# CodexploreRepo/deepfm

Measured on AMD Instinct MI355X. Metric: train samples/sec DeepFM Criteo-shape bs4096, higher is better.
Workload: dtype f32

## Files before the change

deepfm_amd/_lib.py:

```python

from __future__ import annotations

import ctypes as C
import os
from typing import Optional

_HERE = os.path.dirname(os.path.abspath(__file__))
LIB_PATH = os.environ.get("DFM_LIB_PATH") or os.path.join(_HERE, "lib", "libdeepfm_hip.so")

ABI_VERSION = 9

MAX_FIELDS = 64
MAX_RANKS = 64
ROWPLAN_CHUNK = 4096
RECORD_PARAM_LDS_BYTES = 32768
BWD_RECORD_MAX_ROW_SAMPLES = 1 << 27
BWD_RECORD_LDS_BYTES = 65536
SPARSE, DENSE, SEQUENCE = 0, 1, 2
COMBINER = {"mean": 0, "sum": 1, "max": 2}

c_float_p = C.c_void_p
c_int_p = C.c_void_p


class Field(C.Structure):
    _fields_ = [("kind", C.c_int32), ("dim", C.c_int32), ("vocab", C.c_int32), ("max_len", C.c_int32),
                ("combiner", C.c_int32), ("flat_offset", C.c_int32), ("stride2", C.c_int32),
                ("stride1", C.c_int32),
                ("w2", C.c_void_p), ("b2", C.c_void_p), ("w1", C.c_void_p), ("b1", C.c_void_p),
                ("proj", C.c_void_p)]


class FieldGrad(C.Structure):
    _fields_ = [("w2", C.c_void_p), ("b2", C.c_void_p), ("w1", C.c_void_p), ("b1", C.c_void_p),
                ("proj", C.c_void_p)]


class Table(C.Structure):
    _fields_ = [("w2", C.c_void_p), ("m2", C.c_void_p), ("v2", C.c_void_p),
                ("w1", C.c_void_p), ("m1", C.c_void_p), ("v1", C.c_void_p),
                ("stride2", C.c_int32), ("stride1", C.c_int32)]


class Optim(C.Structure):
    _fields_ = [("kind", C.c_int32), ("beta1", C.c_float), ("beta2", C.c_float), ("eps", C.c_float),
                ("weight_decay", C.c_float), ("momentum", C.c_float), ("d_lr", C.c_void_p)]


OPT_ADAM, OPT_ADAMW, OPT_SGD = 0, 1, 2


class BnBwd(C.Structure):
    _fields_ = [("z", C.c_void_p), ("mean_rstd", C.c_void_p), ("gamma", C.c_void_p), ("beta", C.c_void_p),
                ("dy", C.c_void_p), ("g_gamma", C.c_void_p), ("g_beta", C.c_void_p),
                ("seed", C.c_void_p), ("workspace", C.c_void_p), ("p_drop", C.c_float), ("salt", C.c_int32)]


class FmBwd(C.Structure):
    _fields_ = [("g_fm", C.c_void_p), ("fm_sum", C.c_void_p), ("e", C.c_void_p), ("addend", C.c_void_p),
                ("dim", C.c_int32)]


class SlabRef(C.Structure):
    _fields_ = [("workspace", C.c_void_p), ("g_w", C.c_void_p), ("batch", C.c_int64), ("out_features", C.c_int32),
                ("in_features", C.c_int32), ("splits", C.c_int32), ("reserved", C.c_int32)]


class SplitJob(C.Structure):
    _fields_ = [("src", C.c_void_p), ("rows", C.c_int64), ("cols", C.c_int64), ("planes_f", C.c_void_p),
                ("planes_s", C.c_void_p)]


class PartialJob(C.Structure):
    _fields_ = [("kind", C.c_int32), ("blocks", C.c_int32), ("n1", C.c_int32), ("n2", C.c_int32),
                ("accumulate", C.c_int32), ("reserved", C.c_int32), ("partial", C.c_void_p), ("out_w", C.c_void_p),
                ("out_b", C.c_void_p), ("ldw", C.c_int64)]


class HeadTail(C.Structure):
    _fields_ = [("g_w", C.c_void_p), ("g_b", C.c_void_p), ("loss", C.c_void_p), ("g_b2", C.c_void_p)]


_P, _I, _L, _F, _SZ = C.c_void_p, C.c_int, C.c_int64, C.c_float, C.c_size_t
SIGNATURES = {
    "dfm_abi_version": (_I, []),
    "dfm_last_error": (C.c_char_p, []),
    "dfm_device_info": (_I, [_P, _P, C.c_char_p, _I]),
    "dfm_debug_empty_launch": (_I, [_P]),
    "dfm_embedding_plan_create": (_I, [C.POINTER(Field), _I, _I, C.POINTER(_P)]),
    "dfm_embedding_plan_destroy": (_I, [_P]),
    "dfm_embedding_plan_is_uniform": (_I, [_P]),
    "dfm_embedding_workspace_bytes": (_SZ, [_P, _L]),
    "dfm_embedding_forward": (_I, [_P, C.POINTER(_P), _L, _P, _P, _P, _P, _P, _P, _P, _P]),
    "dfm_embedding_forward_staged": (_I, [_P, C.POINTER(_P), C.POINTER(_P), _P, _P, _L, _P, _P, _P, _P, _P, _P]),
    "dfm_embedding_forward_staged_update": (_I, [_P, _P, _P, C.POINTER(_P), C.POINTER(_P), _P, _P, _L, _P, _P, _P, _P, _P]),
    "dfm_embedding_forward_record": (_I, [_P, _P, _L, _P, _P, _P, _L, _P, _P, _P, _P]),
    "dfm_embedding_forward_record_update": (_I, [_P, _P, _P, _P, _L, _P, _P, _P, _L, _P, _P, _P]),
    "dfm_embedding_backward_record_parts": (_I, [_L]),
    "dfm_embedding_backward_record_workspace_bytes": (_SZ, [_L, _L]),
    "dfm_embedding_backward_record": (_I, [_P, _P, _L, _P, _P, _P, _L, _P, _L, C.POINTER(FieldGrad), _P, _L, _P, _P]),
    "dfm_embedding_backward_record_update": (_I, [_P, _P, _P, _P, _L, _P, _P, _P, _L, _P, _L, C.POINTER(FieldGrad), _P,
                                                  _L, _P]),
    "dfm_embedding_forward_record_sum": (_I, [_P, _P, _L, _P, _P, _P, _L, _P, _P, _P, _P, _P]),
    "dfm_embedding_forward_record_sum_update": (_I, [_P, _P, _P, _P, _L, _P, _P, _P, _L, _P, _P, _P, _P]),
    "dfm_embedding_backward_record_fm": (_I, [_P, _P, _L, _P, _P, _P, _L, _P, _L, _P, _P, _P, C.POINTER(FieldGrad), _P,
                                              _L, _P, _P]),
    "dfm_embedding_backward_record_fm_update": (_I, [_P, _P, _P, _P, _L, _P, _P, _P, _L, _P, _L, _P, _P, _P,
                                                     C.POINTER(FieldGrad), _P, _L, _P]),
    "dfm_graph_last_node": (_I, [_P, C.POINTER(_P)]),
    "dfm_gather_timing_begin": (_I, [_I]),
    "dfm_gather_timing_end": (_I, [C.POINTER(C.c_float), _I, C.POINTER(_I)]),
    "dfm_gather_set_shape": (_I, [_I]),
    "dfm_cin_set_mode": (_I, [_I]),
    "dfm_cin_get_mode": (_I, []),
    "dfm_embedding_backward_dense": (_I, [_P, C.POINTER(_P), _L, _P, _P, _P, C.POINTER(FieldGrad), _P, _P]),
    "dfm_embedding_backward_dense_fields": (_I, [_P, C.POINTER(_P), _L, _P, _P, _P, C.POINTER(FieldGrad), _P]),
    "dfm_rowplan_build": (_I, [C.POINTER(_P), C.POINTER(C.c_int32), _I, _L, _P, _P, _P, _P, _P, _P, _I, _P]),
    "dfm_rowplan_build_update": (_I, [_P, _P, C.POINTER(_P), C.POINTER(C.c_int32), _I, _L, _P, _P, _P, _P, _P, _P, _I]),
    "dfm_rowgrad_build": (_I, [C.POINTER(C.c_int32), _I, _I, _I, _L, _P, _P, _P, _P, _P, _P, _P, _P]),
    "dfm_rowadam_num_partials": (_L, [_I, _I, _I]),
    "dfm_grad_norm_finalize": (_I, [_P, _L, _F, _P, _P, _P, _P, _P]),
    "dfm_cin_output_dim": (_I, [C.POINTER(C.c_int32), _I, _I]),
    "dfm_cin_saved_bytes": (_SZ, [C.POINTER(C.c_int32), _I, _I, _L, _I, _I]),
    "dfm_cin_backward_workspace_bytes": (_SZ, [C.POINTER(C.c_int32), _I, _I, _L, _I, _I]),
    "dfm_cin_forward_workspace_bytes": (_SZ, [C.POINTER(C.c_int32), _I, _I, _I, _I]),
    "dfm_cin_forward": (_I, [_P, _L, _I, _I, C.POINTER(_P), C.POINTER(_P), C.POINTER(C.c_int32), _I, _I, _P, _P, _P, _P]),
    "dfm_cin_backward": (_I, [_P, _L, _I, _I, C.POINTER(_P), C.POINTER(C.c_int32), _I, _I, _P, _P, _P,
                              C.POINTER(_P), C.POINTER(_P), _P, _P]),
    "dfm_attention_forward": (_I, [_P, _L, _I, _I, _I, _I, _I, C.POINTER(_P), _P, _P]),
    "dfm_attention_backward_workspace_bytes": (_SZ, [_L, _I, _I]),
    "dfm_attention_backward": (_I, [_P, _P, _L, _I, _I, _I, _I, _I, C.POINTER(_P), _P, C.POINTER(_P), _P, _P]),
    "dfm_bn_workspace_bytes": (_SZ, [_L, _I]),
    "dfm_bn_relu_dropout_forward": (_I, [_P, _L, _I, _P, _P, _P, _P, _P, _F, _F, _F, _P, _I, _P, _P, _P, _P]),
    "dfm_bn_relu_dropout_backward": (_I, [_P, _P, _P, _P, _P, _L, _I, _F, _P, _I, _P, _P, _P, _P, _P]),
    "dfm_bce_workspace_bytes": (_SZ, [_L]),
    "dfm_bce_with_logits": (_I, [_P, _P, _L, _P, _P, _P, _P]),
    "dfm_gemm_workspace_bytes": (_SZ, [_I, _I, _I]),
    "dfm_gemm_f32": (_I, [_P, _L, _I, _P, _L, _I, _P, _L, _I, _I, _I, _P, _I, _P, _P]),
    "dfm_weight_grad_workspace_bytes": (_SZ, [_L, _I, _I]),
    "dfm_weight_grad_f32": (_I, [_P, _L, _P, _L, _L, _I, _I, _P, _L, _P, _I, _P, _P]),
    "dfm_attention_core_supported": (_I, [_I, _I, _I]),
    "dfm_attention_core_forward": (_I, [_P, _L, _I, _I, _I, _P, _P]),
    "dfm_attention_core_backward": (_I, [_P, _P, _L, _I, _I, _I, _P, _P]),
    "dfm_attention_qkv_core_supported": (_I, [_I, _I, _I, _I]),
    "dfm_attention_qkv_core_forward": (_I, [_P, _P, _P, _L, _I, _I, _I, _I, _P, _P]),
    "dfm_attention_qkv_core_backward": (_I, [_P, _P, _P, _P, _L, _I, _I, _I, _I, _P, _P]),
    "dfm_attention_block_supported": (_I, [_I, _I, _I, _I]),
    "dfm_attention_block_forward": (_I, [_P, _P, _P, _P, _P, _P, _P, _F, _L, _I, _I, _I, _I, _P, _P, _P, _P, _L, _P, _L,
                                         _P]),
    "dfm_attention_block_backward": (_I, [_P, _P, _P, _P, _P, _I, _L, _I, _I, _I, _I, _P, _P, _P, _L, _P, _P, _P]),
    "dfm_layernorm_workspace_bytes": (_SZ, [_L, _I]),
    "dfm_layernorm_forward": (_I, [_P, _P, _L, _I, _P, _P, _F, _P, _P, _L, _L, _P]),
    "dfm_layernorm_backward": (_I, [_P, _P, _P, _P, _L, _I, _P, _P, _P, _P, _P, _L, _L, _P]),
    "dfm_linear_bn_workspace_bytes": (_SZ, [_L, _I]),
    "dfm_linear_bn_forward": (_I, [_P, _L, _P, _P, _L, _I, _I, _P, _P, _P]),
    "dfm_bn_relu_dropout_apply": (_I, [_P, _L, _I, _P, _P, _P, _P, _P, _P, _P, _F, _F, _F, _P, _I, _P, _P]),
    "dfm_bn_bwd_workspace_bytes": (_SZ, [_L, _I]),
    "dfm_bn_backward_apply": (_I, [C.POINTER(BnBwd), _L, _I, C.POINTER(HeadTail), _P, _P]),
    "dfm_linear1_supported": (_I, [_I]),
    "dfm_linear1_forward": (_I, [_P, _L, _I, _P, _P, _P, _P]),
    "dfm_linear1_backward_splits": (_I, [_L]),
    "dfm_linear1_backward": (_I, [_P, _P, _L, _I, _P, _P, _P, _P]),
    "dfm_head_bce": (_I, [_P, _L, _I, _P, _P, _P, _P, _P, _P, _P, C.POINTER(BnBwd), _P]),
    "dfm_head_bn_bce": (_I, [_P, _P, _P, _P, _P, _F, _F, _L, _I, _P, _P, _P, _P, _P, _P, _P, C.POINTER(BnBwd), _P]),
    "dfm_linear_backward_workspace_bytes": (_SZ, [_L, _I, _I]),
    "dfm_linear_backward": (_I, [_P, _L, _I, _P, _I, _P, _P, C.POINTER(BnBwd), C.POINTER(FmBwd), _I, _P, _P]),
    "dfm_linear_backward_finish": (_I, [C.POINTER(SlabRef), _I, _P]),
    "dfm_linear_backward_splits": (_I, [_L, _I, _I]),
    "dfm_step_embedding_backward": (_I, [_P, _I, C.POINTER(_P), C.POINTER(FieldGrad), C.POINTER(C.c_int32), _I, _I, _I,
                                         _L, _P, _P, _P, _P, _P, _P, _P, _P, _I, _P, _L, _P]),
    "dfm_step_prepare_num_partials": (_L, [_I, _I, _I, _L]),
    "dfm_step_match_bytes": (_SZ, [_I, _I]),
    "dfm_step_prepare": (_I, [C.POINTER(Table), _I, _I, _I, _P, _P, _P, _P, _P, _F, _F, _P, _P, _L, _L,
                              C.POINTER(SlabRef), _I, _P, _I, _L, _P, _L, _P, _P]),
    "dfm_step_apply": (_I, [C.POINTER(Table), _I, _I, _I, _P, _P, _P, _P, _P, _P, C.POINTER(Optim), _P, _P, _P, _P,
                            _P, _L, _I, _P]),
    "dfm_step_apply_plan": (_I, [C.POINTER(Table), _I, _I, _I, _P, _P, _P, _P, _P, _P, C.POINTER(Optim), _P, _P, _P,
                                 _P, _P, _L, _I, _P, _L, _P, _I, _L, _P, _P, _P, _P, _P, _P]),
    "dfm_step_apply_plan_update": (_I, [_P, _P, C.POINTER(Table), _I, _I, _I, _P, _P, _P, _P, _P, _P,
                                        C.POINTER(Optim), _P, _P, _P, _P, _P, _L, _I, _P, _L, _P, _I, _L, _P, _P, _P,
                                        _P, _P]),
    "dfm_step_dense_num_partials": (_L, [_L]),
    "dfm_step_dense_prepare": (_I, [_F, _P, _P, _L, _L, C.POINTER(SlabRef), _I, _P, _P]),
    "dfm_step_dense_apply": (_I, [_P, C.POINTER(Optim), _P, _P, _P, _P, _P, _L, _I, _P]),
    "dfm_weight_grad_partial_blocks": (_I, [_L]),
    "dfm_weight_grad_partials_f32": (_I, [_P, _L, _P, _L, _L, _I, _I, _P, _P]),
    "dfm_weight_grad_partials_pair_f32": (_I, [_P, _L, _P, _L, _I, _I, _P, _P, _L, _P, _L, _I, _I, _P, _L, _P]),
    "dfm_layernorm_partial_blocks": (_I, [_L]),
    "dfm_partials_finish": (_I, [C.POINTER(PartialJob), _I, _P]),
    "dfm_tower_set_mode": (_I, [_I]),
    "dfm_tower_get_mode": (_I, []),
    "dfm_planes_bytes": (_SZ, [_L, _L]),
    "dfm_tower_x6_supported": (_I, [_L, _I, _I]),
    "dfm_split_planes": (_I, [C.POINTER(SplitJob), _I, _P]),
    "dfm_linear_bn_forward_x6": (_I, [_P, _L, _P, _P, _P, _L, _I, _I, _P, _P, _P]),
    "dfm_bn_relu_dropout_apply_planes": (_I, [_P, _L, _I, _P, _P, _P, _P, _P, _P, _P, _F, _F, _F, _P, _I, _P, _P, _P,
                                              _P]),
    "dfm_bn_backward_apply_planes": (_I, [C.POINTER(BnBwd), _L, _I, C.POINTER(HeadTail), _P, _P, _P, _P]),
    "dfm_linear_backward_x6_splits": (_I, [_L, _I, _I]),
    "dfm_linear_backward_x6_workspace_bytes": (_SZ, [_L, _I, _I]),
    "dfm_linear_backward_x6": (_I, [_P, _P, _L, _I, _P, _P, _I, _P, _P, C.POINTER(BnBwd), C.POINTER(FmBwd), _P, _P]),
    "dfm_fm_forward": (_I, [_P, _L, _I, _I, _P, _P]),
    "dfm_fm_backward": (_I, [_P, _P, _L, _I, _I, _P, _P]),
    "dfm_copy_2d": (_I, [_P, _L, _P, _L, _L, _I, _P]),
    "dfm_stage_record": (_I, [_P, _P, _L, _P]),
    "dfm_stage_record_update": (_I, [_P, _P, _P, _P, _L]),
    "dfm_shard_gather": (_I, [C.POINTER(Table), C.POINTER(C.c_int32), _I, _I, _I, _L, _P, _P, _P, _P, _P]),
    "dfm_shard_pack_segment": (_L, [_L, _I, _I, _L]),
    "dfm_shard_pack": (_I, [C.POINTER(C.c_int32), C.POINTER(C.c_int32), _I, C.POINTER(C.c_int32), _I, _I, _I, _L,
                            _P, _P, _P, _L, C.POINTER(SlabRef), _I, _P, _P]),
    "dfm_shard_rowgrad": (_I, [_I, _I, _I, _L, _P, _L, _P, _P, _P, _P, _P, _P]),
    "dfm_sum_floats": (_I, [_P, _L, _P, _P]),
    "dfm_embedding_grad_combine": (_I, [_P, _L, _P, _P, _P, _P, _L, _I, _I, _P, _P]),
    "dfm_linear_bn_eval": (_I, [_P, _L, _P, _P, _L, _I, _I, _P, _P, _P, _P, _F, _P, _P]),
    "dfm_predict_head": (_I, [_P, _L, _I, _P, _P, _P, _P, _L, _P, _P, _P]),
    "dfm_predict_head_update": (_I, [_P, _P, _P, _L, _I, _P, _P, _P, _P, _L, _P, _P]),
    "dfm_metrics_workspace_bytes": (_SZ, [_L]),
    "dfm_metrics_prepare": (_I, [_P, _P, _L, _P, _P, _P]),
    "dfm_metrics_finish": (_I, [_P, _P, _L, _P, _P, _P, _P]),
    "dfm_ranking_workspace_bytes": (_SZ, [_L, _L]),
    "dfm_ranking_metrics": (_I, [_P, _P, _P, _L, _L, _P, _I, _I, _P, _P, _P]),
}

_lib: Optional[C.CDLL] = None


class HipLibraryError(RuntimeError):
    pass


def load() -> C.CDLL:
    global _lib
    if _lib is not None:
        return _lib
    if not os.path.exists(LIB_PATH):
        raise HipLibraryError(
            f"{LIB_PATH} not found: build it with `python -c 'import __graft_entry__ as g; g.build()'` "
            "(or `make -C deepfm_amd/csrc`). deepfm_amd has no CPU or eager-PyTorch fallback.")
    lib = C.CDLL(LIB_PATH)
    for name, (restype, argtypes) in SIGNATURES.items():
        fn = getattr(lib, name)
        fn.restype = restype
        fn.argtypes = argtypes
    if lib.dfm_abi_version() != ABI_VERSION:
        raise HipLibraryError(f"ABI version mismatch: library {lib.dfm_abi_version()} != binding {ABI_VERSION} "
                              f"(stale {LIB_PATH}? rebuild with make -C deepfm_amd/csrc)")
    _lib = lib
    return lib


ERR_UNSUPPORTED = 3


def check(rc: int) -> None:
    if rc != 0:
        msg = load().dfm_last_error().decode("utf-8", "replace")
        raise HipLibraryError(f"deepfm_hip error {rc}: {msg}")


def ptr(t) -> int:
    return 0 if t is None else t.data_ptr()


def stream_handle() -> int:
    import torch
    return torch.cuda.current_stream().cuda_stream


def require_device(t, what: str) -> None:
    if not t.is_cuda:
        raise RuntimeError(
            f"{what} is on {t.device}: deepfm_amd runs on an MI355X HIP device only "
            "(there is no CPU fallback; use the reference implementation on CPU).")
```

deepfm_amd/csrc/step_tail.hip:

```cpp
#include "rowplan_body.h"
#include "tail_bodies.h"

using namespace dfm;
using namespace dfm::tail;

namespace {
constexpr int kStepPrepPerThread = 4;
__device__ __forceinline__ void dense_prepare_slabs_body(int blk, float* __restrict__ g, const float* __restrict__ p,
                                                         int64_t n, int64_t n_l2, float l2, const SlabTable& st,
                                                         const float* __restrict__ gathered, int world,
                                                         int64_t gathered_stride, float scale,
                                                         float* __restrict__ partial) {
  const int64_t i = (static_cast<int64_t>(blk) * kTailThreads + threadIdx.x) * kStepPrepPerThread;
  float sq = 0.f;
  const float k = 2.f * l2;
  if (i + 3 < n) {
    float4 gi = ld4(g + i);
    bool dirty = false;
    if (gathered) {
      gi = make_float4(0.f, 0.f, 0.f, 0.f);
      for (int r = 0; r < world; ++r) {
        const float4 t = ld4(gathered + static_cast<int64_t>(r) * gathered_stride + i);
        gi.x += t.x; gi.y += t.y; gi.z += t.z; gi.w += t.w;
      }
      gi.x *= scale; gi.y *= scale; gi.z *= scale; gi.w *= scale;
      dirty = true;
    }
    if (add_slabs(gi, g + i, st)) dirty = true;
    if (i < n_l2) {
      const float4 pi = ld4(p + i);
      gi.x = fmaf(k, pi.x, gi.x); gi.y = fmaf(k, pi.y, gi.y); gi.z = fmaf(k, pi.z, gi.z); gi.w = fmaf(k, pi.w, gi.w);
      dirty = true;
    }
    if (dirty) st4(g + i, gi);
    sq = fmaf(gi.x, gi.x, sq); sq = fmaf(gi.y, gi.y, sq); sq = fmaf(gi.z, gi.z, sq); sq = fmaf(gi.w, gi.w, sq);
  } else {
    for (int64_t e = i; e < n; ++e) {
      float ge = g[e];
      if (gathered) {
        ge = 0.f;
        for (int r = 0; r < world; ++r) ge += gathered[static_cast<int64_t>(r) * gathered_stride + e];
        ge *= scale;
        g[e] = ge;
      }
      if (e < n_l2) { ge = fmaf(k, p[e], ge); g[e] = ge; }
      sq = fmaf(ge, ge, sq);
    }
  }
  block_partial(sq, partial, blk);
}
}

__global__ __launch_bounds__(kTailThreads) void step_embedding_backward_kernel(
    int dense_blocks, const int32_t* __restrict__ dense_list, PtrTable in, GradTable gt, int64_t B, int F, int D,
    const float* __restrict__ g_first, const float* __restrict__ g_field, FieldMap fmap, int S, int lists,
    const int32_t* __restrict__ sorted_pos, int32_t* seg_start,
    const int32_t* __restrict__ num_uniq, float* __restrict__ row_g2, float* __restrict__ row_g1,
    DensePartials dp) {
  const int blk = blockIdx.x;
  if (blk < dense_blocks)
    dense_fields_uniform_body(blk, dense_list, in, gt, B, F, D, g_first, g_field, dp);
  else
    rowgrad_body(blk - dense_blocks, fmap, S, F, D, lists, g_first, g_field, sorted_pos, seg_start, num_uniq, row_g2,
                 row_g1);
}

constexpr int kMatchThreads = 1024;
__global__ __launch_bounds__(kMatchThreads) void step_match_kernel(int S, int L, const int32_t* __restrict__ uniq_rows,
                                                                  const int32_t* __restrict__ num_uniq,
                                                                  uint8_t* __restrict__ match) {
  rowadam_match_body<kMatchThreads>(blockIdx.x, S, L, uniq_rows, num_uniq, match);
}

__global__ __launch_bounds__(kTailThreads) void step_prepare_kernel(
    int merge_blocks, TableArgs tabs, int S, int D, int L, const int32_t* __restrict__ uniq_rows,
    const int32_t* __restrict__ num_uniq, float* __restrict__ row_g2, float* __restrict__ row_g1,
    int32_t* __restrict__ owner_flag, float grad_scale, float l2, float* __restrict__ g, const float* __restrict__ p,
    int64_t n, int64_t n_l2, SlabTable slabs, const float* __restrict__ dense_gathered, int world,
    int64_t gathered_stride, float* __restrict__ partial, int64_t dense_partial_offset,
    const uint8_t* __restrict__ match) {
  const int blk = blockIdx.x;
  if (blk < merge_blocks)
    rowadam_merge_body(blk, tabs, S, D, L, uniq_rows, num_uniq, row_g2, row_g1, owner_flag, grad_scale, l2, partial,
                       match);
  else
    dense_prepare_slabs_body(blk - merge_blocks, g, p, n, n_l2, l2, slabs, dense_gathered, world, gathered_stride,
                             grad_scale, partial + dense_partial_offset);
}

__global__ __launch_bounds__(1024) void norm_finalize_kernel(const float* __restrict__ partial, int n,
                                                             float max_norm, float* __restrict__ sq_out,
                                                             float* __restrict__ clip_out,
                                                             int32_t* __restrict__ step_tick,
                                                             int64_t* __restrict__ seed_tick) {
  __shared__ float wsum[16];
  float acc = 0.f;
  for (int i = threadIdx.x; i < n; i += 1024) acc += partial[i];
#pragma unroll
  for (int m = 32; m >= 1; m >>= 1) acc += __shfl_xor(acc, m, kWave);
  if (lane_id() == 0) wsum[threadIdx.x >> 6] = acc;
  __syncthreads();
  if (threadIdx.x == 0) {
    float tot = 0.f;
    for (int i = 0; i < 16; ++i) tot += wsum[i];
    sq_out[0] = tot;
    if (clip_out) {
      float c = 1.f;
      if (max_norm > 0.f) c = fminf(1.f, max_norm / (sqrtf(tot) + 1e-6f));
      clip_out[0] = c;
    }
    if (step_tick) step_tick[0] += 1;
    if (seed_tick) seed_tick[0] += 1;
  }
}

template <int RULE>
__global__ __launch_bounds__(kTailThreads) void step_apply_kernel(
    int row_blocks, TableArgs tabs, int S, int D, int L, const int32_t* __restrict__ uniq_rows,
    const int32_t* __restrict__ num_uniq, const float* __restrict__ row_g2, const float* __restrict__ row_g1,
    const int32_t* __restrict__ owner_flag, const float* __restrict__ clip_coef, const float* __restrict__ lr_ptr,
    OptHyper h, const int32_t* __restrict__ step_ptr, float* __restrict__ p, float* __restrict__ m,
    float* __restrict__ v, float* __restrict__ g, int64_t n, int zero_grad) {
  const int blk = blockIdx.x;
  const float lr_now = lr_ptr[0];
  if (blk < row_blocks)
    rowadam_apply_body<RULE>(blk, tabs, S, D, L, uniq_rows, num_uniq, row_g2, row_g1, owner_flag, clip_coef, lr_now, h,
                             step_ptr);
  else
    dense_adam_body<RULE>(blk - row_blocks, p, m, v, g, n, clip_coef, lr_now, h, step_ptr, zero_grad ? g : nullptr);
}

template <typename KeyT, int SHIFT, int RULE>
__global__ __launch_bounds__(rowplan::SORT_THREADS) void step_apply_plan_kernel(
    int plan_blocks, const int64_t* __restrict__ ids_base, int64_t ids_stride, const int32_t* __restrict__ vocab,
    int64_t plan_n, int chunks, int32_t* __restrict__ p_sorted_pos, int32_t* __restrict__ p_uniq_rows,
    int32_t* __restrict__ p_seg_start, int32_t* __restrict__ p_num_uniq, int32_t* p_error,
    int row_blocks4, TableArgs tabs, int S, int D, int L, const int32_t* __restrict__ uniq_rows,
    const int32_t* __restrict__ num_uniq, const float* __restrict__ row_g2, const float* __restrict__ row_g1,
    const int32_t* __restrict__ owner_flag, const float* __restrict__ clip_coef, const float* __restrict__ lr_ptr,
    OptHyper h, const int32_t* __restrict__ step_ptr, float* __restrict__ p, float* __restrict__ m,
    float* __restrict__ v, float* __restrict__ g, int64_t n, int zero_grad) {
  if (static_cast<int>(blockIdx.x) < plan_blocks) {
    const int s = blockIdx.x % S, y = blockIdx.x / S;
    const int64_t* src = ids_base + s * ids_stride;
    if (y < chunks) {
      rowplan::rowplan_chunk_body<KeyT, SHIFT>(src, vocab[s], s, y, S, plan_n, p_sorted_pos, p_uniq_rows, p_seg_start,
                                               p_num_uniq, p_error, 0);
    } else {
      const int q = y - chunks;
      const dfm_table tb = tabs.t[s];
      rowplan::rowplan_touch_body(src, vocab[s], tb.w2, tb.stride2, q / rowplan::kTouchParts, q % rowplan::kTouchParts,
                                  plan_n);
    }
    return;
  }
  const int blk = (static_cast<int>(blockIdx.x) - plan_blocks) * (rowplan::SORT_THREADS / kTailThreads);
  const float lr_now = lr_ptr[0];
  if (blk < row_blocks4)
    rowadam_apply_body<RULE>(blk, tabs, S, D, L, uniq_rows, num_uniq, row_g2, row_g1, owner_flag, clip_coef, lr_now, h,
                             step_ptr);
  else
    dense_adam_body<RULE>(blk - row_blocks4, p, m, v, g, n, clip_coef, lr_now, h, step_ptr, zero_grad ? g : nullptr);
}

namespace {
int fill_tables(const dfm_table* tables, int S, int D, TableArgs* out, int need_state) {
  memset(out, 0, sizeof(*out));
  for (int s = 0; s < S; ++s) {
    DFM_REQUIRE(tables[s].w2 && tables[s].w1, "table %d: null weights", s);
    if (need_state >= 1) DFM_REQUIRE(tables[s].m2 && tables[s].m1, "table %d: null optimizer state", s);
    if (need_state >= 2) DFM_REQUIRE(tables[s].v2 && tables[s].v1, "table %d: null Adam state", s);
    out->t[s] = tables[s];
    if (out->t[s].stride2 == 0) out->t[s].stride2 = D;
    if (out->t[s].stride1 == 0) out->t[s].stride1 = 1;
    DFM_REQUIRE(out->t[s].stride2 >= D && out->t[s].stride2 % 4 == 0 && out->t[s].stride1 >= 1,
                "table %d: bad row strides", s);
  }
  return DFM_OK;
}
inline int64_t row_blocks(int S, int D, int L) {
  return (static_cast<int64_t>(L) * S * CH * (D / 4) + kTailThreads - 1) / kTailThreads;
}
inline int64_t prep_blocks(int64_t n) {
  const int64_t per = static_cast<int64_t>(kTailThreads) * kStepPrepPerThread;
  return (n + per - 1) / per;
}
}

extern "C" int dfm_step_embedding_backward(const int32_t* d_dense_list, int num_dense, const void* const* dense_x,
                                           const dfm_field_grad* dense_grads, const int32_t* field_of_sparse,
                                           int num_sparse, int num_fields, int dim, int64_t batch,
                                           const float* d_g_first, const float* d_g_field,
                                           const int32_t* d_sorted_pos, int32_t* d_seg_start,
                                           const int32_t* d_num_uniq, float* d_row_g2, float* d_row_g1,
                                           float* d_dense_partials, int dense_parts, const float* d_dense_grad_base,
                                           int64_t dense_grad_elems, dfm_stream_t stream) {
  DFM_REQUIRE(d_g_first && d_g_field, "null argument");
  DFM_REQUIRE(num_dense >= 0 && num_sparse >= 0 && num_dense + num_sparse > 0 && num_fields <= DFM_MAX_FIELDS &&
                  num_dense + num_sparse <= num_fields, "bad field counts");
  DFM_REQUIRE(dim > 0 && dim % 4 == 0 && batch > 0 && batch < (int64_t(1) << 31), "bad shape");
  DFM_REQUIRE((reinterpret_cast<uintptr_t>(d_g_field) & 15) == 0, "d_g_field must be 16-byte aligned");
  PtrTable in;
  GradTable gt;
  memset(&in, 0, sizeof(in));
  memset(&gt, 0, sizeof(gt));
  if (num_dense > 0) {
    DFM_REQUIRE(d_dense_list && dense_x && dense_grads, "null argument");
    for (int f = 0; f < num_fields; ++f) {
      in.p[f] = dense_x[f];
      gt.g[f] = dense_grads[f];
    }
  }
  FieldMap fm;
  memset(&fm, 0, sizeof(fm));
  int lists = 0;
  int64_t rg_blocks = 0;
  if (num_sparse > 0) {
    DFM_REQUIRE(field_of_sparse && d_sorted_pos && d_seg_start && d_num_uniq && d_row_g2 && d_row_g1, "null argument");
    for (int s = 0; s < num_sparse; ++s) {
      DFM_REQUIRE(field_of_sparse[s] >= 0 && field_of_sparse[s] < num_fields, "field_of_sparse[%d] out of range", s);
      fm.f[s] = field_of_sparse[s];
    }
    lists = static_cast<int>((batch + CH - 1) / CH) * num_sparse;
    rg_blocks = (static_cast<int64_t>(lists) * CH * (dim / 4) + kTailThreads - 1) / kTailThreads;
  }
  int dense_blocks = num_dense * (dim / 4 + 1);
  DensePartials dp = {nullptr, nullptr, 0, 0, 0};
  if (d_dense_partials && num_dense > 0) {
    DFM_REQUIRE(dense_parts >= 1 && dense_parts <= 64 && d_dense_grad_base && dense_grad_elems > 0, "bad dense slices");
    for (int i = 0; i < num_fields; ++i) {
      const dfm_field_grad& g = gt.g[i];
      if (!g.w2) continue;
      DFM_REQUIRE(g.w2 >= d_dense_grad_base && g.w2 + dim <= d_dense_grad_base + dense_grad_elems &&
                      g.b2 >= d_dense_grad_base && g.b2 + dim <= d_dense_grad_base + dense_grad_elems &&
                      g.w1 >= d_dense_grad_base && g.w1 < d_dense_grad_base + dense_grad_elems &&
                      g.b1 >= d_dense_grad_base && g.b1 < d_dense_grad_base + dense_grad_elems,
                  "field %d: a DENSE-field gradient buffer lies outside the sliced range", i);
    }
    dp.out = d_dense_partials; dp.base = d_dense_grad_base; dp.elems = dense_grad_elems;
    dp.rows = (batch + dense_parts - 1) / dense_parts;
    dp.per_slice = dense_blocks;
    dense_blocks *= dense_parts;
  }
  hipLaunchKernelGGL(step_embedding_backward_kernel, dim3(static_cast<unsigned>(dense_blocks + rg_blocks)),
                     dim3(kTailThreads), 0, as_stream(stream), dense_blocks, d_dense_list, in, gt, batch, num_fields, dim,
                     d_g_first, d_g_field, fm, num_sparse, lists, d_sorted_pos, d_seg_start, d_num_uniq, d_row_g2,
                     d_row_g1, dp);
  DFM_LAUNCH_CHECK();
  return DFM_OK;
}

extern "C" size_t dfm_step_match_bytes(int num_sparse, int num_lists) {
  return num_lists > 2 ? static_cast<size_t>(num_lists) * num_sparse * CH * num_lists : 0;
}

extern "C" int64_t dfm_rowadam_num_partials(int num_sparse, int dim, int num_lists) {
  return row_blocks(num_sparse, dim, num_lists);
}

extern "C" int64_t dfm_step_prepare_num_partials(int num_sparse, int dim, int num_lists, int64_t n) {
  return row_blocks(num_sparse, dim, num_lists) + prep_blocks(n);
}

extern "C" int dfm_step_prepare(const dfm_table* tables, int num_sparse, int dim, int num_lists,
                                const int32_t* d_uniq_rows, const int32_t* d_num_uniq, float* d_row_g2,
                                float* d_row_g1, int32_t* d_owner_flag, float grad_scale, float l2, float* d_g,
                                const float* d_p, int64_t n, int64_t n_l2, const dfm_slab_ref* slabs, int num_slabs,
                                const float* d_dense_gathered, int world, int64_t gathered_stride, float* d_partials,
                                int64_t dense_partial_offset, void* d_match, dfm_stream_t stream) {
  DFM_REQUIRE(tables && d_uniq_rows && d_num_uniq && d_row_g2 && d_row_g1 && d_owner_flag && d_partials && d_g && d_p,
              "null argument");
  DFM_REQUIRE(num_sparse > 0 && num_sparse <= DFM_MAX_FIELDS && num_lists > 0, "bad sizes");
  DFM_REQUIRE(dim > 0 && dim % 4 == 0 && dim <= 256, "dim must be a multiple of 4 and <= 256");
  DFM_REQUIRE(n > 0 && n_l2 >= 0 && n_l2 <= n && n_l2 % 16 == 0, "bad dense sizes (n_l2 must be a multiple of 16)");
  DFM_REQUIRE((reinterpret_cast<uintptr_t>(d_g) & 63) == 0 && (reinterpret_cast<uintptr_t>(d_p) & 15) == 0,
              "dense buffers must be 64-byte aligned");
  DFM_REQUIRE(!d_dense_gathered || (world >= 1 && (reinterpret_cast<uintptr_t>(d_dense_gathered) & 15) == 0 && n % 4 == 0),
              "gathered dense gradients: world >= 1, 16-byte aligned, n a multiple of 4");
  if (d_dense_gathered && gathered_stride == 0) gathered_stride = n;
  DFM_REQUIRE(!d_dense_gathered || (gathered_stride >= n && gathered_stride % 4 == 0),
              "gathered dense gradients: the stride between ranks must be >= n and a multiple of 4 floats");
  TableArgs ta;
  if (int rc = fill_tables(tables, num_sparse, dim, &ta, 0)) return rc;
  SlabTable st = {};
  if (int rc = fill_slab_table(slabs, num_slabs, d_g, n, &st)) return rc;
  const int64_t mb = row_blocks(num_sparse, dim, num_lists), pb = prep_blocks(n);
  if (dense_partial_offset == 0) dense_partial_offset = mb;
  DFM_REQUIRE(dense_partial_offset >= mb, "the dense partials must not overlap the %lld row partials", (long long)mb);
  uint8_t* match = (d_match && num_lists > 2) ? static_cast<uint8_t*>(d_match) : nullptr;
  if (match) {
    DFM_REQUIRE(num_lists <= 255, "at most 255 lists");
    hipLaunchKernelGGL(step_match_kernel, dim3(static_cast<unsigned>(num_sparse * num_lists * num_lists)),
                       dim3(kMatchThreads), 0, as_stream(stream), num_sparse, num_lists, d_uniq_rows, d_num_uniq, match);
    DFM_LAUNCH_CHECK();
  }
  hipLaunchKernelGGL(step_prepare_kernel, dim3(static_cast<unsigned>(mb + pb)), dim3(kTailThreads), 0,
                     as_stream(stream), static_cast<int>(mb), ta, num_sparse, dim, num_lists, d_uniq_rows, d_num_uniq,
                     d_row_g2, d_row_g1, d_owner_flag, grad_scale, l2, d_g, d_p, n, n_l2, st, d_dense_gathered, world,
                     gathered_stride, d_partials, dense_partial_offset, match);
  DFM_LAUNCH_CHECK();
  return DFM_OK;
}

extern "C" int dfm_grad_norm_finalize(const float* d_partials, int64_t num_partials, float max_norm,
                                      float* d_sq_norm, float* d_clip_coef, int32_t* d_step_tick,
                                      int64_t* d_seed_tick, dfm_stream_t stream) {
  DFM_REQUIRE(d_partials && d_sq_norm, "null argument");
  DFM_REQUIRE(num_partials >= 0 && num_partials < (int64_t(1) << 31), "bad partial count");
  hipLaunchKernelGGL(norm_finalize_kernel, dim3(1), dim3(1024), 0, as_stream(stream), d_partials,
                     static_cast<int>(num_partials), max_norm, d_sq_norm, d_clip_coef, d_step_tick, d_seed_tick);
  DFM_LAUNCH_CHECK();
  return DFM_OK;
}

namespace {
int check_optim(const dfm_optim* o) {
  DFM_REQUIRE(o, "null dfm_optim");
  DFM_REQUIRE(o->kind == DFM_OPT_ADAM || o->kind == DFM_OPT_ADAMW || o->kind == DFM_OPT_SGD,
              "unknown dfm_optim.kind %d", static_cast<int>(o->kind));
  DFM_REQUIRE(o->d_lr, "dfm_optim.d_lr must point to the learning rate on the device");
  DFM_REQUIRE((reinterpret_cast<uintptr_t>(o->d_lr) & 3) == 0, "dfm_optim.d_lr must be 4-byte aligned");
  return DFM_OK;
}
inline int state_needed(int kind) { return kind == DFM_OPT_SGD ? 1 : 2; }
inline OptHyper hyper_of(const dfm_optim& o) { return OptHyper{o.beta1, o.beta2, o.eps, o.weight_decay, o.momentum}; }
}

extern "C" int dfm_step_apply(const dfm_table* tables, int num_sparse, int dim, int num_lists,
                              const int32_t* d_uniq_rows, const int32_t* d_num_uniq, const float* d_row_g2,
                              const float* d_row_g1, const int32_t* d_owner_flag, const float* d_clip_coef,
                              const dfm_optim* opt, const int32_t* d_step, float* d_p, float* d_m, float* d_v,
                              float* d_g, int64_t n, int zero_grad, dfm_stream_t stream) {
  if (int rc = check_optim(opt)) return rc;
  const dfm_optim& o = *opt;
  DFM_REQUIRE(tables && d_uniq_rows && d_num_uniq && d_row_g2 && d_row_g1 && d_owner_flag && d_step && d_p && d_m &&
                  (d_v || o.kind == DFM_OPT_SGD) && d_g, "null argument");
  DFM_REQUIRE(num_sparse > 0 && num_sparse <= DFM_MAX_FIELDS && num_lists > 0 && n > 0, "bad sizes");
  DFM_REQUIRE(dim > 0 && dim % 4 == 0 && dim <= 256, "dim must be a multiple of 4 and <= 256");
  TableArgs ta;
  if (int rc = fill_tables(tables, num_sparse, dim, &ta, state_needed(o.kind))) return rc;
  const int64_t rb = row_blocks(num_sparse, dim, num_lists), ab = (n + kTailThreads - 1) / kTailThreads;
  const OptHyper h = hyper_of(o);
  const dim3 grid(static_cast<unsigned>(rb + ab));
  switch (o.kind) {
#define DFM_LAUNCH_APPLY(RULE)                                                                                          \
  hipLaunchKernelGGL((step_apply_kernel<RULE>), grid, dim3(kTailThreads), 0, as_stream(stream), static_cast<int>(rb), ta, \
                     num_sparse, dim, num_lists, d_uniq_rows, d_num_uniq, d_row_g2, d_row_g1, d_owner_flag,            \
                     d_clip_coef, o.d_lr, h, d_step, d_p, d_m, d_v, d_g, n, zero_grad)
    case DFM_OPT_ADAM: DFM_LAUNCH_APPLY(kRuleAdam); break;
    case DFM_OPT_ADAMW: DFM_LAUNCH_APPLY(kRuleAdamW); break;
    default: DFM_LAUNCH_APPLY(kRuleSGD); break;
#undef DFM_LAUNCH_APPLY
  }
  DFM_LAUNCH_CHECK();
  return DFM_OK;
}

namespace {
struct ApplyPlanLaunch {
  const void* func = nullptr;
  dim3 grid, block;
  unsigned lds = 0;
  int plan_blocks = 0, chunks = 0, row_blocks4 = 0, S = 0, D = 0, L = 0, zero_grad = 0;
  const int64_t* ids_base = nullptr;
  int64_t ids_stride = 0, plan_n = 0, n = 0;
  const int32_t* vocab = nullptr;
  int32_t *p_sorted_pos = nullptr, *p_uniq_rows = nullptr, *p_seg_start = nullptr, *p_num_uniq = nullptr, *p_error = nullptr;
  TableArgs tabs;
  const int32_t *uniq_rows = nullptr, *num_uniq = nullptr, *owner_flag = nullptr, *step_ptr = nullptr;
  const float *row_g2 = nullptr, *row_g1 = nullptr, *clip_coef = nullptr, *lr_ptr = nullptr;
  OptHyper h = {0, 0, 0, 0, 0};
  float *p = nullptr, *m = nullptr, *v = nullptr, *g = nullptr;
  void* params[36];
  void bind() {
    int k = 0;
    params[k++] = &plan_blocks; params[k++] = &ids_base; params[k++] = &ids_stride; params[k++] = &vocab;
    params[k++] = &plan_n; params[k++] = &chunks; params[k++] = &p_sorted_pos; params[k++] = &p_uniq_rows;
    params[k++] = &p_seg_start; params[k++] = &p_num_uniq; params[k++] = &p_error; params[k++] = &row_blocks4;
    params[k++] = &tabs; params[k++] = &S; params[k++] = &D; params[k++] = &L; params[k++] = &uniq_rows;
    params[k++] = &num_uniq; params[k++] = &row_g2; params[k++] = &row_g1; params[k++] = &owner_flag;
    params[k++] = &clip_coef; params[k++] = &lr_ptr; params[k++] = &h;
    params[k++] = &step_ptr; params[k++] = &p; params[k++] = &m; params[k++] = &v; params[k++] = &g; params[k++] = &n;
    params[k++] = &zero_grad;
  }
};

template <int RULE>
const void* apply_plan_func(bool narrow) {
  return narrow ? reinterpret_cast<const void*>(step_apply_plan_kernel<uint32_t, 12, RULE>)
                : reinterpret_cast<const void*>(step_apply_plan_kernel<unsigned long long, 32, RULE>);
}

int describe_apply_plan(const dfm_table* tables, int num_sparse, int dim, int num_lists, const int32_t* d_uniq_rows,
                        const int32_t* d_num_uniq, const float* d_row_g2, const float* d_row_g1,
                        const int32_t* d_owner_flag, const float* d_clip_coef, const dfm_optim& o,
                        const int32_t* d_step, float* d_p, float* d_m, float* d_v, float* d_g, int64_t n,
                        int zero_grad, const int64_t* d_next_ids, int64_t ids_stride, const int32_t* d_vocab,
                        int max_vocab, int64_t batch, int32_t* d_next_sorted_pos, int32_t* d_next_uniq_rows,
                        int32_t* d_next_seg_start, int32_t* d_next_num_uniq, int32_t* d_error_flag, ApplyPlanLaunch* a) {
  DFM_REQUIRE(tables && d_uniq_rows && d_num_uniq && d_row_g2 && d_row_g1 && d_owner_flag && d_step && d_p && d_m &&
                  (d_v || o.kind == DFM_OPT_SGD) && d_g, "null argument");
  DFM_REQUIRE(d_next_ids && d_vocab && d_next_sorted_pos && d_next_uniq_rows && d_next_seg_start && d_next_num_uniq,
              "null row-plan argument");
  DFM_REQUIRE(num_sparse > 0 && num_sparse <= DFM_MAX_FIELDS && num_lists > 0 && n > 0, "bad sizes");
  DFM_REQUIRE(dim > 0 && dim % 4 == 0 && dim <= 256, "dim must be a multiple of 4 and <= 256");
  DFM_REQUIRE(batch > 0 && batch < (int64_t(1) << 31) && ids_stride >= batch && max_vocab > 0, "bad batch / id stride");
  if (int rc = fill_tables(tables, num_sparse, dim, &a->tabs, state_needed(o.kind))) return rc;
  const bool narrow = max_vocab < (1 << 20) - 1;
  a->func = o.kind == DFM_OPT_ADAM ? apply_plan_func<kRuleAdam>(narrow)
          : o.kind == DFM_OPT_ADAMW ? apply_plan_func<kRuleAdamW>(narrow)
                                    : apply_plan_func<kRuleSGD>(narrow);
  a->lds = rowplan::lds_bytes(narrow);
  static bool allowed[3][2] = {{false, false}, {false, false}, {false, false}};
  if (!allowed[o.kind][narrow ? 0 : 1]) {
    DFM_HIP_TRY(hipFuncSetAttribute(a->func, hipFuncAttributeMaxDynamicSharedMemorySize, static_cast<int>(a->lds)));
    allowed[o.kind][narrow ? 0 : 1] = true;
  }
  constexpr int kPer = rowplan::SORT_THREADS / kTailThreads;
  const int64_t rb = row_blocks(num_sparse, dim, num_lists), ab = (n + kTailThreads - 1) / kTailThreads;
  const int64_t rb4 = (rb + kPer - 1) / kPer * kPer;
  a->chunks = static_cast<int>((batch + CH - 1) / CH);
  a->plan_blocks = num_sparse * a->chunks * (1 + rowplan::kTouchParts);
  a->row_blocks4 = static_cast<int>(rb4);
  a->grid = dim3(static_cast<unsigned>(a->plan_blocks + rb4 / kPer + (ab + kPer - 1) / kPer));
  a->block = dim3(rowplan::SORT_THREADS);
  a->S = num_sparse; a->D = dim; a->L = num_lists; a->zero_grad = zero_grad;
  a->ids_base = d_next_ids; a->ids_stride = ids_stride; a->vocab = d_vocab; a->plan_n = batch; a->n = n;
  a->p_sorted_pos = d_next_sorted_pos; a->p_uniq_rows = d_next_uniq_rows; a->p_seg_start = d_next_seg_start;
  a->p_num_uniq = d_next_num_uniq; a->p_error = d_error_flag;
  a->uniq_rows = d_uniq_rows; a->num_uniq = d_num_uniq; a->row_g2 = d_row_g2; a->row_g1 = d_row_g1;
  a->owner_flag = d_owner_flag; a->clip_coef = d_clip_coef; a->lr_ptr = o.d_lr; a->h = hyper_of(o);
  a->step_ptr = d_step; a->p = d_p; a->m = d_m; a->v = d_v; a->g = d_g;
  a->bind();
  return DFM_OK;
}

int update_apply_plan(void* graph_exec, void* node, const ApplyPlanLaunch& a) {
  return update_kernel_node(graph_exec, node, a.func, a.grid, a.block, a.lds, const_cast<void**>(a.params), true);
}
}

#define DFM_APPLY_PLAN_ARGS                                                                                              \
  tables, num_sparse, dim, num_lists, d_uniq_rows, d_num_uniq, d_row_g2, d_row_g1, d_owner_flag, d_clip_coef, *opt,      \
      d_step, d_p, d_m, d_v, d_g, n, zero_grad, d_next_ids, ids_stride, d_vocab, max_vocab, batch, d_next_sorted_pos,  \
      d_next_uniq_rows, d_next_seg_start, d_next_num_uniq, d_error_flag

extern "C" int dfm_step_apply_plan(const dfm_table* tables, int num_sparse, int dim, int num_lists,
                                   const int32_t* d_uniq_rows, const int32_t* d_num_uniq, const float* d_row_g2,
                                   const float* d_row_g1, const int32_t* d_owner_flag, const float* d_clip_coef,
                                   const dfm_optim* opt, const int32_t* d_step, float* d_p, float* d_m, float* d_v,
                                   float* d_g, int64_t n, int zero_grad, const int64_t* d_next_ids, int64_t ids_stride,
                                   const int32_t* d_vocab, int max_vocab, int64_t batch, int32_t* d_next_sorted_pos,
                                   int32_t* d_next_uniq_rows, int32_t* d_next_seg_start, int32_t* d_next_num_uniq,
                                   int32_t* d_error_flag, dfm_stream_t stream) {
  if (int rc = check_optim(opt)) return rc;
  ApplyPlanLaunch a;
  if (int rc = describe_apply_plan(DFM_APPLY_PLAN_ARGS, &a)) return rc;
  DFM_HIP_TRY(hipLaunchKernel(a.func, a.grid, a.block, a.params, a.lds, as_stream(stream)));
  DFM_LAUNCH_CHECK();
  return DFM_OK;
}

extern "C" int dfm_step_apply_plan_update(void* graph_exec, void* node, const dfm_table* tables, int num_sparse, int dim,
                                          int num_lists, const int32_t* d_uniq_rows, const int32_t* d_num_uniq,
                                          const float* d_row_g2, const float* d_row_g1, const int32_t* d_owner_flag,
                                          const float* d_clip_coef, const dfm_optim* opt, const int32_t* d_step,
                                          float* d_p, float* d_m, float* d_v, float* d_g, int64_t n, int zero_grad,
                                          const int64_t* d_next_ids, int64_t ids_stride, const int32_t* d_vocab,
                                          int max_vocab, int64_t batch, int32_t* d_next_sorted_pos,
                                          int32_t* d_next_uniq_rows, int32_t* d_next_seg_start,
                                          int32_t* d_next_num_uniq, int32_t* d_error_flag) {
  DFM_REQUIRE(graph_exec && node, "null argument");
  if (int rc = check_optim(opt)) return rc;
  ApplyPlanLaunch a;
  if (int rc = describe_apply_plan(DFM_APPLY_PLAN_ARGS, &a)) return rc;
  return update_apply_plan(graph_exec, node, a);
}

__global__ __launch_bounds__(kTailThreads) void step_dense_prepare_kernel(float l2, float* __restrict__ g,
                                                                          const float* __restrict__ p, int64_t n,
                                                                          int64_t n_l2, SlabTable slabs,
                                                                          float* __restrict__ partial) {
  dense_prepare_slabs_body(blockIdx.x, g, p, n, n_l2, l2, slabs, nullptr, 1, 0, 1.f, partial);
}

template <int RULE>
__global__ __launch_bounds__(kTailThreads) void step_dense_apply_kernel(
    const float* __restrict__ clip_coef, const float* __restrict__ lr_ptr, OptHyper h,
    const int32_t* __restrict__ step_ptr, float* __restrict__ p, float* __restrict__ m, float* __restrict__ v,
    float* __restrict__ g, int64_t n, int zero_grad) {
  dense_adam_body<RULE>(blockIdx.x, p, m, v, g, n, clip_coef, lr_ptr[0], h, step_ptr, zero_grad ? g : nullptr);
}

extern "C" int64_t dfm_step_dense_num_partials(int64_t n) { return n > 0 ? prep_blocks(n) : 0; }

extern "C" int dfm_step_dense_prepare(float l2, float* d_g, const float* d_p, int64_t n, int64_t n_l2,
                                      const dfm_slab_ref* slabs, int num_slabs, float* d_partials,
                                      dfm_stream_t stream) {
  DFM_REQUIRE(d_g && d_p && d_partials, "null argument");
  DFM_REQUIRE(n > 0 && n < (int64_t(1) << 40) && n_l2 >= 0 && n_l2 <= n && n_l2 % 16 == 0,
              "bad dense sizes (n_l2 must be a multiple of 16)");
  DFM_REQUIRE((reinterpret_cast<uintptr_t>(d_g) & 63) == 0 && (reinterpret_cast<uintptr_t>(d_p) & 15) == 0,
              "dense buffers must be 64-byte aligned");
  SlabTable st = {};
  if (int rc = fill_slab_table(slabs, num_slabs, d_g, n, &st)) return rc;
  hipLaunchKernelGGL(step_dense_prepare_kernel, dim3(static_cast<unsigned>(prep_blocks(n))), dim3(kTailThreads), 0,
                     as_stream(stream), l2, d_g, d_p, n, n_l2, st, d_partials);
  DFM_LAUNCH_CHECK();
  return DFM_OK;
}

extern "C" int dfm_step_dense_apply(const float* d_clip_coef, const dfm_optim* opt, const int32_t* d_step, float* d_p,
                                    float* d_m, float* d_v, float* d_g, int64_t n, int zero_grad,
                                    dfm_stream_t stream) {
  if (int rc = check_optim(opt)) return rc;
  const dfm_optim& o = *opt;
  DFM_REQUIRE(d_step && d_p && d_m && (d_v || o.kind == DFM_OPT_SGD) && d_g, "null argument");
  DFM_REQUIRE(n > 0 && n < (int64_t(1) << 38), "bad size");
  const OptHyper h = hyper_of(o);
  const dim3 grid(static_cast<unsigned>((n + kTailThreads - 1) / kTailThreads));
  switch (o.kind) {
#define DFM_LAUNCH_DENSE_APPLY(RULE)                                                                              \
  hipLaunchKernelGGL((step_dense_apply_kernel<RULE>), grid, dim3(kTailThreads), 0, as_stream(stream), d_clip_coef, \
                     o.d_lr, h, d_step, d_p, d_m, d_v, d_g, n, zero_grad)
    case DFM_OPT_ADAM: DFM_LAUNCH_DENSE_APPLY(kRuleAdam); break;
    case DFM_OPT_ADAMW: DFM_LAUNCH_DENSE_APPLY(kRuleAdamW); break;
    default: DFM_LAUNCH_DENSE_APPLY(kRuleSGD); break;
#undef DFM_LAUNCH_DENSE_APPLY
  }
  DFM_LAUNCH_CHECK();
  return DFM_OK;
}
```

deepfm_amd/csrc/tail_bodies.h:

```cpp
#pragma once

#include "common.h"

namespace dfm {
namespace tail {

constexpr int CH = DFM_ROWPLAN_CHUNK;
constexpr int kTailThreads = 256;

struct FieldMap {
  int32_t f[DFM_MAX_FIELDS];
};
struct TableArgs {
  dfm_table t[DFM_MAX_FIELDS];
};

constexpr int kMaxSlabs = 16;
struct SlabTable {
  const float* slabs[kMaxSlabs];
  float* g[kMaxSlabs];
  int64_t elems[kMaxSlabs];
  int splits[kMaxSlabs];
  int count;
};

__device__ __forceinline__ bool add_slabs(float4& gi, const float* gptr, const SlabTable& st) {
  bool any = false;
  for (int r = 0; r < st.count; ++r) {
    const int64_t off = gptr - st.g[r];
    if (off >= 0 && off < st.elems[r]) {
      const float* sl = st.slabs[r] + off;
      const int64_t stride = st.elems[r];
      const int splits = st.splits[r];
      int q = 0;
      for (; q + 8 <= splits; q += 8) {
        float4 t[8];
#pragma unroll
        for (int u = 0; u < 8; ++u) t[u] = ld4(sl + (q + u) * stride);
#pragma unroll
        for (int u = 0; u < 8; ++u) { gi.x += t[u].x; gi.y += t[u].y; gi.z += t[u].z; gi.w += t[u].w; }
      }
      for (; q < splits; ++q) {
        const float4 t = ld4(sl + q * stride);
        gi.x += t.x; gi.y += t.y; gi.z += t.z; gi.w += t.w;
      }
      any = true;
    }
  }
  return any;
}

__device__ __forceinline__ void block_partial(float sq, float* __restrict__ partial, int blk) {
  __shared__ float wsum[4];
#pragma unroll
  for (int m = 32; m >= 1; m >>= 1) sq += __shfl_xor(sq, m, kWave);
  if (lane_id() == 0) wsum[threadIdx.x >> 6] = sq;
  __syncthreads();
  if (threadIdx.x == 0) partial[blk] = (wsum[0] + wsum[1]) + (wsum[2] + wsum[3]);
}

__device__ __forceinline__ void block_sum2(float& a, float& b2) {
  __shared__ float sa[4], sb[4];
#pragma unroll
  for (int m = 32; m >= 1; m >>= 1) {
    a += __shfl_xor(a, m, kWave);
    b2 += __shfl_xor(b2, m, kWave);
  }
  const int w = threadIdx.x >> 6;
  __syncthreads();
  if (lane_id() == 0) { sa[w] = a; sb[w] = b2; }
  __syncthreads();
  a = sa[0] + sa[1] + sa[2] + sa[3];
  b2 = sb[0] + sb[1] + sb[2] + sb[3];
}

struct DensePartials {
  float* out;
  const float* base;
  int64_t elems, rows;
  int per_slice;
};
__device__ __forceinline__ void dense_fields_uniform_body(int blk, const int32_t* __restrict__ dense_list, PtrTable in, GradTable gt, int64_t B, int F, int D, const float* __restrict__ g_first, const float* __restrict__ g_field, DensePartials dp = DensePartials{nullptr, nullptr, 0, 0, 0}) {
  const int groups = D / 4 + 1;
  int64_t b_lo = 0, b_hi = B;
  int slice = 0;
  if (dp.out) {
    slice = blk / dp.per_slice;
    blk -= slice * dp.per_slice;
    b_lo = slice * dp.rows;
    b_hi = b_lo + dp.rows < B ? b_lo + dp.rows : B;
  }
  const int f = dense_list[blk / groups];
  const int jq = blk % groups;
  const float* x = static_cast<const float*>(in.p[f]);
  float sw[4] = {0.f, 0.f, 0.f, 0.f}, sb[4] = {0.f, 0.f, 0.f, 0.f};
  if (jq * 4 < D) {
    const float* g = g_field + static_cast<int64_t>(f) * D + jq * 4;
#pragma unroll 8
    for (int64_t b = b_lo + threadIdx.x; b < b_hi; b += 256) {
      const float4 v = ld4(g + b * F * D);
      const float xb = x[b];
      sw[0] = fmaf(xb, v.x, sw[0]); sw[1] = fmaf(xb, v.y, sw[1]);
      sw[2] = fmaf(xb, v.z, sw[2]); sw[3] = fmaf(xb, v.w, sw[3]);
      sb[0] += v.x; sb[1] += v.y; sb[2] += v.z; sb[3] += v.w;
    }
  } else {
    for (int64_t b = b_lo + threadIdx.x; b < b_hi; b += 256) {
      const float v = g_first[b];
      sw[0] = fmaf(x[b], v, sw[0]);
      sb[0] += v;
    }
  }
#pragma unroll
  for (int u = 0; u < 4; ++u) block_sum2(sw[u], sb[u]);
  if (threadIdx.x == 0) {
    const dfm_field_grad g = gt.g[f];
    if (dp.out) {
      float* o = dp.out + slice * dp.elems;
      if (jq * 4 < D) {
#pragma unroll
        for (int u = 0; u < 4; ++u) { o[(g.w2 + jq * 4 + u) - dp.base] = sw[u]; o[(g.b2 + jq * 4 + u) - dp.base] = sb[u]; }
      } else {
        o[g.w1 - dp.base] = sw[0]; o[g.b1 - dp.base] = sb[0];
      }
    } else if (jq * 4 < D) {
#pragma unroll
      for (int u = 0; u < 4; ++u) { g.w2[jq * 4 + u] += sw[u]; g.b2[jq * 4 + u] += sb[u]; }
    } else {
      g.w1[0] += sw[0]; g.b1[0] += sb[0];
    }
  }
}

struct SampleSegments {
  int64_t samples;
  int64_t stride;
};

constexpr int kLongRun = 64;
constexpr int kSplitRun = 2048;
constexpr int kMaxSplitRuns = 2;
constexpr int kMaxSlices = 64;
constexpr int kRowgradLds = 2048;

__device__ __forceinline__ void rowgrad_load(const float* __restrict__ g_field, const float* __restrict__ g_first,
                                             int64_t b, int F, int f, int D, int q, const SampleSegments& segs,
                                             float4& g, float& g1) {
  int64_t off = 0;
  if (segs.samples > 0) {
    const int64_t sg = b / segs.samples;
    off = sg * segs.stride;
    b -= sg * segs.samples;
  }
  g = ld4(g_field + off + (b * F + f) * D + q * 4);
  g1 = q == 0 ? g_first[off + b] : 0.f;
}
constexpr int kRunBatch = 8;
__device__ __forceinline__ void st_agent(float* p, float v) {
  __hip_atomic_store(p, v, __ATOMIC_RELAXED, __HIP_MEMORY_SCOPE_AGENT);
}
__device__ __forceinline__ float ld_agent(const float* p) {
  return __hip_atomic_load(p, __ATOMIC_RELAXED, __HIP_MEMORY_SCOPE_AGENT);
}
__device__ __forceinline__ void rowgrad_run(const float* __restrict__ g_field, const float* __restrict__ g_first,
                                            const int32_t* __restrict__ pos, int p0, int p1, int step, int F, int f,
                                            int D, int q, const SampleSegments& segs, float4& acc, float& acc1) {
  int32_t b[kRunBatch];
#pragma unroll
  for (int u = 0; u < kRunBatch; ++u) b[u] = p0 + u * step < p1 ? pos[p0 + u * step] : 0;
  for (int p = p0; p < p1; p += kRunBatch * step) {
    float4 g[kRunBatch];
    float g1[kRunBatch];
#pragma unroll
    for (int u = 0; u < kRunBatch; ++u) {
      g[u] = make_float4(0.f, 0.f, 0.f, 0.f);
      g1[u] = 0.f;
      if (p + u * step < p1) rowgrad_load(g_field, g_first, b[u], F, f, D, q, segs, g[u], g1[u]);
    }
    const int pn = p + kRunBatch * step;
#pragma unroll
    for (int u = 0; u < kRunBatch; ++u) b[u] = pn + u * step < p1 ? pos[pn + u * step] : 0;
#pragma unroll
    for (int u = 0; u < kRunBatch; ++u) {
      if (p + u * step < p1) {
        acc.x += g[u].x; acc.y += g[u].y; acc.z += g[u].z; acc.w += g[u].w;
        acc1 += g1[u];
      }
    }
  }
}

__device__ __forceinline__ void rowgrad_body(int blk, FieldMap fmap, int S, int F, int D, int lists, const float* __restrict__ g_first,
    const float* __restrict__ g_field, const int32_t* __restrict__ sorted_pos,
    int32_t* seg_start, const int32_t* __restrict__ num_uniq,
    float* row_g2, float* row_g1, SampleSegments segs = SampleSegments{0, 0}) {
  __shared__ float red[kRowgradLds];
  __shared__ int s_last;
  __shared__ int s_long, s_ent[kTailThreads], s_p0[kTailThreads], s_p1[kTailThreads];
  const int lpr = D / 4, groups = kTailThreads / lpr;
  const bool coop = kTailThreads % lpr == 0;
  const int q = threadIdx.x % lpr, grp = threadIdx.x / lpr;
  const int nbl = coop ? CH / groups : 1;
  int64_t list;
  int u;
  if (coop) {
    list = blk / nbl;
    u = grp * nbl + blk % nbl;
  } else {
    const int64_t entry = (static_cast<int64_t>(blk) * kTailThreads + threadIdx.x) / lpr;
    list = entry / CH;
    u = static_cast<int>(entry % CH);
  }
  const int nu = list < lists ? num_uniq[list] : 0;
  const bool valid = threadIdx.x < groups * lpr && u < nu;
  int32_t* seg = seg_start + (list < lists ? list : 0) * (CH + 1);
  const int n_split = coop && nu > 0 && nu <= CH - kSplitRun ? seg[CH] : 0;
  int p0 = 0, p1 = 0;
  if (valid) {
    p0 = seg[u]; p1 = seg[u + 1];
  }
  if (threadIdx.x == 0) s_long = 0;
  __syncthreads();
  const bool is_split = coop && valid && p1 - p0 > kSplitRun;
  const bool is_long = coop && valid && !is_split && p1 - p0 > kLongRun;
  if (is_long && q == 0) {
    const int i = atomicAdd(&s_long, 1);
    s_ent[i] = u; s_p0[i] = p0; s_p1[i] = p1;
  }
  if (valid && !is_long && !is_split) {
    const int f = fmap.f[static_cast<int>(list % S)];
    const int32_t* pos = sorted_pos + list * CH;
    float4 acc = make_float4(0.f, 0.f, 0.f, 0.f);
    float acc1 = 0.f;
    rowgrad_run(g_field, g_first, pos, p0, p1, 1, F, f, D, q, segs, acc, acc1);
    st4(row_g2 + (list * CH + u) * D + q * 4, acc);
    if (q == 0) row_g1[list * CH + u] = acc1;
  }
  __syncthreads();
  if (!s_long && !n_split) return;
  const int n_long = s_long;
  for (int e = 0; e < n_long; ++e) {
    const int64_t ls = list;
    const int ue = s_ent[e], q0 = s_p0[e], q1 = s_p1[e];
    const int f = fmap.f[static_cast<int>(ls % S)];
    const int32_t* pos = sorted_pos + ls * CH;
    float4 acc = make_float4(0.f, 0.f, 0.f, 0.f);
    float acc1 = 0.f;
    if (grp < groups) rowgrad_run(g_field, g_first, pos, q0 + grp, q1, groups, F, f, D, q, segs, acc, acc1);
    if (grp < groups) {
      st4(red + grp * (D + 4) + q * 4, acc);
      if (q == 0) red[grp * (D + 4) + D] = acc1;
    }
    __syncthreads();
    if (grp == 0) {
      float4 tot = make_float4(0.f, 0.f, 0.f, 0.f);
      float tot1 = 0.f;
      for (int gi = 0; gi < groups; ++gi) {
        const float4 v = ld4(red + gi * (D + 4) + q * 4);
        tot.x += v.x; tot.y += v.y; tot.z += v.z; tot.w += v.w;
        if (q == 0) tot1 += red[gi * (D + 4) + D];
      }
      st4(row_g2 + (ls * CH + ue) * D + q * 4, tot);
      if (q == 0) row_g1[ls * CH + ue] = tot1;
    }
    __syncthreads();
  }
  if (!n_split) return;
  const int nsl = nbl < kMaxSlices ? nbl : kMaxSlices, bl = blk % nbl;
  if (bl >= nsl) return;
  const int f = fmap.f[static_cast<int>(list % S)];
  const int32_t* pos = sorted_pos + list * CH;
  for (int e = 0; e < n_split; ++e) {
    const int ue = seg[CH - 1 - e];
    const int q0 = seg[ue], q1 = seg[ue + 1];
    const int per = (q1 - q0 + nsl - 1) / nsl;
    const int s0 = q0 + bl * per, s1 = s0 + per < q1 ? s0 + per : q1;
    float4 acc = make_float4(0.f, 0.f, 0.f, 0.f);
    float acc1 = 0.f;
    if (grp < groups) {
      rowgrad_run(g_field, g_first, pos, s0 + grp, s1, groups, F, f, D, q, segs, acc, acc1);
      st4(red + grp * (D + 4) + q * 4, acc);
      if (q == 0) red[grp * (D + 4) + D] = acc1;
    }
    __syncthreads();
    if (grp == 0) {
      float4 tot = make_float4(0.f, 0.f, 0.f, 0.f);
      float tot1 = 0.f;
      for (int gi = 0; gi < groups; ++gi) {
        const float4 v = ld4(red + gi * (D + 4) + q * 4);
        tot.x += v.x; tot.y += v.y; tot.z += v.z; tot.w += v.w;
        if (q == 0) tot1 += red[gi * (D + 4) + D];
      }
      const int64_t prow = list * CH + CH - 1 - (e * nsl + bl);
      st_agent(row_g2 + prow * D + q * 4 + 0, tot.x);
      st_agent(row_g2 + prow * D + q * 4 + 1, tot.y);
      st_agent(row_g2 + prow * D + q * 4 + 2, tot.z);
      st_agent(row_g2 + prow * D + q * 4 + 3, tot.w);
      if (q == 0) st_agent(row_g1 + prow, tot1);
    }
    __syncthreads();
  }
  int* counter = seg + (CH - 1 - kMaxSplitRuns);
  __syncthreads();
  if (threadIdx.x == 0)
    s_last = __hip_atomic_fetch_add(counter, 1, __ATOMIC_RELAXED, __HIP_MEMORY_SCOPE_AGENT) == nsl - 1 ? 1 : 0;
  __syncthreads();
  if (!s_last) return;
  const int nred = groups < nsl ? groups : nsl;
  for (int e = 0; e < n_split; ++e) {
    const int ue = seg[CH - 1 - e];
    if (grp < nred) {
      float4 acc = make_float4(0.f, 0.f, 0.f, 0.f);
      float acc1 = 0.f;
      for (int r = grp; r < nsl; r += groups) {
        const int64_t prow = list * CH + CH - 1 - (e * nsl + r);
        const float* pr = row_g2 + prow * D + q * 4;
        acc.x += ld_agent(pr); acc.y += ld_agent(pr + 1); acc.z += ld_agent(pr + 2); acc.w += ld_agent(pr + 3);
        if (q == 0) acc1 += ld_agent(row_g1 + prow);
      }
      st4(red + grp * (D + 4) + q * 4, acc);
      if (q == 0) red[grp * (D + 4) + D] = acc1;
    }
    __syncthreads();
    if (grp == 0) {
      float4 tot = make_float4(0.f, 0.f, 0.f, 0.f);
      float tot1 = 0.f;
      for (int gi = 0; gi < nred; ++gi) {
        const float4 v = ld4(red + gi * (D + 4) + q * 4);
        tot.x += v.x; tot.y += v.y; tot.z += v.z; tot.w += v.w;
        if (q == 0) tot1 += red[gi * (D + 4) + D];
      }
      st4(row_g2 + (list * CH + ue) * D + q * 4, tot);
      if (q == 0) row_g1[list * CH + ue] = tot1;
    }
    __syncthreads();
  }
  if (threadIdx.x == 0) __hip_atomic_store(counter, 0, __ATOMIC_RELAXED, __HIP_MEMORY_SCOPE_AGENT);
}

__device__ __forceinline__ int find_row(const int32_t* __restrict__ rows, int n, int32_t row) {
  int lo = 0, hi = n;
  while (lo < hi) {
    const int mid = (lo + hi) >> 1;
    const int32_t v = rows[mid];
    if (v < row) lo = mid + 1; else hi = mid;
  }
  return (lo < n && rows[lo] == row) ? lo : -1;
}

template <int THREADS>
__device__ __forceinline__ void rowadam_match_body(int blk, int S, int L, const int32_t* __restrict__ uniq_rows,
                                                   const int32_t* __restrict__ num_uniq,
                                                   uint8_t* __restrict__ match) {
  __shared__ int32_t rows[CH];
  const int s = blk % S;
  const int pair = blk / S;
  const int ln = pair / L, lq = pair % L;
  if (ln == lq) return;
  const int64_t lt = static_cast<int64_t>(ln) * S + s, lqs = static_cast<int64_t>(lq) * S + s;
  const int nt = num_uniq[lt], nq = num_uniq[lqs];
  for (int i = threadIdx.x; i < nt; i += THREADS) rows[i] = uniq_rows[lt * CH + i];
  __syncthreads();
  for (int u = threadIdx.x; u < nq; u += THREADS) {
    const int32_t row = uniq_rows[lqs * CH + u];
    int lo = 0, hi = nt;
    while (lo < hi) {
      const int mid = (lo + hi) >> 1;
      if (rows[mid] < row) lo = mid + 1; else hi = mid;
    }
    match[(lqs * CH + u) * L + ln] = (lo < nt && rows[lo] == row) ? 1 : 0;
  }
}

__device__ __forceinline__ void rowadam_merge_body(int blk, TableArgs tabs, int S, int D, int L, const int32_t* __restrict__ uniq_rows,
    const int32_t* __restrict__ num_uniq, float* __restrict__ row_g2, float* __restrict__ row_g1,
    int32_t* __restrict__ owner_flag, float grad_scale, float l2, float* __restrict__ partial,
    const uint8_t* __restrict__ match = nullptr) {
  const int lpr = D / 4;
  const int64_t t = static_cast<int64_t>(blk) * kTailThreads + threadIdx.x;
  const int q = static_cast<int>(t % lpr);
  const int64_t entry = t / lpr;
  const int64_t list = entry / CH;
  const int u = static_cast<int>(entry % CH);
  float sq = 0.f;
  if (list < static_cast<int64_t>(L) * S && u < num_uniq[list]) {
    const int l = static_cast<int>(list / S), s = static_cast<int>(list % S);
    const int32_t row = uniq_rows[list * CH + u];
    const uint8_t* mt = match ? match + (list * CH + u) * L : nullptr;
    bool owner = true;
    for (int lp = 0; lp < l && owner; ++lp) {
      const int64_t other = static_cast<int64_t>(lp) * S + s;
      if (mt ? mt[lp] != 0 : find_row(uniq_rows + other * CH, num_uniq[other], row) >= 0) owner = false;
    }
    if (q == 0) owner_flag[list * CH + u] = owner ? 1 : 0;
    if (owner) {
      float4 g = ld4(row_g2 + (list * CH + u) * D + q * 4);
      float g1 = q == 0 ? row_g1[list * CH + u] : 0.f;
      for (int ln = l + 1; ln < L; ++ln) {
        if (mt && mt[ln] == 0) continue;
        const int64_t other = static_cast<int64_t>(ln) * S + s;
        const int pos = find_row(uniq_rows + other * CH, num_uniq[other], row);
        if (pos >= 0) {
          const float4 o = ld4(row_g2 + (other * CH + pos) * D + q * 4);
          g.x += o.x; g.y += o.y; g.z += o.z; g.w += o.w;
          if (q == 0) g1 += row_g1[other * CH + pos];
        }
      }
      const dfm_table tb = tabs.t[s];
      const float4 w = ld4(tb.w2 + static_cast<int64_t>(row) * tb.stride2 + q * 4);
      const float k = 2.f * l2;
      g.x = fmaf(k, w.x, grad_scale * g.x); g.y = fmaf(k, w.y, grad_scale * g.y);
      g.z = fmaf(k, w.z, grad_scale * g.z); g.w = fmaf(k, w.w, grad_scale * g.w);
      st4(row_g2 + (list * CH + u) * D + q * 4, g);
      sq = g.x * g.x + g.y * g.y + g.z * g.z + g.w * g.w;
      if (q == 0) {
        g1 = fmaf(k, tb.w1[static_cast<int64_t>(row) * tb.stride1], grad_scale * g1);
        row_g1[list * CH + u] = g1;
        sq = fmaf(g1, g1, sq);
      }
    }
  }
  block_partial(sq, partial, blk);
}

enum OptRule : int { kRuleAdam = DFM_OPT_ADAM, kRuleAdamW = DFM_OPT_ADAMW, kRuleSGD = DFM_OPT_SGD };

struct OptHyper {
  float b1, b2, eps, wd, momentum;
};

__device__ __forceinline__ void adam1(float& w, float& m, float& v, float g, float b1, float b2,
                                      float step_size, float inv_bc2_sqrt, float eps) {
  m = fmaf(b1, m, (1.f - b1) * g);
  v = fmaf(b2, v, (1.f - b2) * g * g);
  const float denom = sqrtf(v) * inv_bc2_sqrt + eps;
  w -= step_size * (m / denom);
}

struct RuleScalars {
  float lr, step_size, inv_bc2_sqrt, decay;
};
template <int RULE>
__device__ __forceinline__ RuleScalars rule_scalars(float lr, const OptHyper& h, const int32_t* __restrict__ step_ptr) {
  RuleScalars r;
  r.lr = lr;
  r.step_size = 0.f; r.inv_bc2_sqrt = 0.f; r.decay = 1.f;
  if (RULE != kRuleSGD) {
    const float step = static_cast<float>(step_ptr[0]);
    r.step_size = lr / (1.f - powf(h.b1, step));
    r.inv_bc2_sqrt = 1.f / sqrtf(1.f - powf(h.b2, step));
  }
  if (RULE == kRuleAdamW) r.decay = 1.f - lr * h.wd;
  return r;
}

template <int RULE>
__device__ __forceinline__ void rule1(float& w, float& m, float& v, float g, const OptHyper& h, const RuleScalars& r) {
  if (RULE == kRuleSGD) {
    m = fmaf(h.momentum, m, g);
    w = fmaf(-r.lr, m, w);
  } else {
    if (RULE == kRuleAdamW) w *= r.decay;
    adam1(w, m, v, g, h.b1, h.b2, r.step_size, r.inv_bc2_sqrt, h.eps);
  }
}

template <int RULE>
__device__ __forceinline__ void rowadam_apply_body(int blk, TableArgs tabs, int S, int D, int L, const int32_t* __restrict__ uniq_rows,
    const int32_t* __restrict__ num_uniq, const float* __restrict__ row_g2,
    const float* __restrict__ row_g1, const int32_t* __restrict__ owner_flag,
    const float* __restrict__ clip_coef, float lr, const OptHyper& h,
    const int32_t* __restrict__ step_ptr) {
  const int lpr = D / 4;
  const int64_t t = static_cast<int64_t>(blk) * kTailThreads + threadIdx.x;
  const int q = static_cast<int>(t % lpr);
  const int64_t entry = t / lpr;
  const int64_t list = entry / CH;
  const int u = static_cast<int>(entry % CH);
  if (list >= static_cast<int64_t>(L) * S || u >= num_uniq[list]) return;
  if (!owner_flag[list * CH + u]) return;
  const int s = static_cast<int>(list % S);
  const int64_t row = uniq_rows[list * CH + u];
  const float clip = clip_coef ? clip_coef[0] : 1.f;
  const RuleScalars r = rule_scalars<RULE>(lr, h, step_ptr);
  const dfm_table tb = tabs.t[s];
  float4 g = ld4(row_g2 + (list * CH + u) * D + q * 4);
  const int64_t o2 = row * tb.stride2 + q * 4, o1 = row * tb.stride1;
  float4 w = ld4(tb.w2 + o2);
  float4 m = ld4(tb.m2 + o2);
  float4 v = RULE == kRuleSGD ? make_float4(0.f, 0.f, 0.f, 0.f) : ld4(tb.v2 + o2);
  rule1<RULE>(w.x, m.x, v.x, g.x * clip, h, r);
  rule1<RULE>(w.y, m.y, v.y, g.y * clip, h, r);
  rule1<RULE>(w.z, m.z, v.z, g.z * clip, h, r);
  rule1<RULE>(w.w, m.w, v.w, g.w * clip, h, r);
  st4(tb.w2 + o2, w);
  st4(tb.m2 + o2, m);
  if (RULE != kRuleSGD) st4(tb.v2 + o2, v);
  if (q == 0) {
    float w1 = tb.w1[o1], m1 = tb.m1[o1], v1 = RULE == kRuleSGD ? 0.f : tb.v1[o1];
    rule1<RULE>(w1, m1, v1, row_g1[list * CH + u] * clip, h, r);
    tb.w1[o1] = w1; tb.m1[o1] = m1;
    if (RULE != kRuleSGD) tb.v1[o1] = v1;
  }
}

template <int RULE>
__device__ __forceinline__ void dense_adam_body(int blk, float* __restrict__ p, float* __restrict__ m,
                                                float* __restrict__ v, const float* __restrict__ g, int64_t n,
                                                const float* __restrict__ clip_coef, float lr, const OptHyper& h,
                                                const int32_t* __restrict__ step_ptr, float* __restrict__ g_zero) {
  const int64_t i = static_cast<int64_t>(blk) * kTailThreads + threadIdx.x;
  if (i >= n) return;
  const float clip = clip_coef ? clip_coef[0] : 1.f;
  const RuleScalars r = rule_scalars<RULE>(lr, h, step_ptr);
  const float gi = g[i] * clip;
  float pi = p[i], mi = m[i], vi = RULE == kRuleSGD ? 0.f : v[i];
  rule1<RULE>(pi, mi, vi, gi, h, r);
  m[i] = mi;
  if (RULE != kRuleSGD) v[i] = vi;
  p[i] = pi;
  if (g_zero) g_zero[i] = 0.f;
}

}
}

extern "C" int dfm_linear_backward_splits(int64_t batch, int out_features, int in_features);

namespace dfm {
namespace tail {
inline int fill_slab_table(const dfm_slab_ref* slabs, int num_slabs, const float* d_g, int64_t n, SlabTable* st) {
  DFM_REQUIRE(num_slabs >= 0 && num_slabs <= kMaxSlabs && (num_slabs == 0 || slabs), "0..%d slab references", kMaxSlabs);
  memset(st, 0, sizeof(*st));
  for (int i = 0; i < num_slabs; ++i) {
    const dfm_slab_ref& h = slabs[i];
    DFM_REQUIRE(h.workspace && h.g_w && h.batch > 0 && h.out_features > 0 && h.in_features > 0, "incomplete dfm_slab_ref");
    const int64_t elems = static_cast<int64_t>(h.out_features) * h.in_features;
    DFM_REQUIRE(elems % 4 == 0 && (reinterpret_cast<uintptr_t>(h.workspace) & 15) == 0 && h.g_w >= d_g &&
                    h.g_w + elems <= d_g + n && ((h.g_w - d_g) % 16) == 0,
                "slab-backed weights must be 64-byte aligned views of the dense gradient buffer");
    st->slabs[i] = static_cast<const float*>(h.workspace);
    st->g[i] = h.g_w;
    st->elems[i] = elems;
    st->splits[i] = h.splits > 0 ? h.splits : dfm_linear_backward_splits(h.batch, h.out_features, h.in_features);
  }
  st->count = num_slabs;
  return DFM_OK;
}
}
}
```

deepfm_amd/models/layers/embedding.py:

```python

from __future__ import annotations

import ctypes as C
import os
from typing import Dict, List, Optional, Tuple

import torch
import torch.nn as nn

from deepfm_amd import _lib
from deepfm_amd.data.schema import DatasetSchema, FeatureType, FieldSchema

_KIND = {FeatureType.SPARSE: _lib.SPARSE, FeatureType.DENSE: _lib.DENSE, FeatureType.SEQUENCE: _lib.SEQUENCE}


def _holders(spec: FieldSchema) -> Tuple[nn.Module, nn.Module]:
    if spec.feature_type is FeatureType.SPARSE:
        return (nn.Embedding(spec.vocabulary_size, spec.embedding_dim, padding_idx=0),
                nn.Embedding(spec.vocabulary_size, 1, padding_idx=0))
    if spec.feature_type is FeatureType.SEQUENCE:
        return (nn.EmbeddingBag(spec.vocabulary_size, spec.embedding_dim, mode=spec.combiner, padding_idx=0),
                nn.EmbeddingBag(spec.vocabulary_size, 1, mode=spec.combiner, padding_idx=0))
    if spec.feature_type is FeatureType.DENSE:
        return nn.Linear(1, spec.embedding_dim), nn.Linear(1, 1)
    raise ValueError(f"unsupported feature type {spec.feature_type!r}")


class RowSparseBuffers:

    def __init__(self, num_sparse: int, dim: int, batch: int, device: torch.device) -> None:
        ch = _lib.ROWPLAN_CHUNK
        self.chunks = (batch + ch - 1) // ch
        self.batch, self.num_sparse, self.dim = batch, num_sparse, dim
        i32 = dict(dtype=torch.int32, device=device)
        f32 = dict(dtype=torch.float32, device=device)
        self.sorted_pos = torch.empty(self.chunks, num_sparse, ch, **i32)
        self.uniq_rows = torch.empty(self.chunks, num_sparse, ch, **i32)
        self.seg_start = torch.empty(self.chunks, num_sparse, ch + 1, **i32)
        self.num_uniq = torch.zeros(self.chunks, num_sparse, **i32)
        self.row_g2 = torch.empty(self.chunks, num_sparse, ch, dim, **f32)
        self.row_g1 = torch.empty(self.chunks, num_sparse, ch, **f32)
        self.has_grad = False


class FeatureEmbedding(nn.Module):
    def __init__(self, schema: DatasetSchema, fm_embed_dim: int = 16) -> None:
        super().__init__()
        self.schema = schema
        self.fm_embed_dim = fm_embed_dim
        self.field_names: List[str] = list(schema.fields)

        self.second_order_embeddings = nn.ModuleDict()
        self.first_order_embeddings = nn.ModuleDict()
        self.projections = nn.ModuleDict()
        for name, spec in schema.fields.items():
            second, first = _holders(spec)
            self.second_order_embeddings[name] = second
            self.first_order_embeddings[name] = first
            if spec.embedding_dim != fm_embed_dim:
                self.projections[name] = nn.Linear(spec.embedding_dim, fm_embed_dim, bias=False)
        self._init_weights()

        self.grad_mode = "dense"
        self.strict_indices = os.environ.get("DEEPFM_AMD_STRICT_INDICES", "0") == "1"
        self.rowsparse: Optional[RowSparseBuffers] = None
        self.packed: Dict[str, dict] = {}
        self._plan = None
        self._plan_key = None
        self._plan_uniform = False
        self._err: Optional[torch.Tensor] = None
        self._anchor: Optional[torch.Tensor] = None
        self._dense_list: Optional[torch.Tensor] = None
        self._plan_static = False
        self._sparse_pos = [i for i, s in enumerate(schema.fields.values())
                            if s.feature_type is FeatureType.SPARSE]
        self._row_source: Optional[Dict[str, Tuple[torch.Tensor, torch.Tensor]]] = None

    def _init_weights(self) -> None:
        for module in self.modules():
            if isinstance(module, (nn.Embedding, nn.EmbeddingBag)):
                nn.init.xavier_uniform_(module.weight.data[1:])
            elif isinstance(module, nn.Linear):
                nn.init.xavier_uniform_(module.weight.data)
                if module.bias is not None:
                    nn.init.zeros_(module.bias.data)

    def __del__(self):
        try:
            self._drop_plan()
        except Exception:
            pass

    def pin_plan(self, device: torch.device, pinned: bool = True) -> None:
        self._plan_static = False
        if pinned:
            self._ensure_plan(device)
        self._plan_static = pinned

    def bind_row_source(self, views: Optional[Dict[str, Tuple[torch.Tensor, torch.Tensor]]]) -> None:
        if views is not None:
            missing = [n for n, sp in self.schema.fields.items()
                       if sp.feature_type is FeatureType.SPARSE and n not in views]
            if missing:
                raise KeyError(f"bind_row_source: no view for SPARSE field(s) {missing[:3]}")
        self._row_source = views
        self._drop_plan()

    def _drop_plan(self) -> None:
        self._plan_static = False
        if self._plan is not None:
            _lib.load().dfm_embedding_plan_destroy(self._plan)
            self._plan = None
            self._plan_key = None

    def _field_params(self) -> List[Tuple[str, FieldSchema, nn.Module, nn.Module, Optional[nn.Module]]]:
        out = []
        for name in self.field_names:
            out.append((name, self.schema.fields[name], self.second_order_embeddings[name],
                        self.first_order_embeddings[name],
                        self.projections[name] if name in self.projections else None))
        return out

    def table_parameters(self) -> List[nn.Parameter]:
        out = []
        for name, spec, second, first, _ in self._field_params():
            if spec.feature_type is FeatureType.SPARSE:
                out += [second.weight, first.weight]
        return out

    def pack_tables_(self) -> "FeatureEmbedding":
        self.packed = {}
        for name, spec, second, first, _ in self._field_params():
            if spec.feature_type is not FeatureType.SPARSE:
                continue
            d, V = spec.embedding_dim, spec.vocabulary_size
            if d % 4:
                raise NotImplementedError("packed row records need embedding_dim % 4 == 0")
            rs = ((3 * d + 4 + 31) // 32) * 32
            buf = torch.zeros(V, rs, dtype=torch.float32, device=second.weight.device)
            buf[:, :d].copy_(second.weight.data)
            buf[:, d:d + 1].copy_(first.weight.data)
            second.weight.data = buf[:, :d]
            first.weight.data = buf[:, d:d + 1]
            self.packed[name] = dict(buffer=buf, m1=buf[:, d + 1:d + 2], v1=buf[:, d + 2:d + 3],
                                     m2=buf[:, d + 4:2 * d + 4], v2=buf[:, 2 * d + 4:3 * d + 4])
        self._drop_plan()
        return self

    def non_table_parameters(self) -> List[nn.Parameter]:
        tables = {id(p) for p in self.table_parameters()}
        return [p for p in self.parameters() if id(p) not in tables]

    def set_grad_mode(self, mode: str) -> "FeatureEmbedding":
        if mode not in ("dense", "rowsparse"):
            raise ValueError(f"grad_mode must be 'dense' or 'rowsparse', got {mode!r}")
        if mode == "rowsparse":
            for spec in self.schema.fields.values():
                if spec.feature_type is FeatureType.SEQUENCE or spec.embedding_dim != self.fm_embed_dim \
                        or self.fm_embed_dim % 4:
                    raise NotImplementedError(
                        "rowsparse gradients need a uniform schema (SPARSE/DENSE fields, "
                        "embedding_dim == fm_embed_dim, multiple of 4)")
        self.grad_mode = mode
        for p in self.table_parameters():
            p.requires_grad_(mode == "dense")
        return self

    def _ensure_plan(self, device: torch.device):
        if self._plan_static and self._plan is not None:
            return self._plan
        params = list(self.parameters())
        if self._row_source is not None:
            params = params + [t for pair in self._row_source.values() for t in pair]
        key = (device, tuple((p.data_ptr(), p.stride(0)) for p in params))
        if self._plan is not None and key == self._plan_key:
            return self._plan
        self._drop_plan()
        lib = _lib.load()
        n = len(self.field_names)
        if n > _lib.MAX_FIELDS:
            raise ValueError(f"{n} fields > DFM_MAX_FIELDS={_lib.MAX_FIELDS}")
        arr = (_lib.Field * n)()
        for i, (name, spec, second, first, proj) in enumerate(self._field_params()):
            w2, w1, rows = second.weight, first.weight, spec.vocabulary_size
            if self._row_source is not None and spec.feature_type is FeatureType.SPARSE:
                w2, w1 = self._row_source[name]
                rows = w2.shape[0]
            for p in (w2, w1):
                _lib.require_device(p, f"parameter of field {name!r}")
                if p.dtype != torch.float32 or p.dim() != 2 or (p.shape[1] > 1 and p.stride(1) != 1):
                    raise TypeError("embedding parameters must be float32 with contiguous rows")
            fd = arr[i]
            fd.kind = _KIND[spec.feature_type]
            fd.dim = spec.embedding_dim
            fd.vocab = rows if spec.feature_type is not FeatureType.DENSE else 0
            fd.max_len = spec.max_length
            fd.combiner = _lib.COMBINER[spec.combiner] if spec.feature_type is FeatureType.SEQUENCE else 0
            fd.w2, fd.w1 = w2.data_ptr(), w1.data_ptr()
            if spec.feature_type is not FeatureType.DENSE:
                fd.stride2, fd.stride1 = w2.stride(0), w1.stride(0)
            if spec.feature_type is FeatureType.DENSE:
                fd.b2, fd.b1 = second.bias.data_ptr(), first.bias.data_ptr()
            fd.proj = proj.weight.data_ptr() if proj is not None else None
        handle = C.c_void_p()
        _lib.check(lib.dfm_embedding_plan_create(arr, n, self.fm_embed_dim, C.byref(handle)))
        self._plan, self._plan_key = handle, key
        self._plan_uniform = bool(lib.dfm_embedding_plan_is_uniform(handle))
        if self._err is None or self._err.device != torch.device(device):
            self._err = torch.zeros(1, dtype=torch.int32, device=device)
        return handle

    def _gather_inputs(self, batch: Dict[str, torch.Tensor]) -> Tuple[List[torch.Tensor], int]:
        inputs: List[torch.Tensor] = []
        size = None
        for name in self.field_names:
            spec = self.schema.fields[name]
            x = batch[name]
            _lib.require_device(x, f"batch[{name!r}]")
            if spec.feature_type is FeatureType.DENSE:
                if x.dtype != torch.float32:
                    x = x.float()
                if x.dim() != 1:
                    raise ValueError(f"DENSE field {name!r} expects shape (B,), got {tuple(x.shape)}")
            else:
                if x.dtype != torch.int64:
                    x = x.long()
                want = 2 if spec.feature_type is FeatureType.SEQUENCE else 1
                if x.dim() != want:
                    raise ValueError(f"field {name!r} expects {want}-D ids, got {tuple(x.shape)}")
                if want == 2 and x.shape[1] != spec.max_length:
                    raise ValueError(f"SEQUENCE field {name!r} expects (B, {spec.max_length}), got {tuple(x.shape)}")
            x = x.contiguous()
            if size is None:
                size = x.shape[0]
            elif x.shape[0] != size:
                raise ValueError(f"field {name!r}: batch size {x.shape[0]} != {size}")
            inputs.append(x)
        return inputs, int(size)

    @staticmethod
    def _ptr_array(tensors: List[torch.Tensor]):
        arr = (C.c_void_p * len(tensors))()
        for i, t in enumerate(tensors):
            arr[i] = t.data_ptr()
        return arr

    def raise_on_bad_index(self) -> None:
        if self._err is not None and int(self._err.item()) != 0:
            self._err.zero_()
            raise IndexError("index out of range in FeatureEmbedding (id < 0 or id >= vocabulary_size)")

    def forward_into(self, inputs: List[torch.Tensor], B: int, fo: torch.Tensor, fe: torch.Tensor,
                     flat: Optional[torch.Tensor] = None, fm_out: Optional[torch.Tensor] = None,
                     ws: Optional[torch.Tensor] = None, fm_sum: Optional[torch.Tensor] = None) -> None:
        plan = self._ensure_plan(inputs[0].device)
        if B > 0:
            _lib.check(_lib.load().dfm_embedding_forward(
                plan, self._ptr_array(inputs), B, fo.data_ptr(), fe.data_ptr(), _lib.ptr(flat),
                _lib.ptr(fm_out), _lib.ptr(fm_sum), _lib.ptr(ws), self._err.data_ptr(), _lib.stream_handle()))

    def forward_staged(self, src_ptrs: List[int], stage_out: List[torch.Tensor], B: int, fo: torch.Tensor,
                       fe: torch.Tensor, fm_out: Optional[torch.Tensor] = None, fm_sum: Optional[torch.Tensor] = None,
                       extra_src_ptr: int = 0, extra_dst: Optional[torch.Tensor] = None) -> None:
        plan = self._ensure_plan(fe.device)
        if not self._plan_uniform:
            raise NotImplementedError("staged gather needs a uniform schema")
        if B > 0:
            src = (C.c_void_p * len(src_ptrs))(*src_ptrs)
            _lib.check(_lib.load().dfm_embedding_forward_staged(
                plan, src, self._ptr_array(stage_out), extra_src_ptr or None, _lib.ptr(extra_dst), B, fo.data_ptr(),
                fe.data_ptr(), _lib.ptr(fm_out), _lib.ptr(fm_sum), self._err.data_ptr(), _lib.stream_handle()))

    def forward_staged_update(self, graph_exec: int, node, src_ptrs: List[int], stage_out: List[torch.Tensor], B: int,
                              fo: torch.Tensor, fe: torch.Tensor, fm_out: Optional[torch.Tensor] = None,
                              fm_sum: Optional[torch.Tensor] = None, extra_src_ptr: int = 0,
                              extra_dst: Optional[torch.Tensor] = None) -> None:
        plan = self._ensure_plan(fe.device)
        src = (C.c_void_p * len(src_ptrs))(*src_ptrs)
        _lib.check(_lib.load().dfm_embedding_forward_staged_update(
            plan, C.c_void_p(graph_exec), node, src, self._ptr_array(stage_out), extra_src_ptr or None,
            _lib.ptr(extra_dst), B, fo.data_ptr(), fe.data_ptr(), _lib.ptr(fm_out), _lib.ptr(fm_sum),
            self._err.data_ptr()))

    def _record_args(self, record_ptr: int, B: int, fo: torch.Tensor, fe: Optional[torch.Tensor], flat_ptr: int,
                     ld_flat: int, fm_out: Optional[torch.Tensor], labels_out: Optional[torch.Tensor],
                     fm_sum: Optional[torch.Tensor] = None):
        head = (C.c_void_p(record_ptr), B, fo.data_ptr(), _lib.ptr(fe), C.c_void_p(flat_ptr), ld_flat, _lib.ptr(fm_out))
        mid = () if fm_sum is None else (fm_sum.data_ptr(),)
        return head + mid + (_lib.ptr(labels_out), self._err.data_ptr())

    def forward_record(self, record_ptr: int, B: int, fo: torch.Tensor, fe: Optional[torch.Tensor], flat_ptr: int,
                       ld_flat: int, fm_out: Optional[torch.Tensor] = None,
                       labels_out: Optional[torch.Tensor] = None, fm_sum: Optional[torch.Tensor] = None) -> None:
        plan = self._ensure_plan(fo.device)
        lib = _lib.load()
        fn = lib.dfm_embedding_forward_record if fm_sum is None else lib.dfm_embedding_forward_record_sum
        _lib.check(fn(plan, *self._record_args(record_ptr, B, fo, fe, flat_ptr, ld_flat, fm_out, labels_out, fm_sum),
                      _lib.stream_handle()))

    def forward_record_update(self, graph_exec: int, node, record_ptr: int, B: int, fo: torch.Tensor,
                              fe: Optional[torch.Tensor], flat_ptr: int, ld_flat: int,
                              fm_out: Optional[torch.Tensor] = None, labels_out: Optional[torch.Tensor] = None,
                              fm_sum: Optional[torch.Tensor] = None) -> None:
        plan = self._ensure_plan(fo.device)
        lib = _lib.load()
        fn = lib.dfm_embedding_forward_record_update if fm_sum is None else lib.dfm_embedding_forward_record_sum_update
        _lib.check(fn(plan, C.c_void_p(graph_exec), node,
                      *self._record_args(record_ptr, B, fo, fe, flat_ptr, ld_flat, fm_out, labels_out, fm_sum)))

    def _launch_forward(self, inputs: List[torch.Tensor], B: int, want_fm: bool = False):
        dev = inputs[0].device
        self._ensure_plan(dev)
        F, fm = len(self.field_names), self.fm_embed_dim
        fo = torch.empty(B, 1, dtype=torch.float32, device=dev)
        fe = torch.empty(B, F, fm, dtype=torch.float32, device=dev)
        flat = ws = fm_out = None
        if not self._plan_uniform:
            flat = torch.empty(B, self.schema.total_embedding_dim, dtype=torch.float32, device=dev)
            ws = torch.empty(max(B * F, 1), dtype=torch.float32, device=dev)
        elif want_fm:
            fm_out = torch.empty(B, 1, dtype=torch.float32, device=dev)
        self.forward_into(inputs, B, fo, fe, flat, fm_out, ws)
        if B > 0 and self.strict_indices:
            self.raise_on_bad_index()
        return fo, fe, flat, fm_out

    def backward_rowsparse(self, inputs: List[torch.Tensor], g_fo: torch.Tensor, g_fe: torch.Tensor,
                           dense_grads: Dict[int, torch.Tensor], sparse: bool = True,
                           dense_slices: Optional[Tuple[torch.Tensor, int, torch.Tensor]] = None) -> None:
        B, F, D = g_fe.shape
        if B == 0:
            return
        lib = _lib.load()
        plan = self._ensure_plan(g_fe.device)
        S = len(self._sparse_pos) if sparse else 0
        rs = self.rowsparse
        fmap = (C.c_int32 * max(S, 1))(*self._sparse_pos[:S])
        if dense_grads and self._plan_uniform and g_fe.data_ptr() % 16 == 0 and self._all_dense_grads(dense_grads):
            if self._dense_list is None or self._dense_list.device != g_fe.device:
                pos = [i for i, sp in enumerate(self.schema.fields.values()) if sp.feature_type is FeatureType.DENSE]
                self._dense_list = torch.tensor(pos, dtype=torch.int32, device=g_fe.device)
            nd = self._dense_list.numel()
            _lib.check(lib.dfm_step_embedding_backward(
                self._dense_list.data_ptr(), nd, self._ptr_array(inputs), self._grad_struct(dense_grads), fmap, S, F, D,
                B, g_fo.data_ptr(), g_fe.data_ptr(), rs.sorted_pos.data_ptr() if S else None,
                rs.seg_start.data_ptr() if S else None, rs.num_uniq.data_ptr() if S else None,
                rs.row_g2.data_ptr() if S else None, rs.row_g1.data_ptr() if S else None,
                dense_slices[0].data_ptr() if dense_slices else None, dense_slices[1] if dense_slices else 0,
                dense_slices[2].data_ptr() if dense_slices else None,
                dense_slices[0].numel() // dense_slices[1] if dense_slices else 0, _lib.stream_handle()))
            if S:
                rs.has_grad = True
            return
        if dense_grads:
            _lib.check(lib.dfm_embedding_backward_dense_fields(
                plan, self._ptr_array(inputs), B, g_fo.data_ptr(), g_fe.data_ptr(), None,
                self._grad_struct(dense_grads), _lib.stream_handle()))
        if S:
            _lib.check(lib.dfm_rowgrad_build(
                fmap, S, F, D, B, g_fo.data_ptr(), g_fe.data_ptr(), rs.sorted_pos.data_ptr(),
                rs.seg_start.data_ptr(), rs.num_uniq.data_ptr(), rs.row_g2.data_ptr(),
                rs.row_g1.data_ptr(), _lib.stream_handle()))
            rs.has_grad = True

    def _all_dense_grads(self, grads: Dict[int, torch.Tensor]) -> bool:
        for _, spec, second, first, _ in self._field_params():
            if spec.feature_type is FeatureType.DENSE:
                if any(id(p) not in grads for p in (second.weight, second.bias, first.weight, first.bias)):
                    return False
        return True

    def _grad_struct(self, grads: Dict[int, torch.Tensor]):
        arr = (_lib.FieldGrad * len(self.field_names))()
        for i, (name, spec, second, first, proj) in enumerate(self._field_params()):
            g = arr[i]
            g.w2 = _lib.ptr(grads.get(id(second.weight)))
            g.w1 = _lib.ptr(grads.get(id(first.weight)))
            if spec.feature_type is FeatureType.DENSE:
                g.b2 = _lib.ptr(grads.get(id(second.bias)))
                g.b1 = _lib.ptr(grads.get(id(first.bias)))
            if proj is not None:
                g.proj = _lib.ptr(grads.get(id(proj.weight)))
        return arr

    def _touch_tables(self):
        arr = (_lib.Table * len(self._sparse_pos))()
        for j, i in enumerate(self._sparse_pos):
            w = self.second_order_embeddings[self.field_names[i]].weight
            arr[j].w2, arr[j].stride2 = w.data_ptr(), w.stride(0)
        return arr

    def _rowplan_args(self, ids_ptrs, B: int, touch: bool):
        S = len(self._sparse_pos)
        rs = self.rowsparse
        ids = (C.c_void_p * S)(*ids_ptrs)
        specs = list(self.schema.fields.values())
        vocab = (C.c_int32 * S)(*[specs[i].vocabulary_size for i in self._sparse_pos])
        tabs = self._touch_tables() if touch else None
        keep = (ids, vocab, tabs)
        return keep, (ids, vocab, S, B, rs.sorted_pos.data_ptr(), rs.uniq_rows.data_ptr(), rs.seg_start.data_ptr(),
                      rs.num_uniq.data_ptr(), self._err.data_ptr(), tabs, self.fm_embed_dim)

    def build_rowplan(self, inputs: List[torch.Tensor], B: int, ids_ptrs: Optional[List[int]] = None,
                      touch: bool = False) -> RowSparseBuffers:
        dev = inputs[0].device
        S = len(self._sparse_pos)
        rs = self.rowsparse
        if rs is None or rs.batch != B or rs.row_g2.device != dev:
            rs = self.rowsparse = RowSparseBuffers(S, self.fm_embed_dim, B, dev)
        rs.has_grad = False
        if S == 0 or B == 0:
            return rs
        if ids_ptrs is None:
            ids_ptrs = [inputs[i].data_ptr() for i in self._sparse_pos]
        keep, args = self._rowplan_args(ids_ptrs, B, touch)
        _lib.check(_lib.load().dfm_rowplan_build(*args, _lib.stream_handle()))
        return rs

    def rowplan_update(self, graph_exec: int, node, ids_ptrs: List[int], B: int, touch: bool) -> None:
        keep, args = self._rowplan_args(ids_ptrs, B, touch)
        _lib.check(_lib.load().dfm_rowplan_build_update(C.c_void_p(graph_exec), node, *args))

    def forward(self, batch: Dict[str, torch.Tensor]) -> Tuple[torch.Tensor, torch.Tensor, torch.Tensor]:
        inputs, B = self._gather_inputs(batch)
        if self.grad_mode == "rowsparse":
            self._ensure_plan(inputs[0].device)
            if torch.is_grad_enabled():
                self.build_rowplan(inputs, B)
                if self._anchor is None or self._anchor.device != inputs[0].device:
                    self._anchor = torch.zeros(1, device=inputs[0].device, requires_grad=True)
                fo, fe = _RowSparseFn.apply(self, inputs, self._anchor, *self.non_table_parameters())
            else:
                fo, fe, _, _ = self._launch_forward(inputs, B)
            return fo, fe, fe.view(B, fe.shape[1] * fe.shape[2])
        params = list(self.parameters())
        if torch.is_grad_enabled() and any(p.requires_grad for p in params):
            outs = _DenseGradFn.apply(self, inputs, *params)
        else:
            fo, fe, flat, _ = self._launch_forward(inputs, B)
            outs = (fo, fe) if flat is None else (fo, fe, flat)
        if len(outs) == 2:
            return outs[0], outs[1], outs[1].view(B, outs[1].shape[1] * outs[1].shape[2])
        return outs


def _c(t: Optional[torch.Tensor], like: torch.Tensor) -> torch.Tensor:
    if t is None:
        return torch.zeros_like(like)
    return t.contiguous()


class _DenseGradFn(torch.autograd.Function):

    @staticmethod
    def forward(ctx, module: FeatureEmbedding, inputs, *params):
        B = inputs[0].shape[0]
        fo, fe, flat, _ = module._launch_forward(inputs, B)
        ctx.module, ctx.inputs, ctx.params = module, inputs, params
        ctx.flat = flat
        ctx.shapes = (fo, fe)
        if flat is None:
            return fo, fe
        return fo, fe, flat

    @staticmethod
    def backward(ctx, g_fo, g_fe, g_flat=None):
        module, inputs = ctx.module, ctx.inputs
        fo, fe = ctx.shapes
        B = fe.shape[0]
        g_fo, g_fe = _c(g_fo, fo), _c(g_fe, fe)
        if ctx.flat is not None:
            g_flat = _c(g_flat, ctx.flat)
        grads = {id(p): torch.zeros_like(p) for p in ctx.params}
        if B > 0:
            plan = module._ensure_plan(fe.device)
            _lib.check(_lib.load().dfm_embedding_backward_dense(
                plan, module._ptr_array(inputs), B, g_fo.data_ptr(), g_fe.data_ptr(), _lib.ptr(g_flat),
                module._grad_struct(grads), _lib.ptr(ctx.flat), _lib.stream_handle()))
        return (None, None) + tuple(grads[id(p)] if p.requires_grad else None for p in ctx.params)


class _RowSparseFn(torch.autograd.Function):

    @staticmethod
    def forward(ctx, module: FeatureEmbedding, inputs, anchor, *dense_params):
        B = inputs[0].shape[0]
        fo, fe, _, _ = module._launch_forward(inputs, B)
        ctx.module, ctx.inputs, ctx.params = module, inputs, dense_params
        ctx.shapes = (fo, fe)
        return fo, fe

    @staticmethod
    def backward(ctx, g_fo, g_fe):
        module, inputs = ctx.module, ctx.inputs
        fo, fe = ctx.shapes
        B, F, D = fe.shape
        g_fo, g_fe = _c(g_fo, fo), _c(g_fe, fe)
        grads = {id(p): torch.zeros_like(p) for p in ctx.params}
        module.backward_rowsparse(inputs, g_fo, g_fe, grads)
        return (None, None, None) + tuple(grads[id(p)] for p in ctx.params)
```

deepfm_amd/training/eligibility.py:

```python

from __future__ import annotations

from typing import Optional

from deepfm_amd import _lib
from deepfm_amd.data.schema import FeatureType

_BWD_STAGE = 256
_FAMILY = "DeepFM, xDeepFM and AttentionDeepFM"


def model_kind(model, exact: bool = True) -> Optional[str]:
    from deepfm_amd.models.attention_deepfm import AttentionDeepFM
    from deepfm_amd.models.deepfm import DeepFM
    from deepfm_amd.models.xdeepfm import xDeepFM
    family = {DeepFM: "deepfm", xDeepFM: "xdeepfm", AttentionDeepFM: "attention"}
    if exact:
        return family.get(type(model))
    return next((kind for cls, kind in family.items() if isinstance(model, cls)), None)


def family_reason(model, what: str, exact: bool = True) -> Optional[str]:
    if model_kind(model, exact) is None:
        return f"no {what} for {type(model).__name__}: {_FAMILY} only"
    return None


def _hidden_widths(dnn):
    return [dnn.mlp[4 * i].out_features for i in range(dnn._n_layers)]


def training_tower_reason(model) -> Optional[str]:
    if not model.training:
        return "the model must be in training mode"
    dnn = getattr(model, "dnn", None)
    ok = dnn is not None and getattr(dnn, "_fusable", False)
    if ok:
        widths, bn = _hidden_widths(dnn), dnn.mlp[1]
        ok = not (any(w % 4 for w in widths) or widths[-1] % 32 or widths[-1] > 256 or bn.momentum is None
                  or not bn.affine or dnn.mlp[0].in_features % 4)
    if not ok:
        return ("the DNN tower is not fusable: Linear -> BatchNorm1d (affine, momentum) -> ReLU, hidden widths "
                "multiples of 4, the last one a multiple of 32 and <= 256, input width a multiple of 4")
    return None


def eval_tower_reason(model) -> Optional[str]:
    dnn = model.dnn
    if not dnn._fusable:
        return "the DNN tower must be Linear -> BatchNorm1d -> ReLU (use_batch_norm=True, activation='relu')"
    widths = _hidden_widths(dnn)
    if any(w % 4 for w in widths):
        return f"hidden widths {widths} must be multiples of 4"
    for i in range(dnn._n_layers):
        bn = dnn.mlp[4 * i + 1]
        if not bn.affine or not bn.track_running_stats or bn.running_mean is None:
            return "every BatchNorm1d needs affine parameters and running statistics"
    return None


def attention_reason(model) -> Optional[str]:
    att = model.attention
    F = model.schema.num_fields
    if att.embed_dim % 4 or att.attention_dim % 4 or att.embed_dim > 64:
        return (f"attention embed_dim {att.embed_dim} / attention_dim {att.attention_dim}: the fused attention kernels "
                "take multiples of 4 with embed_dim <= 64")
    if not _lib.load().dfm_attention_core_supported(F, att.attention_dim, att.num_heads):
        return (f"attention over {F} fields with attention_dim {att.attention_dim} and {att.num_heads} heads is outside "
                "the attention core kernel's shapes (dfm_attention_core_supported)")
    if not all(b.gemm_path for b in att.layers):
        return "an attention block does not run on the GEMM path (gemm_path is off)"
    return None


def cin_reason(model) -> Optional[str]:
    cin = model.cin
    sizes = list(cin.layer_sizes)
    if not 1 <= len(sizes) <= 16:
        return f"the CIN has {len(sizes)} layers: the CIN kernels take 1 to 16"
    for i, c in enumerate(sizes):
        if c < 1 or (cin.split_half and i < len(sizes) - 1 and c < 2):
            return f"CIN layer {i} has {c} feature maps: too small" + (" to split in half" if c == 1 else "")
    return None


def _released_table(model) -> Optional[str]:
    for name, spec in model.schema.fields.items():
        if spec.feature_type is FeatureType.SPARSE and \
                model.embedding.second_order_embeddings[name].weight.shape[0] != spec.vocabulary_size:
            return name
    return None


def released_table_reason(model) -> Optional[str]:
    name = _released_table(model)
    if name is not None:
        return (f"the embedding table of field {name!r} is released (field-sharded model, "
                "TableShard.released): call restore_tables() first")
    return None


def uniform_schema_reason(model) -> Optional[str]:
    D = model.embedding.fm_embed_dim
    for name, spec in model.schema.fields.items():
        if spec.feature_type is FeatureType.SEQUENCE:
            return f"field {name!r} is a SEQUENCE field: the staged gather needs a uniform SPARSE / DENSE schema"
        if spec.embedding_dim != D or D % 4:
            return (f"field {name!r}: embedding_dim {spec.embedding_dim} with fm_embed_dim {D}: the staged gather "
                    "needs embedding_dim == fm_embed_dim, a multiple of 4")
    return None


def mixed_param_bytes(model) -> int:
    D = model.embedding.fm_embed_dim
    floats = 0
    for spec in model.schema.fields.values():
        d = spec.embedding_dim
        if d != D:
            floats += D * d
        if spec.feature_type is FeatureType.DENSE:
            floats += 2 * d + 4
    return 4 * floats


def record_gather_reason(model) -> Optional[str]:
    D = model.embedding.fm_embed_dim
    if D not in (4, 8, 16, 32, 64):
        return f"fm_embed_dim {D}: the record gather takes 4, 8, 16, 32 or 64"
    for name, spec in model.schema.fields.items():
        if spec.embedding_dim % 4:
            return f"field {name!r}: embedding_dim {spec.embedding_dim} is not a multiple of 4 (16-byte row pieces)"
    nbytes = mixed_param_bytes(model)
    if nbytes > _lib.RECORD_PARAM_LDS_BYTES:
        return (f"projection and DENSE parameters take {nbytes} bytes of LDS, over the record gather's cap of "
                f"{_lib.RECORD_PARAM_LDS_BYTES}")
    return None


def backward_lds_bytes(model) -> int:
    D = model.embedding.fm_embed_dim
    need = 0
    for spec in model.schema.fields.values():
        d = spec.embedding_dim
        L = spec.max_length if spec.feature_type is FeatureType.SEQUENCE else 1
        proj = D * d if d != D else 0
        need = max(need, 16 * (_BWD_STAGE * (d // 4 + 1) + (_BWD_STAGE * L + 3) // 4 + 1) + 4 * proj)
        if proj:
            need = max(need, 4 * _BWD_STAGE * (D + d))
    return need


def record_backward_reason(model, batch_size: Optional[int] = None) -> Optional[str]:
    specs = model.schema.fields
    for name, spec in specs.items():
        if spec.feature_type is FeatureType.SEQUENCE and spec.combiner == "max":
            return (f"field {name!r} pools with max: the embedding backward's arg-max recompute is not built "
                    "(mean and sum bags only; train it in dense autograd mode)")
    nbytes = backward_lds_bytes(model)
    if nbytes > _lib.BWD_RECORD_LDS_BYTES:
        return (f"the embedding backward stages {nbytes} bytes of LDS for the widest field, over its cap of "
                f"{_lib.BWD_RECORD_LDS_BYTES}")
    rows = sum(s.vocabulary_size for s in specs.values() if s.feature_type is not FeatureType.DENSE)
    if batch_size is not None and rows * batch_size > _lib.BWD_RECORD_MAX_ROW_SAMPLES:
        return (f"{rows} table rows x {batch_size} samples is over the row-owned scan's cap of "
                f"{_lib.BWD_RECORD_MAX_ROW_SAMPLES} (tables this large belong to a row-sparse design)")
    return None


def _predictor_reason(model, gather_reason) -> Optional[str]:
    if family_reason(model, "fused predictor") is not None:
        return f"no fused predictor for {type(model).__name__} ({_FAMILY} only)"
    reason = gather_reason(model) or eval_tower_reason(model)
    if reason is None and model_kind(model) == "attention" and attention_reason(model) is not None:
        reason = "attention blocks outside the fused attention kernels' shapes"
    return reason or released_table_reason(model)


def ineligible_reason(model) -> Optional[str]:
    return _predictor_reason(model, uniform_schema_reason)


def mixed_ineligible_reason(model) -> Optional[str]:
    return _predictor_reason(model, record_gather_reason)


def _mixed_step_reason(model, batch_size: Optional[int]) -> Optional[str]:
    if uniform_schema_reason(model) is None:
        return "uniform schema: use the row-sparse step (set_grad_mode('rowsparse') and fused_step_class(model))"
    reason = record_gather_reason(model) or record_backward_reason(model, batch_size)
    if reason is None and model.embedding.grad_mode != "dense":
        reason = "the embedding must be in 'dense' grad mode (its tables are dense parameters of the flat buffer)"
    return reason or training_tower_reason(model) or released_table_reason(model)


def mixed_train_ineligible_reason(model, batch_size: Optional[int] = None) -> Optional[str]:
    if model_kind(model) != "deepfm":
        return (f"no fused mixed-schema step for {type(model).__name__}: DeepFM only (xDeepFM and AttentionDeepFM "
                "are the next step, DESIGN.md section 9)")
    return _mixed_step_reason(model, batch_size)


def mixed_step_ineligible_reason(model, batch_size: Optional[int] = None) -> Optional[str]:
    reason = family_reason(model, "fused mixed-schema step") or _mixed_step_reason(model, batch_size)
    if reason is None:
        own = {"xdeepfm": cin_reason, "attention": attention_reason}.get(model_kind(model))
        reason = own(model) if own is not None else None
    return reason
```

deepfm_amd/training/rowsparse.py:

```python

from __future__ import annotations

import ctypes as C
from typing import Optional

import torch
import torch.distributed as dist

from deepfm_amd import _lib
from deepfm_amd.data.schema import FeatureType
from deepfm_amd.training import exchange
from deepfm_amd.models.layers.embedding import FeatureEmbedding


_KIND_CODE = {"adam": _lib.OPT_ADAM, "adamw": _lib.OPT_ADAMW, "sgd": _lib.OPT_SGD}


class RowSparseOptimizer:
    kind = "adam"
    row_tables = True

    def __init__(self, model: torch.nn.Module, lr: float = 1e-3, betas=(0.9, 0.999), eps: float = 1e-8,
                 l2: float = 0.0, max_grad_norm: Optional[float] = None,
                 process_group: Optional[dist.ProcessGroup] = None,
                 row_embedding: Optional[FeatureEmbedding] = None, weight_decay: float = 0.0,
                 momentum: float = 0.0) -> None:
        emb = model.embedding
        if not isinstance(emb, FeatureEmbedding):
            raise ValueError("model.embedding must be a FeatureEmbedding")
        if self.row_tables and emb.grad_mode != "rowsparse":
            raise ValueError("model.embedding must be a FeatureEmbedding in 'rowsparse' grad mode")
        self.model, self.emb = model, emb
        self.row_emb = row_embedding if row_embedding is not None else emb
        self.betas, self.eps, self.l2 = tuple(betas), eps, l2
        self.weight_decay, self.momentum = float(weight_decay), float(momentum)
        self.max_grad_norm = max_grad_norm
        self.group = process_group
        self.world = exchange.world_size(process_group)
        import os
        self.split = self.world > 1 or (os.environ.get("DFM_FORCE_DP_PATH") == "1" and dist.is_available()
                                        and dist.is_initialized())

        tables = self.row_emb.table_parameters() if self.row_tables else []
        if self.row_tables and not tables:
            raise ValueError("no SPARSE tables to optimise")
        anchor = tables[0] if tables else next(emb.parameters())
        dev = anchor.device
        _lib.require_device(anchor, "embedding tables")
        self.device = dev
        self._scalars = torch.zeros(16, dtype=torch.float32, device=dev)
        self._lr_dev = self._scalars[1:2]
        self.lr = lr
        self.num_sparse = len(tables) // 2
        self.dim = emb.fm_embed_dim
        second = self.kind != "sgd"
        self.exp_avg, self.exp_avg_sq = [], []
        sparse_names = [n for n, spec in self.row_emb.schema.fields.items() if spec.feature_type is FeatureType.SPARSE]
        for name, w2, w1 in zip(sparse_names, tables[0::2], tables[1::2]):
            rec = self.row_emb.packed.get(name) if getattr(self.row_emb, "packed", None) else None
            if rec is not None and rec["buffer"].data_ptr() == w2.data_ptr():
                self.exp_avg += [rec["m2"], rec["m1"]]
                self.exp_avg_sq += [rec["v2"], rec["v1"]] if second else [None, None]
            else:
                self.exp_avg += [torch.zeros_like(w2, memory_format=torch.contiguous_format),
                                 torch.zeros_like(w1, memory_format=torch.contiguous_format)]
                self.exp_avg_sq += ([torch.zeros_like(w2, memory_format=torch.contiguous_format),
                                     torch.zeros_like(w1, memory_format=torch.contiguous_format)] if second
                                    else [None, None])
        self._tables = tables
        self.step_count = torch.zeros(1, dtype=torch.int32, device=dev)
        self.sq_norm = torch.zeros(1, dtype=torch.float32, device=dev)
        self.clip_coef = self._scalars[0:1]
        self.clip_coef.fill_(1.0)

        table_ids = {id(p) for p in tables} | ({id(p) for p in emb.table_parameters()} if self.row_tables else set())
        emb_dense = [p for p in (emb.non_table_parameters() if self.row_tables else emb.parameters()) if p.requires_grad]
        emb_ids = {id(p) for p in emb_dense}
        others = [p for p in model.parameters()
                  if id(p) not in table_ids and id(p) not in emb_ids and p.requires_grad]
        groups = [g for m in model.modules() if hasattr(m, "adjacent_parameters") for g in m.adjacent_parameters()]
        for g in groups:
            ids = {id(p) for p in g}
            if all(any(p is q for q in others) for p in g):
                first = min(i for i, q in enumerate(others) if id(q) in ids)
                rest = [q for q in others if id(q) not in ids]
                first -= sum(1 for q in others[:first] if id(q) in ids)
                others = rest[:first] + list(g) + rest[first:]
        self.dense_params = emb_dense + others
        def padded(n):
            return (n + 15) // 16 * 16
        self.n_l2 = sum(padded(p.numel()) for p in emb_dense)
        total = sum(padded(p.numel()) for p in self.dense_params)
        self.flat_param = torch.zeros(total, dtype=torch.float32, device=dev)
        self.flat_grad = torch.zeros(total, dtype=torch.float32, device=dev)
        self.flat_m = torch.zeros(total, dtype=torch.float32, device=dev)
        self.flat_v = torch.zeros(total if second else 16, dtype=torch.float32, device=dev)
        off = 0
        for p in self.dense_params:
            n = p.numel()
            self.flat_param[off:off + n].copy_(p.data.reshape(-1))
            p.data = self.flat_param[off:off + n].view_as(p)
            p.grad = self.flat_grad[off:off + n].view_as(p)
            off += padded(n)
        self._owner = None
        self.next_plan = None
        self._vocab_dev, self._max_vocab, self._keep_tabs = None, 0, None
        specs = list(self.row_emb.schema.fields.values())
        vocab = [specs[i].vocabulary_size for i in self.row_emb._sparse_pos] if self.row_tables else []
        if vocab:
            self._vocab_dev = torch.tensor(vocab, dtype=torch.int32, device=self.device)
            self._max_vocab = max(vocab)
        self._gathered = None
        self._partials = None
        self._match = None
        self._cur = None
        self.seed_tick: Optional[torch.Tensor] = None
        self.slab_refs = None

    @property
    def lr(self) -> float:
        return self._lr

    @lr.setter
    def lr(self, value: float) -> None:
        if torch.cuda.is_current_stream_capturing():
            raise RuntimeError("the learning rate cannot be changed inside a graph capture (set it between launches)")
        self._lr = float(value)
        self._lr_dev.fill_(self._lr)

    @property
    def param_groups(self):
        return [_LrGroup(self)]

    def _optim_struct(self) -> "_lib.Optim":
        o = _lib.Optim()
        o.kind = _KIND_CODE[self.kind]
        o.beta1, o.beta2, o.eps = self.betas[0], self.betas[1], self.eps
        o.weight_decay, o.momentum = self.weight_decay, self.momentum
        o.d_lr = self._lr_dev.data_ptr()
        return o

    def zero_grad(self, force: bool = False) -> None:
        if force:
            self.flat_grad.zero_()
        if self.row_emb.rowsparse is not None:
            self.row_emb.rowsparse.has_grad = False

    def _table_struct(self):
        arr = (_lib.Table * self.num_sparse)()
        for s in range(self.num_sparse):
            t = arr[s]
            t.w2, t.w1 = self._tables[2 * s].data_ptr(), self._tables[2 * s + 1].data_ptr()
            t.m2, t.m1 = self.exp_avg[2 * s].data_ptr(), self.exp_avg[2 * s + 1].data_ptr()
            t.v2, t.v1 = _lib.ptr(self.exp_avg_sq[2 * s]), _lib.ptr(self.exp_avg_sq[2 * s + 1])
            t.stride2, t.stride1 = self._tables[2 * s].stride(0), self._tables[2 * s + 1].stride(0)
            for a, b in ((self.exp_avg[2 * s], t.stride2), (self.exp_avg_sq[2 * s], t.stride2),
                         (self.exp_avg[2 * s + 1], t.stride1), (self.exp_avg_sq[2 * s + 1], t.stride1)):
                if a is not None and a.stride(0) != b:
                    raise RuntimeError("Adam state and table row strides differ (re-create the optimizer after "
                                       "pack_tables_() / .to())")
        return arr

    @torch.no_grad()
    def exchange(self) -> None:
        rs = self.row_emb.rowsparse
        if rs is None or not rs.has_grad:
            raise RuntimeError(f"{type(self).__name__}: no row gradients (run a backward pass first)")
        local = (rs.uniq_rows, rs.num_uniq, rs.row_g2, rs.row_g1)
        if not self.split:
            self._cur = local + (rs.chunks,)
            return
        world = max(self.world, 1)
        full = (self.flat_grad.view(1, -1),) + local
        if self._gathered is None or self._gathered[1].shape[0] != world * rs.chunks:
            self._gathered = exchange.alloc_gathered(full, world)
        exchange.allgather_step(full, self._gathered, self.group)
        self._cur = self._gathered[1:] + (world * rs.chunks,)

    @torch.no_grad()
    def apply(self) -> None:
        lib = _lib.load()
        stream = _lib.stream_handle()
        grad_scale = 1.0 / self.world
        uniq, num, g2, g1, lists = self._cur
        n_dense = self.flat_param.numel()
        n_partials = lib.dfm_step_prepare_num_partials(self.num_sparse, self.dim, lists, n_dense)
        if self._owner is None or self._owner.shape != uniq.shape:
            self._owner = torch.empty_like(uniq)
            self._partials = torch.zeros(n_partials + self._extra_partial_count(lists), dtype=torch.float32,
                                         device=self.device)
            mbytes = lib.dfm_step_match_bytes(self.num_sparse, lists)
            self._match = torch.empty(mbytes, dtype=torch.uint8, device=self.device) if mbytes else None
        dense_gathered, gathered_stride = self._dense_source()
        tabs = self._table_struct()
        refs, n_refs = self.slab_refs if (self.slab_refs is not None and not self.split) else (None, 0)
        _lib.check(lib.dfm_step_prepare(tabs, self.num_sparse, self.dim, lists, uniq.data_ptr(), num.data_ptr(),
                                        g2.data_ptr(), g1.data_ptr(), self._owner.data_ptr(), grad_scale, self.l2,
                                        self.flat_grad.data_ptr(), self.flat_param.data_ptr(), n_dense, self.n_l2,
                                        refs, n_refs, _lib.ptr(dense_gathered), max(self.world, 1), gathered_stride,
                                        self._partials.data_ptr(), self._dense_partial_offset(lists),
                                        _lib.ptr(self._match), stream))
        norm_ptr, n_norm = self._norm_partials(n_partials, lists)
        _lib.check(lib.dfm_grad_norm_finalize(norm_ptr, n_norm,
                                              self.max_grad_norm or 0.0, self.sq_norm.data_ptr(),
                                              self.clip_coef.data_ptr(), self.step_count.data_ptr(),
                                              _lib.ptr(self.seed_tick), stream))
        if self.next_plan is not None:
            ids_ptr, target = self.next_plan
            self.next_plan = None
            _lib.check(lib.dfm_step_apply_plan(*self._apply_plan_args(self._cur, ids_ptr, target), stream))
        else:
            _lib.check(lib.dfm_step_apply(*self._apply_args(tabs, self._cur), stream))
        self.row_emb.rowsparse.has_grad = False

    def _apply_args(self, tabs, cur):
        uniq, num, g2, g1, lists = cur
        return (tabs, self.num_sparse, self.dim, lists, uniq.data_ptr(), num.data_ptr(), g2.data_ptr(), g1.data_ptr(),
                self._owner.data_ptr(), self.clip_coef.data_ptr(), C.byref(self._optim_struct()),
                self.step_count.data_ptr(), self.flat_param.data_ptr(), self.flat_m.data_ptr(), self._flat_v_ptr(),
                self.flat_grad.data_ptr(), self.flat_param.numel(), 1)

    def _apply_plan_args(self, cur, ids_ptr: int, target):
        if self._vocab_dev is None:
            raise RuntimeError(f"{type(self).__name__}: no SPARSE fields to plan for")
        tabs = self._table_struct()
        self._keep_tabs = tabs
        B = target.batch
        return self._apply_args(tabs, cur) + (
            ids_ptr, B, self._vocab_dev.data_ptr(), self._max_vocab, B, target.sorted_pos.data_ptr(),
            target.uniq_rows.data_ptr(), target.seg_start.data_ptr(), target.num_uniq.data_ptr(),
            self.row_emb._err.data_ptr())

    def apply_plan_update(self, graph_exec: int, node, cur, ids_ptr: int, target) -> None:
        _lib.check(_lib.load().dfm_step_apply_plan_update(C.c_void_p(graph_exec), node,
                                                          *self._apply_plan_args(cur, ids_ptr, target)))

    def _flat_v_ptr(self) -> int:
        return self.flat_v.data_ptr() if self.kind != "sgd" else 0

    def _dense_source(self):
        if (self.split and self._gathered is not None and self._cur is not None
                and self._cur[0] is self._gathered[1]):
            return self._gathered[0], 0
        return None, 0

    def _extra_partial_count(self, lists: int) -> int:
        return 0

    def _dense_partial_offset(self, lists: int) -> int:
        return 0

    def _norm_partials(self, n_partials: int, lists: int):
        return self._partials.data_ptr(), n_partials

    def step(self) -> None:
        self.exchange()
        self.apply()

    def _table_state(self):
        return list(zip(self._tables, self.exp_avg, self.exp_avg_sq))

    def _named(self):
        names = {id(p): n for n, p in self.model.named_parameters()}
        return ([(names[id(p)], m, v) for p, m, v in self._table_state()],
                [(names[id(p)], p) for p in self.dense_params])

    def _slots(self):
        return ("momentum_buffer",) if self.kind == "sgd" else ("exp_avg", "exp_avg_sq")

    def state_dict(self) -> dict:
        tables, dense = self._named()
        slots = self._slots()
        state = {}
        for name, m, v in tables:
            arrays = (m,) if self.kind == "sgd" else (m, v)
            state[name] = {k: a.detach().clone().contiguous() for k, a in zip(slots, arrays)}
        off = 0
        for name, p in dense:
            n = p.numel()
            arrays = (self.flat_m,) if self.kind == "sgd" else (self.flat_m, self.flat_v)
            state[name] = {k: a[off:off + n].view_as(p).clone() for k, a in zip(slots, arrays)}
            off += (n + 15) // 16 * 16
        return {"step": int(self.step_count.item()), "state": state,
                "hyper": {"kind": self.kind, "lr": self.lr, "betas": list(self.betas), "eps": self.eps,
                          "weight_decay": self.weight_decay, "momentum": self.momentum, "l2": self.l2,
                          "max_grad_norm": self.max_grad_norm}}

    @staticmethod
    def _torch_kind(group: dict) -> str:
        if "betas" not in group:
            return "sgd"
        if "decoupled_weight_decay" in group:
            return "adamw" if group["decoupled_weight_decay"] else "adam"
        return "adamw" if group.get("weight_decay", 0.0) else "adam"

    def load_state_dict(self, sd: dict) -> None:
        slots = self._slots()
        lr = None
        if "param_groups" in sd:
            kinds = {self._torch_kind(g) for g in sd["param_groups"]}
            if kinds != {self.kind}:
                raise ValueError(f"{type(self).__name__} cannot load the state of a torch {'/'.join(sorted(kinds))} "
                                 f"optimizer")
            lr = sd["param_groups"][0].get("lr")
            names = [n for n, _ in self.model.named_parameters()]
            order = [i for g in sd["param_groups"] for i in g["params"]]
            if len(order) != len(names):
                raise KeyError(f"torch optimizer state covers {len(order)} parameters, the model has {len(names)}")
            shapes = dict(self.model.named_parameters())
            state, step = {}, 0
            for i, name in zip(order, names):
                st = sd["state"].get(i)
                if st is None or any(k not in st for k in slots):
                    state[name] = {k: torch.zeros_like(shapes[name], memory_format=torch.contiguous_format)
                                   for k in slots}
                else:
                    state[name] = {k: st[k] for k in slots}
                if st is not None and "step" in st:
                    step = max(step, int(st["step"]))
            sd = {"step": step, "state": state}
        else:
            hyper = sd.get("hyper", {})
            kind = hyper.get("kind", "adam")
            if kind != self.kind:
                raise ValueError(f"{type(self).__name__} cannot load the state of a row-sparse {kind} optimizer")
            lr = hyper.get("lr")
        tables, dense = self._named()
        want = {n for n, _, _ in tables} | {n for n, _ in dense}
        if set(sd["state"]) != want:
            raise KeyError(f"optimizer state keys differ: {sorted(set(sd['state']) ^ want)[:5]} ...")
        with torch.no_grad():
            for name, m, v in tables:
                m.copy_(sd["state"][name][slots[0]])
                if self.kind != "sgd":
                    v.copy_(sd["state"][name][slots[1]])
            off = 0
            for name, p in dense:
                n = p.numel()
                self.flat_m[off:off + n].copy_(sd["state"][name][slots[0]].reshape(-1))
                if self.kind != "sgd":
                    self.flat_v[off:off + n].copy_(sd["state"][name][slots[1]].reshape(-1))
                off += (n + 15) // 16 * 16
            self.step_count.fill_(int(sd["step"]))
        if lr is not None:
            self.lr = float(lr)


class _LrGroup(dict):

    def __init__(self, opt: RowSparseOptimizer) -> None:
        super().__init__(lr=opt.lr)
        self._opt = opt

    def __getitem__(self, key):
        return self._opt.lr if key == "lr" else super().__getitem__(key)

    def __setitem__(self, key, value) -> None:
        if key == "lr":
            self._opt.lr = value
        super().__setitem__(key, value)


class RowSparseAdam(RowSparseOptimizer):
    kind = "adam"

    def __init__(self, model: torch.nn.Module, lr: float = 1e-3, betas=(0.9, 0.999), eps: float = 1e-8,
                 l2: float = 0.0, max_grad_norm: Optional[float] = None,
                 process_group: Optional[dist.ProcessGroup] = None,
                 row_embedding: Optional[FeatureEmbedding] = None) -> None:
        super().__init__(model, lr=lr, betas=betas, eps=eps, l2=l2, max_grad_norm=max_grad_norm,
                         process_group=process_group, row_embedding=row_embedding)


class RowSparseAdamW(RowSparseOptimizer):
    kind = "adamw"

    def __init__(self, model: torch.nn.Module, lr: float = 1e-3, betas=(0.9, 0.999), eps: float = 1e-8,
                 weight_decay: float = 1e-2, l2: float = 0.0, max_grad_norm: Optional[float] = None,
                 process_group: Optional[dist.ProcessGroup] = None,
                 row_embedding: Optional[FeatureEmbedding] = None) -> None:
        super().__init__(model, lr=lr, betas=betas, eps=eps, l2=l2, max_grad_norm=max_grad_norm,
                         process_group=process_group, row_embedding=row_embedding, weight_decay=weight_decay)


class RowSparseSGD(RowSparseOptimizer):
    kind = "sgd"

    def __init__(self, model: torch.nn.Module, lr: float = 1e-3, momentum: float = 0.9, l2: float = 0.0,
                 max_grad_norm: Optional[float] = None, process_group: Optional[dist.ProcessGroup] = None,
                 row_embedding: Optional[FeatureEmbedding] = None) -> None:
        super().__init__(model, lr=lr, l2=l2, max_grad_norm=max_grad_norm, process_group=process_group,
                         row_embedding=row_embedding, momentum=momentum)


OPTIMIZERS = {"adam": RowSparseAdam, "adamw": RowSparseAdamW, "sgd": RowSparseSGD}


def build_optimizer(model: torch.nn.Module, cfg) -> RowSparseOptimizer:
    tc = cfg.training
    cls = OPTIMIZERS.get(tc.optimizer)
    if cls is None:
        raise ValueError(f"Unknown optimizer: {tc.optimizer}")
    clip = tc.gradient_clip_norm
    return cls(model, lr=tc.lr, l2=cfg.feature.embedding_l2_reg, max_grad_norm=clip if clip else None)
```

deepfm_amd/training/step.py:

```python

from __future__ import annotations

import atexit
import ctypes as C
import os
import weakref
from typing import List, Optional

import torch

from deepfm_amd import _lib
from deepfm_amd.data.packed import RecordLayout
from deepfm_amd.data.schema import FeatureType
from deepfm_amd.training.losses import bce_with_logits_mean
from deepfm_amd.training.rowsparse import RowSparseOptimizer


TOWER_MODE_DEFAULT = 0

_LIVE_STEPS: "weakref.WeakSet" = weakref.WeakSet()


def release_all_graphs() -> None:
    for step in list(_LIVE_STEPS):
        try:
            step.release_graphs()
        except Exception:
            pass


atexit.register(release_all_graphs)


class _GraphSlot:

    def __init__(self) -> None:
        self.graph: Optional[torch.cuda.CUDAGraph] = None
        self.nodes: List[C.c_void_p] = []
        self.done: Optional[torch.cuda.Event] = None


class RowSparseTrainStep:
    exchange_in_body = False
    rowplan_first_default = True
    plan_lookahead_default = True

    def __init__(self, model, optimizer: RowSparseOptimizer, batch_size: int, use_graph: bool = True) -> None:
        self.model, self.opt, self.B = model, optimizer, batch_size
        self.emb = model.embedding
        self._check_embedding()
        dev = optimizer.device
        specs = list(model.schema.fields.values())
        lay = RecordLayout.of(model.schema, batch_size)
        self.n_sparse, self.n_dense, self.packed_bytes = lay.n_sparse, lay.n_dense, lay.record_bytes
        self.packed = torch.zeros(self.packed_bytes, dtype=torch.uint8, device=dev)
        self.inbox = torch.zeros(self.packed_bytes, dtype=torch.uint8, device=dev)
        self.pad = torch.zeros(self.packed_bytes, dtype=torch.uint8, device=dev)
        self.ids, self.dense, self.labels, self.bags = lay.views(self.packed)
        self.in_ids, self.in_dense, self.in_labels, self.in_bags = lay.views(self.inbox)
        cols = {FeatureType.SPARSE: iter(self.ids), FeatureType.DENSE: iter(self.dense), FeatureType.SEQUENCE: iter(self.bags)}
        self.inputs: List[torch.Tensor] = [next(cols[s.feature_type]) for s in specs]
        self._rec_offsets = list(lay.field_offsets)
        self._rec_labels = lay.labels_offset
        self._rec_id_offsets = [o for o, k in zip(lay.field_offsets, lay.kinds) if k is FeatureType.SPARSE]
        self.rowplan_first = self.n_sparse > 0 and self.rowplan_first_default
        self._plan_done = False
        self.plan_lookahead = self.rowplan_first and self.plan_lookahead_default
        self._plan_sets = None
        self.cont_slots: List[_GraphSlot] = []
        self._turn_cont = 0
        self._prepared = None
        self._handoff_ptr: Optional[int] = None
        self._record: torch.Tensor = self.inbox
        F, D = len(specs), self.emb.fm_embed_dim
        self.fo = torch.empty(batch_size, 1, dtype=torch.float32, device=dev)
        self.fe = torch.empty(batch_size, F, D, dtype=torch.float32, device=dev)
        self.loss = torch.zeros((), dtype=torch.float32, device=dev)
        self.use_graph = use_graph
        self.side = torch.cuda.Stream(device=dev)
        self.slots: List[_GraphSlot] = []
        self.steps_per_graph = 1
        self._turn = 0
        self.graph_b: Optional[torch.cuda.CUDAGraph] = None
        self.body_graph: Optional[torch.cuda.CUDAGraph] = None
        self.dense_grads = {id(p): p.grad for p in self.emb.non_table_parameters() if p.grad is not None}
        self.emb.pin_plan(dev)
        _LIVE_STEPS.add(self)
        for m in model.modules():
            if hasattr(m, "direct_grads"):
                m.direct_grads = True

    def _check_embedding(self) -> None:
        if self.emb.grad_mode != "rowsparse":
            raise ValueError("RowSparseTrainStep needs model.embedding in 'rowsparse' grad mode")

    @property
    def graph_a(self) -> Optional[torch.cuda.CUDAGraph]:
        return self.slots[0].graph if self.slots else None

    def load_batch(self, ids: torch.Tensor, dense: torch.Tensor, labels: torch.Tensor) -> None:
        if self.n_sparse:
            self.in_ids.copy_(ids, non_blocking=True)
        if self.n_dense:
            self.in_dense.copy_(dense, non_blocking=True)
        self.in_labels.copy_(labels, non_blocking=True)
        self._record = self.inbox

    def pack_batches(self, ids: torch.Tensor, dense: torch.Tensor, labels: torch.Tensor) -> torch.Tensor:
        n = labels.shape[0]
        parts = []
        if self.n_sparse:
            parts.append(ids.contiguous().view(n, -1).view(torch.uint8))
        else:
            parts.append(torch.zeros(n, self.B * 8, dtype=torch.uint8, device=labels.device))
        if self.n_dense:
            parts.append(dense.contiguous().view(n, -1).view(torch.uint8))
        else:
            parts.append(torch.zeros(n, self.B * 4, dtype=torch.uint8, device=labels.device))
        parts.append(labels.contiguous().view(n, -1).view(torch.uint8))
        return torch.cat(parts, dim=1).contiguous()

    def load_packed(self, record: torch.Tensor) -> None:
        self.inbox.copy_(record, non_blocking=True)
        self._record = self.inbox

    def _gather_args(self) -> dict:
        return {}

    def _gather_call(self, record: torch.Tensor):
        base = record.data_ptr()
        return ([base + o for o in self._rec_offsets], self.inputs, self.B, self.fo, self.fe), \
            dict(extra_src_ptr=base + self._rec_labels, extra_dst=self.labels, **self._gather_args())

    def _plan_from_record(self, record: torch.Tensor) -> None:
        base = record.data_ptr()
        self.emb.build_rowplan(self.inputs, self.B, ids_ptrs=[base + o for o in self._rec_id_offsets], touch=True)
        self._plan_done = True

    def _gather(self, record: Optional[torch.Tensor] = None) -> None:
        record = self._record if record is None else record
        self._plan_done = False
        if self.rowplan_first and self._handoff_ptr is not None and self._handoff_ptr == record.data_ptr():
            self._plan_done = True
        elif self.rowplan_first:
            self._plan_from_record(record)
        self._handoff_ptr = None
        a, kw = self._gather_call(record)
        self.emb.forward_staged(*a, **kw)

    def _capture_gather(self, record: torch.Tensor, with_plan: bool = True):
        plan_node = None
        self._plan_done = False
        if self.rowplan_first and not with_plan:
            self._plan_done = True
        elif self.rowplan_first:
            self._plan_from_record(record)
            plan_node = C.c_void_p()
            _lib.check(_lib.load().dfm_graph_last_node(_lib.stream_handle(), C.byref(plan_node)))
        a, kw = self._gather_call(record)
        self.emb.forward_staged(*a, **kw)
        node = C.c_void_p()
        _lib.check(_lib.load().dfm_graph_last_node(_lib.stream_handle(), C.byref(node)))
        return (node, plan_node)

    def _update_gather(self, graph_exec: int, node, record: torch.Tensor) -> None:
        node, plan_node = node
        if plan_node is not None:
            base = record.data_ptr()
            self.emb.rowplan_update(graph_exec, plan_node, [base + o for o in self._rec_id_offsets], self.B, True)
        a, kw = self._gather_call(record)
        self.emb.forward_staged_update(graph_exec, node, *a, **kw)

    def _build_rowplan(self) -> None:
        if self._plan_done:
            self._plan_done = False
            return
        self.emb.build_rowplan(self.inputs, self.B)

    def _embedding_backward(self, g_fo: torch.Tensor, g_fe: torch.Tensor) -> None:
        self.emb.backward_rowsparse(self.inputs, g_fo, g_fe, self.dense_grads, dense_slices=self._dense_slices())

    def _dense_slices(self):
        return None

    def _body_a(self) -> None:
        self.opt.zero_grad()
        cur = torch.cuda.current_stream()
        side = os.environ.get("DFM_ROWPLAN_SIDE_STREAM") == "1"
        if side:
            self.side.wait_stream(cur)
            with torch.cuda.stream(self.side):
                self._build_rowplan()
        else:
            self._build_rowplan()
        fo = self.fo.detach().requires_grad_()
        fe = self.fe.detach().requires_grad_()
        logits = self.model._forward_components(fo, fe, fe.view(self.B, -1))
        loss = bce_with_logits_mean(logits.view(-1), self.labels)
        loss.backward()
        self.loss.copy_(loss.detach())
        if side:
            cur.wait_stream(self.side)
        self._embedding_backward(fo.grad, fe.grad)

    def _body_b(self) -> None:
        self.opt.apply()

    def _mutable_state(self) -> List[torch.Tensor]:
        opt = self.opt
        ts = [opt.flat_param, opt.flat_m, opt.flat_v, opt.flat_grad, opt.step_count, opt.sq_norm, opt.clip_coef,
              self.loss, self.packed]
        if opt.seed_tick is not None:
            ts.append(opt.seed_tick)
        seed = getattr(getattr(self.model, "dnn", None), "_seed", None)
        if seed is not None:
            ts.append(seed)
        ts += list(self.model.buffers())
        return ts

    def capture(self, warmup_iters: int = 1, timed_variant: bool = False, steps_per_graph: int = 1) -> None:
        if not self.use_graph:
            return
        state = self._mutable_state()
        saved = [t.clone() for t in state]
        try:
            self._capture(warmup_iters, timed_variant, steps_per_graph)
        except BaseException:
            self.slots, self.body_graph, self.graph_b = [], None, None
            self.cont_slots, self._turn_cont, self._handoff_ptr = [], 0, None
            self.steps_per_graph, self._turn = 1, 0
            self._plan_done = False
            raise
        finally:
            torch.cuda.synchronize()
            with torch.no_grad():
                for t, v in zip(state, saved):
                    t.copy_(v)
            torch.cuda.synchronize()

    def _capture(self, warmup_iters: int, timed_variant: bool, steps_per_graph: int) -> None:
        side = torch.cuda.Stream()
        side.wait_stream(torch.cuda.current_stream())
        with torch.cuda.stream(side):
            for _ in range(warmup_iters):
                self._gather(self.pad)
                self._body_a()
                self.opt.exchange()
                self._body_b()
        torch.cuda.current_stream().wait_stream(side)
        torch.cuda.synchronize()
        single = not self.opt.split
        fused_exchange = self.exchange_in_body or (
            (not single) and os.environ.get("DFM_DP_GRAPH_COLLECTIVE") == "1"
            and torch.distributed.is_initialized() and torch.distributed.get_backend() == "nccl")
        mode = dict(capture_error_mode="thread_local")
        def body():
            self._body_a()
            if single or fused_exchange:
                self.opt.exchange()
                self._body_b()
        if steps_per_graph < 1 or (steps_per_graph > 1 and not single and not fused_exchange):
            raise ValueError("steps_per_graph > 1 needs the whole step inside one graph (one rank, or the in-graph exchange)")
        self.steps_per_graph = steps_per_graph
        self.slots = []
        lib = _lib.load()
        look = self.plan_lookahead and steps_per_graph > 1 and (single or fused_exchange) and self.emb.rowsparse is not None
        sets = None
        if look:
            from deepfm_amd.models.layers.embedding import RowSparseBuffers
            rs = self.emb.rowsparse
            mk = lambda: RowSparseBuffers(rs.num_sparse, rs.dim, rs.batch, rs.row_g2.device)
            sets = self._plan_sets = [rs, mk(), mk()]
        self.cont_slots = []
        ids0 = self.pad.data_ptr() + (self._rec_id_offsets[0] if self._rec_id_offsets else 0)

        def capture_slot(cont: bool) -> _GraphSlot:
            slot = _GraphSlot()
            slot.graph = torch.cuda.CUDAGraph(keep_graph=True)
            with torch.cuda.graph(slot.graph, **mode):
                for k in range(steps_per_graph):
                    if look:
                        self.emb.rowsparse = sets[0] if k == 0 else sets[1 + (k - 1) % 2]
                    read_nodes = (self._capture_gather(self.pad, with_plan=not (look and (k > 0 or cont)))
                                  if self.rowplan_first else self._capture_gather(self.pad))
                    apply_node = cur = target = None
                    if look:
                        target = sets[1 + k % 2] if k + 1 < steps_per_graph else sets[0]
                        self.opt.next_plan = (ids0, target)
                    body()
                    if target is not None:
                        apply_node = C.c_void_p()
                        _lib.check(lib.dfm_graph_last_node(_lib.stream_handle(), C.byref(apply_node)))
                        cur = self.opt._cur
                    slot.nodes.append((read_nodes, apply_node, cur, target))
            slot.graph.instantiate()
            return slot

        for _ in range(2):
            self.slots.append(capture_slot(False))
        if look:
            for _ in range(2):
                self.cont_slots.append(capture_slot(True))
            self.emb.rowsparse = sets[0]
        if timed_variant:
            self.body_graph = torch.cuda.CUDAGraph()
            with torch.cuda.graph(self.body_graph, **mode):
                self._plan_done = self.rowplan_first
                body()
        if not single and not fused_exchange:
            self.opt.exchange()
            torch.cuda.synchronize()
            self.graph_b = torch.cuda.CUDAGraph()
            with torch.cuda.graph(self.graph_b, **mode):
                self._body_b()

    def release_graphs(self) -> None:
        if not self.slots and self.body_graph is None and self.graph_b is None:
            return
        torch.cuda.synchronize()
        self.slots, self.body_graph, self.graph_b = [], None, None
        self.cont_slots, self._turn_cont, self._handoff_ptr = [], 0, None
        self.steps_per_graph, self._turn, self._prepared = 1, 0, None
        import gc
        gc.collect()
        torch.cuda.synchronize()

    def run_from(self, record: torch.Tensor, eager_gather: bool = False) -> None:
        if record.numel() != self.packed_bytes or record.dtype != torch.uint8 or not record.is_contiguous():
            raise ValueError("run_from expects one contiguous pack_batches() record")
        if record.data_ptr() % 16:
            raise ValueError("batch records must be 16-byte aligned")
        self._record = record
        self.run(eager_gather)

    def run(self, eager_gather: bool = False) -> None:
        if not self.slots:
            self._gather()
            self._body_a()
            self.opt.exchange()
            self._body_b()
            return
        if eager_gather:
            if self.body_graph is None:
                raise RuntimeError("run(eager_gather=True) needs capture(timed_variant=True)")
            self._gather()
            self.body_graph.replay()
            self._after_graph_a(None)
            return
        if self.steps_per_graph != 1:
            raise RuntimeError(f"the graphs hold {self.steps_per_graph} steps each: use run_group()")
        self._launch([self._record])

    def run_group(self, records, next_record: Optional[torch.Tensor] = None) -> None:
        if len(records) != self.steps_per_graph:
            raise ValueError(f"run_group expects {self.steps_per_graph} records")
        if not self.slots:
            for r in records:
                self.run_from(r)
            return
        for r in records:
            if r.numel() != self.packed_bytes or r.dtype != torch.uint8 or not r.is_contiguous() or r.data_ptr() % 16:
                raise ValueError("run_group expects contiguous, 16-byte aligned pack_batches() records")
        self._launch(list(records), next_record)

    def prepare_group(self, records, next_record: Optional[torch.Tensor] = None) -> None:
        if len(records) != self.steps_per_graph or not self.slots:
            raise ValueError(f"prepare_group needs captured graphs of {len(records)} steps")
        if self._prepared is not None:
            raise RuntimeError("a prepared launch is pending: call launch_prepared() first")
        self._prepared = self._prepare(list(records), next_record)

    def launch_prepared(self) -> None:
        if self._prepared is None:
            raise RuntimeError("nothing prepared")
        slot, self._prepared = self._prepared, None
        slot.graph.replay()
        self._after_graph_a(slot.done)

    def _launch(self, records, next_record: Optional[torch.Tensor] = None) -> None:
        if self._prepared is not None:
            raise RuntimeError("a prepared launch is pending: call launch_prepared() first")
        slot = self._prepare(records, next_record)
        slot.graph.replay()
        self._after_graph_a(slot.done)

    def _prepare(self, records, next_record: Optional[torch.Tensor] = None):
        cont = bool(self.cont_slots) and self._handoff_ptr is not None and self._handoff_ptr == records[0].data_ptr()
        if cont:
            slot = self.cont_slots[self._turn_cont]
            self._turn_cont ^= 1
        else:
            slot = self.slots[self._turn]
            self._turn ^= 1
        if slot.done is not None:
            slot.done.synchronize()
        else:
            slot.done = torch.cuda.Event()
        ex = slot.graph.raw_cuda_graph_exec()
        for k, ((read_nodes, apply_node, cur, target), rec) in enumerate(zip(slot.nodes, records)):
            self._update_gather(ex, read_nodes, rec)
            if apply_node is not None:
                nxt = records[k + 1] if k + 1 < len(records) else (next_record if next_record is not None else records[0])
                self.opt.apply_plan_update(ex, apply_node, cur, nxt.data_ptr() + self._rec_id_offsets[0], target)
        self._handoff_ptr = next_record.data_ptr() if (next_record is not None and self.cont_slots) else None
        return slot

    def _after_graph_a(self, done) -> None:
        if self.graph_b is not None:
            self.emb.rowsparse.has_grad = True
            self.opt.exchange()
            self.graph_b.replay()
        if done is not None:
            done.record()
```

include/deepfm_hip.h:

```cpp
#ifndef DEEPFM_HIP_H
#define DEEPFM_HIP_H

#include <stddef.h>
#include <stdint.h>

#ifdef __cplusplus
extern "C" {
#endif

#define DFM_ABI_VERSION 9
#define DFM_MAX_FIELDS 64
#define DFM_MAX_RANKS 64
#define DFM_ROWPLAN_CHUNK 4096

enum dfm_status { DFM_OK = 0, DFM_ERR_INVALID = 1, DFM_ERR_HIP = 2, DFM_ERR_UNSUPPORTED = 3 };
enum dfm_field_kind { DFM_SPARSE = 0, DFM_DENSE = 1, DFM_SEQUENCE = 2 };
enum dfm_combiner { DFM_MEAN = 0, DFM_SUM = 1, DFM_MAX = 2 };

typedef void* dfm_stream_t;

int dfm_abi_version(void);
const char* dfm_last_error(void);
int dfm_device_info(int* cu_count, int* wave_size, char* arch, int arch_len);
int dfm_debug_empty_launch(dfm_stream_t stream);


typedef struct dfm_field {
  int32_t kind;
  int32_t dim;
  int32_t vocab;
  int32_t max_len;
  int32_t combiner;
  int32_t flat_offset;
  int32_t stride2;
  int32_t stride1;
  const float* w2;
  const float* b2;
  const float* w1;
  const float* b1;
  const float* proj;
} dfm_field;

typedef struct dfm_field_grad {
  float* w2;
  float* b2;
  float* w1;
  float* b1;
  float* proj;
} dfm_field_grad;

typedef struct dfm_embedding_plan dfm_embedding_plan;

int dfm_embedding_plan_create(const dfm_field* fields, int num_fields, int fm_dim,
                              dfm_embedding_plan** out_plan);
int dfm_embedding_plan_destroy(dfm_embedding_plan* plan);
int dfm_embedding_plan_is_uniform(const dfm_embedding_plan* plan);
size_t dfm_embedding_workspace_bytes(const dfm_embedding_plan* plan, int64_t batch);

int dfm_embedding_forward(const dfm_embedding_plan* plan, const void* const* inputs, int64_t batch,
                          float* d_first_order, float* d_field_emb, float* d_flat_emb,
                          float* d_fm_out, float* d_fm_sum, void* d_workspace, int32_t* d_error_flag,
                          dfm_stream_t stream);

int dfm_embedding_forward_staged(const dfm_embedding_plan* plan, const void* const* inputs,
                                 void* const* stage_out, const float* d_extra_src, float* d_extra_dst,
                                 int64_t batch, float* d_first_order, float* d_field_emb, float* d_fm_out,
                                 float* d_fm_sum, int32_t* d_error_flag, dfm_stream_t stream);

int dfm_embedding_forward_staged_update(const dfm_embedding_plan* plan, void* graph_exec, void* node,
                                        const void* const* inputs, void* const* stage_out,
                                        const float* d_extra_src, float* d_extra_dst, int64_t batch,
                                        float* d_first_order, float* d_field_emb, float* d_fm_out,
                                        float* d_fm_sum, int32_t* d_error_flag);

#define DFM_RECORD_PARAM_LDS_BYTES 32768
int dfm_embedding_forward_record(const dfm_embedding_plan* plan, const void* d_record, int64_t batch,
                                 float* d_first_order, float* d_field_emb, float* d_flat, int64_t ld_flat,
                                 float* d_fm_out, float* d_labels_out, int32_t* d_error_flag, dfm_stream_t stream);
int dfm_embedding_forward_record_update(const dfm_embedding_plan* plan, void* graph_exec, void* node,
                                        const void* d_record, int64_t batch, float* d_first_order,
                                        float* d_field_emb, float* d_flat, int64_t ld_flat, float* d_fm_out,
                                        float* d_labels_out, int32_t* d_error_flag);
int dfm_embedding_forward_record_sum(const dfm_embedding_plan* plan, const void* d_record, int64_t batch,
                                     float* d_first_order, float* d_field_emb, float* d_flat, int64_t ld_flat,
                                     float* d_fm_out, float* d_fm_sum, float* d_labels_out, int32_t* d_error_flag,
                                     dfm_stream_t stream);
int dfm_embedding_forward_record_sum_update(const dfm_embedding_plan* plan, void* graph_exec, void* node,
                                            const void* d_record, int64_t batch, float* d_first_order,
                                            float* d_field_emb, float* d_flat, int64_t ld_flat, float* d_fm_out,
                                            float* d_fm_sum, float* d_labels_out, int32_t* d_error_flag);

#define DFM_BWD_RECORD_MAX_ROW_SAMPLES (1 << 27)
int dfm_embedding_backward_record_parts(int64_t batch);
size_t dfm_embedding_backward_record_workspace_bytes(int64_t batch, int64_t grad_elems);
int dfm_embedding_backward_record(const dfm_embedding_plan* plan, const void* d_record, int64_t batch,
                                  const float* d_g_first, const float* d_g_field, const float* d_g_flat,
                                  int64_t ld_g_flat, const float* d_flat_saved, int64_t ld_flat,
                                  const dfm_field_grad* grads, const float* d_grad_base, int64_t grad_elems,
                                  void* d_workspace, dfm_stream_t stream);
int dfm_embedding_backward_record_update(const dfm_embedding_plan* plan, void* graph_exec, void* node,
                                         const void* d_record, int64_t batch, const float* d_g_first,
                                         const float* d_g_field, const float* d_g_flat, int64_t ld_g_flat,
                                         const float* d_flat_saved, int64_t ld_flat, const dfm_field_grad* grads,
                                         const float* d_grad_base, int64_t grad_elems, void* d_workspace);
int dfm_embedding_backward_record_fm(const dfm_embedding_plan* plan, const void* d_record, int64_t batch,
                                     const float* d_g_first, const float* d_g_field, const float* d_g_flat,
                                     int64_t ld_g_flat, const float* d_flat_saved, int64_t ld_flat,
                                     const float* d_g_fm, const float* d_fm_sum, const float* d_field_emb,
                                     const dfm_field_grad* grads, const float* d_grad_base, int64_t grad_elems,
                                     void* d_workspace, dfm_stream_t stream);
int dfm_embedding_backward_record_fm_update(const dfm_embedding_plan* plan, void* graph_exec, void* node,
                                            const void* d_record, int64_t batch, const float* d_g_first,
                                            const float* d_g_field, const float* d_g_flat, int64_t ld_g_flat,
                                            const float* d_flat_saved, int64_t ld_flat, const float* d_g_fm,
                                            const float* d_fm_sum, const float* d_field_emb,
                                            const dfm_field_grad* grads, const float* d_grad_base, int64_t grad_elems,
                                            void* d_workspace);

int dfm_graph_last_node(dfm_stream_t stream, void** node_out);

int dfm_gather_timing_begin(int launches);
int dfm_gather_timing_end(float* h_us, int capacity, int* h_count);

int dfm_gather_set_shape(int shape);

int dfm_embedding_backward_dense(const dfm_embedding_plan* plan, const void* const* inputs,
                                 int64_t batch, const float* d_g_first, const float* d_g_field,
                                 const float* d_g_flat, const dfm_field_grad* grads,
                                 const void* d_flat_saved, dfm_stream_t stream);

int dfm_embedding_backward_dense_fields(const dfm_embedding_plan* plan, const void* const* inputs,
                                        int64_t batch, const float* d_g_first,
                                        const float* d_g_field, const float* d_g_flat,
                                        const dfm_field_grad* grads, dfm_stream_t stream);


typedef struct dfm_table dfm_table;
int dfm_rowplan_build(const int64_t* const* ids, const int32_t* vocab, int num_sparse, int64_t n,
                      int32_t* d_sorted_pos, int32_t* d_uniq_rows, int32_t* d_seg_start,
                      int32_t* d_num_uniq, int32_t* d_error_flag, const dfm_table* touch_tables, int dim,
                      dfm_stream_t stream);
int dfm_rowplan_build_update(void* graph_exec, void* node, const int64_t* const* ids, const int32_t* vocab,
                             int num_sparse, int64_t n, int32_t* d_sorted_pos, int32_t* d_uniq_rows,
                             int32_t* d_seg_start, int32_t* d_num_uniq, int32_t* d_error_flag,
                             const dfm_table* touch_tables, int dim);

int dfm_rowgrad_build(const int32_t* field_of_sparse, int num_sparse, int num_fields, int dim,
                      int64_t n, const float* d_g_first, const float* d_g_field,
                      const int32_t* d_sorted_pos, int32_t* d_seg_start,
                      const int32_t* d_num_uniq, float* d_row_g2, float* d_row_g1,
                      dfm_stream_t stream);

typedef struct dfm_table {
  float* w2; float* m2; float* v2;
  float* w1; float* m1; float* v1;
  int32_t stride2;
  int32_t stride1;
} dfm_table;

enum dfm_opt_kind { DFM_OPT_ADAM = 0, DFM_OPT_ADAMW = 1, DFM_OPT_SGD = 2 };
typedef struct dfm_optim {
  int32_t kind;
  float beta1, beta2, eps;
  float weight_decay;
  float momentum;
  const float* d_lr;
} dfm_optim;

int64_t dfm_rowadam_num_partials(int num_sparse, int dim, int num_lists);

int dfm_grad_norm_finalize(const float* d_partials, int64_t num_partials, float max_norm,
                           float* d_sq_norm, float* d_clip_coef, int32_t* d_step_tick,
                           int64_t* d_seed_tick, dfm_stream_t stream);

int dfm_fm_forward(const float* d_field_emb, int64_t batch, int num_fields, int dim, float* d_out,
                   dfm_stream_t stream);
int dfm_fm_backward(const float* d_field_emb, const float* d_g_out, int64_t batch, int num_fields,
                    int dim, float* d_g_field, dfm_stream_t stream);
int dfm_embedding_grad_combine(const float* d_g_flat, int64_t ld_flat, const float* d_g_extra, const float* d_g_fm,
                               const float* d_fm_sum, const float* d_field_emb, int64_t batch, int num_fields, int dim,
                               float* d_g_field, dfm_stream_t stream);
int dfm_copy_2d(const float* d_src, int64_t ld_src, float* d_dst, int64_t ld_dst, int64_t rows, int width,
                dfm_stream_t stream);

int dfm_cin_set_mode(int mode);
int dfm_cin_get_mode(void);

int dfm_cin_output_dim(const int32_t* layer_sizes, int num_layers, int split_half);
size_t dfm_cin_saved_bytes(const int32_t* layer_sizes, int num_layers, int split_half, int64_t batch,
                           int num_fields, int dim);
size_t dfm_cin_forward_workspace_bytes(const int32_t* layer_sizes, int num_layers, int split_half,
                                       int num_fields, int dim);
size_t dfm_cin_backward_workspace_bytes(const int32_t* layer_sizes, int num_layers, int split_half,
                                        int64_t batch, int num_fields, int dim);
int dfm_cin_forward(const float* d_x0, int64_t batch, int num_fields, int dim,
                    const float* const* weights, const float* const* biases,
                    const int32_t* layer_sizes, int num_layers, int split_half, float* d_out,
                    float* d_saved, void* d_workspace, dfm_stream_t stream);
int dfm_cin_backward(const float* d_x0, int64_t batch, int num_fields, int dim,
                     const float* const* weights, const int32_t* layer_sizes, int num_layers,
                     int split_half, const float* d_saved, const float* d_g_out, float* d_g_x0,
                     float* const* g_weights, float* const* g_biases, void* d_workspace,
                     dfm_stream_t stream);

int dfm_attention_forward(const float* d_x, int64_t batch, int num_fields, int embed_dim,
                          int attention_dim, int num_heads, int use_residual,
                          const float* const* params, float* d_out, dfm_stream_t stream);
size_t dfm_attention_backward_workspace_bytes(int64_t batch, int embed_dim, int attention_dim);
int dfm_attention_backward(const float* d_x, const float* d_g_out, int64_t batch, int num_fields,
                           int embed_dim, int attention_dim, int num_heads, int use_residual,
                           const float* const* params, float* d_g_x, float* const* g_params,
                           void* d_workspace, dfm_stream_t stream);

int dfm_attention_core_supported(int num_fields, int attention_dim, int num_heads);
int dfm_attention_core_forward(const float* d_qkv, int64_t batch, int num_fields, int attention_dim,
                               int num_heads, float* d_o, dfm_stream_t stream);
int dfm_attention_core_backward(const float* d_qkv, const float* d_g_o, int64_t batch, int num_fields,
                                int attention_dim, int num_heads, float* d_g_qkv, dfm_stream_t stream);
int dfm_attention_qkv_core_supported(int num_fields, int embed_dim, int attention_dim, int num_heads);
int dfm_attention_qkv_core_forward(const float* d_x, const float* d_w_qkv, const float* d_b_qkv, int64_t batch,
                                   int num_fields, int embed_dim, int attention_dim, int num_heads, float* d_o,
                                   dfm_stream_t stream);
int dfm_attention_qkv_core_backward(const float* d_x, const float* d_w_qkv, const float* d_b_qkv,
                                    const float* d_g_o, int64_t batch, int num_fields, int embed_dim,
                                    int attention_dim, int num_heads, float* d_g_qkv, dfm_stream_t stream);
int dfm_attention_block_supported(int num_fields, int embed_dim, int attention_dim, int num_heads);
int dfm_attention_block_forward(const float* d_x, const float* d_w_qkv, const float* d_b_qkv, const float* d_w_out,
                                const float* d_b_out, const float* d_gamma, const float* d_beta, float eps,
                                int64_t batch, int num_fields, int embed_dim, int attention_dim, int num_heads,
                                float* d_o, float* d_y, float* d_out, float* d_stats, int64_t out_group_stride,
                                float* d_x_copy, int64_t x_copy_group_stride, dfm_stream_t stream);
int dfm_attention_block_backward(const float* d_x, const float* d_w_qkv, const float* d_b_qkv, const float* d_w_out,
                                 const float* d_g_y, int residual, int64_t batch, int num_fields, int embed_dim,
                                 int attention_dim, int num_heads, float* d_g_qkv, float* d_g_x,
                                 const float* d_g_flat, int64_t ld_flat, const float* d_g_fm, const float* d_fm_sum,
                                 dfm_stream_t stream);
size_t dfm_layernorm_workspace_bytes(int64_t rows, int dim);
int dfm_layernorm_forward(const float* d_y, const float* d_res, int64_t rows, int dim, const float* d_gamma,
                          const float* d_beta, float eps, float* d_out, float* d_stats, int64_t out_group_rows,
                          int64_t out_group_stride, dfm_stream_t stream);
int dfm_layernorm_backward(const float* d_g_out, const float* d_y, const float* d_res, const float* d_stats,
                           int64_t rows, int dim, const float* d_gamma, float* d_g_sum, float* d_g_gamma,
                           float* d_g_beta, void* d_workspace, int64_t g_group_rows, int64_t g_group_stride,
                           dfm_stream_t stream);

size_t dfm_bn_workspace_bytes(int64_t batch, int features);
int dfm_bn_relu_dropout_forward(const float* d_z, int64_t batch, int features, const float* d_gamma,
                                const float* d_beta, float* d_running_mean, float* d_running_var,
                                int64_t* d_num_batches, float momentum, float eps, float p_drop,
                                const int64_t* d_seed, int salt, float* d_out, float* d_mean_rstd,
                                void* d_workspace, dfm_stream_t stream);
int dfm_bn_relu_dropout_backward(const float* d_g_out, const float* d_z, const float* d_mean_rstd,
                                 const float* d_gamma, const float* d_beta, int64_t batch, int features,
                                 float p_drop, const int64_t* d_seed, int salt, float* d_g_z,
                                 float* d_g_gamma, float* d_g_beta, void* d_workspace,
                                 dfm_stream_t stream);

size_t dfm_bce_workspace_bytes(int64_t n);
int dfm_bce_with_logits(const float* d_logits, const float* d_labels, int64_t n, float* d_loss,
                        float* d_g_logits, void* d_workspace, dfm_stream_t stream);


typedef struct dfm_bn_bwd {
  const float* z;
  const float* mean_rstd;
  const float* gamma;
  const float* beta;
  float* dy;
  float* g_gamma;
  float* g_beta;
  const int64_t* seed;
  void* workspace;
  float p_drop;
  int32_t salt;
} dfm_bn_bwd;

typedef struct dfm_fm_bwd {
  const float* g_fm;
  const float* fm_sum;
  const float* e;
  const float* addend;
  int32_t dim;
} dfm_fm_bwd;

typedef struct dfm_head_tail {
  float* g_w;
  float* g_b;
  float* loss;
  float* g_b2;
} dfm_head_tail;

size_t dfm_linear_bn_workspace_bytes(int64_t batch, int features);
int dfm_linear_bn_forward(const float* d_x, int64_t ldx, const float* d_w, const float* d_bias,
                          int64_t batch, int out_features, int in_features, float* d_z,
                          void* d_workspace, dfm_stream_t stream);
int dfm_bn_relu_dropout_apply(const float* d_z, int64_t batch, int features, const void* d_workspace,
                              const float* d_gamma, const float* d_beta, float* d_mean_rstd,
                              float* d_running_mean, float* d_running_var, int64_t* d_num_batches,
                              float momentum, float eps, float p_drop, const int64_t* d_seed, int salt,
                              float* d_out, dfm_stream_t stream);
size_t dfm_bn_bwd_workspace_bytes(int64_t batch, int features);
int dfm_head_bce(const float* d_a, int64_t batch, int features, const float* d_w, const float* d_b,
                 const float* d_first_order, const float* d_fm, const float* d_labels, float* d_logits,
                 float* d_g_logits, const dfm_bn_bwd* bn, dfm_stream_t stream);
int dfm_head_bn_bce(const void* d_fwd_workspace, float* d_mean_rstd, float* d_running_mean, float* d_running_var,
                    int64_t* d_num_batches, float momentum, float eps, int64_t batch, int features,
                    const float* d_w, const float* d_b, const float* d_first_order, const float* d_fm,
                    const float* d_labels, float* d_logits, float* d_g_logits, const dfm_bn_bwd* bn,
                    dfm_stream_t stream);
int dfm_bn_backward_apply(const dfm_bn_bwd* bn, int64_t batch, int features, const dfm_head_tail* head,
                          float* d_dz, dfm_stream_t stream);
size_t dfm_linear_backward_workspace_bytes(int64_t batch, int out_features, int in_features);
int dfm_linear_backward(const float* d_dz, int64_t batch, int out_features, const float* d_x,
                        int in_features, const float* d_w, float* d_g_x,
                        const dfm_bn_bwd* bn_below, const dfm_fm_bwd* fm, int parts, void* d_workspace,
                        dfm_stream_t stream);
int dfm_linear1_supported(int features);
int dfm_linear1_forward(const float* d_x, int64_t batch, int features, const float* d_w, const float* d_b,
                        float* d_out, dfm_stream_t stream);
int dfm_linear1_backward_splits(int64_t batch);
int dfm_linear1_backward(const float* d_g, const float* d_x, int64_t batch, int features, const float* d_w,
                         float* d_g_x, void* d_workspace, dfm_stream_t stream);
typedef struct dfm_slab_ref {
  const void* workspace;
  float* g_w;
  int64_t batch;
  int32_t out_features;
  int32_t in_features;
  int32_t splits;
  int32_t reserved;
} dfm_slab_ref;
int dfm_linear_backward_finish(const dfm_slab_ref* refs, int count, dfm_stream_t stream);
int dfm_tower_set_mode(int mode);
int dfm_tower_get_mode(void);

size_t dfm_planes_bytes(int64_t rows, int64_t contraction);
int dfm_tower_x6_supported(int64_t batch, int out_features, int in_features);
typedef struct {
  const float* src;
  int64_t rows, cols;
  void* planes_f;
  void* planes_s;
} dfm_split_job;
int dfm_split_planes(const dfm_split_job* jobs, int count, dfm_stream_t stream);
int dfm_linear_bn_forward_x6(const float* d_x, int64_t ldx, const void* d_x_planes_f, const void* d_w_planes_f,
                             const float* d_bias, int64_t batch, int out_features, int in_features, float* d_z,
                             void* d_workspace, dfm_stream_t stream);
int dfm_bn_relu_dropout_apply_planes(const float* d_z, int64_t batch, int features, const void* d_workspace,
                                     const float* d_gamma, const float* d_beta, float* d_mean_rstd,
                                     float* d_running_mean, float* d_running_var, int64_t* d_num_batches,
                                     float momentum, float eps, float p_drop, const int64_t* d_seed, int salt,
                                     float* d_out, void* d_planes_f, void* d_planes_s, dfm_stream_t stream);
int dfm_bn_backward_apply_planes(const dfm_bn_bwd* bn, int64_t batch, int features, const dfm_head_tail* head,
                                 float* d_dz, void* d_planes_f, void* d_planes_s, dfm_stream_t stream);
int dfm_linear_backward_x6_splits(int64_t batch, int out_features, int in_features);
size_t dfm_linear_backward_x6_workspace_bytes(int64_t batch, int out_features, int in_features);
int dfm_linear_backward_x6(const void* d_dz_planes_f, const void* d_dz_planes_s, int64_t batch, int out_features,
                           const float* d_x, const void* d_x_planes_s, int in_features, const void* d_w_planes_s,
                           float* d_g_x, const dfm_bn_bwd* bn_below, const dfm_fm_bwd* fm, void* d_workspace,
                           dfm_stream_t stream);

int dfm_linear_backward_splits(int64_t batch, int out_features, int in_features);

int dfm_step_embedding_backward(const int32_t* d_dense_list, int num_dense, const void* const* dense_x,
                                const dfm_field_grad* dense_grads, const int32_t* field_of_sparse,
                                int num_sparse, int num_fields, int dim, int64_t batch,
                                const float* d_g_first, const float* d_g_field,
                                const int32_t* d_sorted_pos, int32_t* d_seg_start,
                                const int32_t* d_num_uniq, float* d_row_g2, float* d_row_g1,
                                float* d_dense_partials, int dense_parts, const float* d_dense_grad_base,
                                int64_t dense_grad_elems, dfm_stream_t stream);
int64_t dfm_step_prepare_num_partials(int num_sparse, int dim, int num_lists, int64_t n);
size_t dfm_step_match_bytes(int num_sparse, int num_lists);
int dfm_step_prepare(const dfm_table* tables, int num_sparse, int dim, int num_lists,
                     const int32_t* d_uniq_rows, const int32_t* d_num_uniq, float* d_row_g2,
                     float* d_row_g1, int32_t* d_owner_flag, float grad_scale, float l2, float* d_g,
                     const float* d_p, int64_t n, int64_t n_l2, const dfm_slab_ref* slabs, int num_slabs,
                     const float* d_dense_gathered, int world, int64_t gathered_stride, float* d_partials,
                     int64_t dense_partial_offset, void* d_match, dfm_stream_t stream);
int64_t dfm_step_dense_num_partials(int64_t n);
int dfm_step_dense_prepare(float l2, float* d_g, const float* d_p, int64_t n, int64_t n_l2, const dfm_slab_ref* slabs,
                           int num_slabs, float* d_partials, dfm_stream_t stream);
int dfm_step_dense_apply(const float* d_clip_coef, const dfm_optim* opt, const int32_t* d_step, float* d_p, float* d_m,
                         float* d_v, float* d_g, int64_t n, int zero_grad, dfm_stream_t stream);

int dfm_step_apply(const dfm_table* tables, int num_sparse, int dim, int num_lists,
                   const int32_t* d_uniq_rows, const int32_t* d_num_uniq, const float* d_row_g2,
                   const float* d_row_g1, const int32_t* d_owner_flag, const float* d_clip_coef,
                   const dfm_optim* opt, const int32_t* d_step, float* d_p, float* d_m, float* d_v, float* d_g,
                   int64_t n, int zero_grad, dfm_stream_t stream);
int dfm_step_apply_plan(const dfm_table* tables, int num_sparse, int dim, int num_lists,
                        const int32_t* d_uniq_rows, const int32_t* d_num_uniq, const float* d_row_g2,
                        const float* d_row_g1, const int32_t* d_owner_flag, const float* d_clip_coef,
                        const dfm_optim* opt, const int32_t* d_step, float* d_p, float* d_m, float* d_v,
                        float* d_g, int64_t n, int zero_grad, const int64_t* d_next_ids, int64_t ids_stride,
                        const int32_t* d_vocab, int max_vocab, int64_t batch, int32_t* d_next_sorted_pos,
                        int32_t* d_next_uniq_rows, int32_t* d_next_seg_start, int32_t* d_next_num_uniq,
                        int32_t* d_error_flag, dfm_stream_t stream);
int dfm_step_apply_plan_update(void* graph_exec, void* node, const dfm_table* tables, int num_sparse, int dim,
                               int num_lists, const int32_t* d_uniq_rows, const int32_t* d_num_uniq,
                               const float* d_row_g2, const float* d_row_g1, const int32_t* d_owner_flag,
                               const float* d_clip_coef, const dfm_optim* opt, const int32_t* d_step, float* d_p,
                               float* d_m, float* d_v, float* d_g, int64_t n, int zero_grad,
                               const int64_t* d_next_ids, int64_t ids_stride, const int32_t* d_vocab,
                               int max_vocab, int64_t batch, int32_t* d_next_sorted_pos, int32_t* d_next_uniq_rows,
                               int32_t* d_next_seg_start, int32_t* d_next_num_uniq, int32_t* d_error_flag);

size_t dfm_gemm_workspace_bytes(int m, int n, int k);
int dfm_gemm_f32(const float* d_a, int64_t lda, int a_k_contiguous, const float* d_b, int64_t ldb,
                 int b_k_contiguous, float* d_c, int64_t ldc, int m, int n, int k,
                 const float* d_bias, int accumulate, void* d_workspace, dfm_stream_t stream);

size_t dfm_weight_grad_workspace_bytes(int64_t rows, int n1, int n2);
int dfm_weight_grad_f32(const float* d_g, int64_t ldg, const float* d_x, int64_t ldx, int64_t rows, int n1,
                        int n2, float* d_dw, int64_t lddw, float* d_db, int accumulate, void* d_workspace,
                        dfm_stream_t stream);
int dfm_weight_grad_partial_blocks(int64_t rows);
int dfm_weight_grad_partials_f32(const float* d_g, int64_t ldg, const float* d_x, int64_t ldx, int64_t rows, int n1,
                                 int n2, void* d_workspace, dfm_stream_t stream);
int dfm_weight_grad_partials_pair_f32(const float* d_g_a, int64_t ldg_a, const float* d_x_a, int64_t ldx_a, int n1_a,
                                      int n2_a, void* d_workspace_a, const float* d_g_b, int64_t ldg_b,
                                      const float* d_x_b, int64_t ldx_b, int n1_b, int n2_b, void* d_workspace_b,
                                      int64_t rows, dfm_stream_t stream);
int dfm_layernorm_partial_blocks(int64_t rows);
typedef struct {
  int32_t kind;
  int32_t blocks;
  int32_t n1, n2;
  int32_t accumulate;
  int32_t reserved;
  const float* partial;
  float* out_w;
  float* out_b;
  int64_t ldw;
} dfm_partial_job;
int dfm_partials_finish(const dfm_partial_job* jobs, int count, dfm_stream_t stream);

int dfm_stage_record(const void* d_src, void* d_dst, int64_t nbytes, dfm_stream_t stream);
int dfm_stage_record_update(void* graph_exec, void* node, const void* d_src, void* d_dst, int64_t nbytes);
int dfm_shard_gather(const dfm_table* tables, const int32_t* vocab, int num_owned, int dim, int world,
                     int64_t batch, const int64_t* d_ids, float* d_send, int64_t* d_gids,
                     int32_t* d_error_flag, dfm_stream_t stream);
int64_t dfm_shard_pack_segment(int64_t batch, int num_owned, int dim, int64_t n_dense);
int dfm_shard_pack(const int32_t* first_field, const int32_t* field_count, int world,
                   const int32_t* field_of_sparse, int num_sparse, int num_fields, int dim, int64_t batch,
                   const float* d_g_field, const float* d_g_first, const float* d_dense, int64_t n_dense,
                   const dfm_slab_ref* slabs, int num_slabs, float* d_send, dfm_stream_t stream);
int dfm_shard_rowgrad(int num_owned, int dim, int world, int64_t batch, const float* d_recv, int64_t segment,
                      const int32_t* d_sorted_pos, int32_t* d_seg_start, const int32_t* d_num_uniq,
                      float* d_row_g2, float* d_row_g1, dfm_stream_t stream);
int dfm_sum_floats(const float* d_x, int64_t n, float* d_out, dfm_stream_t stream);

int dfm_linear_bn_eval(const float* d_x, int64_t ldx, const float* d_w, const float* d_bias, int64_t batch,
                       int out_features, int in_features, const float* d_gamma, const float* d_beta,
                       const float* d_running_mean, const float* d_running_var, float eps, float* d_out,
                       dfm_stream_t stream);
int dfm_predict_head(const float* d_a, int64_t batch, int features, const float* d_w, const float* d_b,
                     const float* d_first_order, const float* d_extra, int64_t valid, float* d_logits, float* d_probs,
                     dfm_stream_t stream);
int dfm_predict_head_update(void* graph_exec, void* node, const float* d_a, int64_t batch, int features,
                            const float* d_w, const float* d_b, const float* d_first_order, const float* d_extra,
                            int64_t valid, float* d_logits, float* d_probs);
size_t dfm_metrics_workspace_bytes(int64_t n);
int dfm_metrics_prepare(const float* d_labels, const float* d_scores, int64_t n, float* d_keys, void* d_workspace,
                        dfm_stream_t stream);
int dfm_metrics_finish(const float* d_labels, const float* d_scores, int64_t n, const float* d_sorted_keys,
                       void* d_workspace, double* d_out, dfm_stream_t stream);
size_t dfm_ranking_workspace_bytes(int64_t n, int64_t num_users);
int dfm_ranking_metrics(const int64_t* d_user_ids, const float* d_labels, const float* d_scores, int64_t n,
                        int64_t num_users, const int32_t* h_ks, int num_ks, int require_both_classes,
                        void* d_workspace, double* d_out, dfm_stream_t stream);

#ifdef __cplusplus
}
#endif
#endif
```

Before: 20.23 million.

## Fuse embedding backward with optimizer prepare into one launch plus finalize

After: 20.03 million. 0.99x the previous value.

```diff
diff --git a/deepfm_amd/_lib.py b/deepfm_amd/_lib.py
--- a/deepfm_amd/_lib.py
+++ b/deepfm_amd/_lib.py
@@ -173,6 +173,11 @@
     "dfm_step_match_bytes": (_SZ, [_I, _I]),
     "dfm_step_prepare": (_I, [C.POINTER(Table), _I, _I, _I, _P, _P, _P, _P, _P, _F, _F, _P, _P, _L, _L,
                               C.POINTER(SlabRef), _I, _P, _I, _L, _P, _L, _P, _P]),
+    "dfm_step_backward_prepare_num_partials": (_L, [_I, _I, _L, _L, _L]),
+    "dfm_step_backward_prepare": (_I, [_P, _I, C.POINTER(_P), C.POINTER(FieldGrad), C.POINTER(C.c_int32), _I, _I, _I,
+                                       _L, _P, _P, _P, _P, _P, _P, _P, _P, _I, _P, _L, C.POINTER(Table), _P, _P, _F,
+                                       _F, _P, _P, _L, _L, C.POINTER(SlabRef), _I, _P, _P]),
+    "dfm_step_finalize": (_I, [_P, _I, _L, _F, _P, _P, _L, _P, _L, _F, _P, _P, _P, _P, _P]),
     "dfm_step_apply": (_I, [C.POINTER(Table), _I, _I, _I, _P, _P, _P, _P, _P, _P, C.POINTER(Optim), _P, _P, _P, _P,
                             _P, _L, _I, _P]),
     "dfm_step_apply_plan": (_I, [C.POINTER(Table), _I, _I, _I, _P, _P, _P, _P, _P, _P, C.POINTER(Optim), _P, _P, _P,
diff --git a/deepfm_amd/csrc/step_tail.hip b/deepfm_amd/csrc/step_tail.hip
--- a/deepfm_amd/csrc/step_tail.hip
+++ b/deepfm_amd/csrc/step_tail.hip
@@ -65,6 +65,23 @@
                  row_g1);
 }
 
+__global__ __launch_bounds__(kTailThreads, 5) void step_backward_prepare_kernel(
+    int dense_blocks, const int32_t* __restrict__ dense_list, PtrTable in, GradTable gt, int64_t B, int F, int D,
+    const float* __restrict__ g_first, const float* __restrict__ g_field, FieldMap fmap, int S, int lists,
+    const int32_t* __restrict__ sorted_pos, int32_t* seg_start, const int32_t* __restrict__ num_uniq, float* row_g2,
+    float* row_g1, DensePartials dp, int rg_blocks, RowFinish fin, float* __restrict__ g,
+    const float* __restrict__ p, int64_t n, int64_t n_l2, SlabTable slabs) {
+  const int blk = blockIdx.x;
+  if (blk < dense_blocks)
+    dense_fields_uniform_body(blk, dense_list, in, gt, B, F, D, g_first, g_field, dp);
+  else if (blk < dense_blocks + rg_blocks)
+    rowgrad_body<true>(blk - dense_blocks, fmap, S, F, D, lists, g_first, g_field, sorted_pos, seg_start, num_uniq,
+                       row_g2, row_g1, SampleSegments{0, 0}, &fin);
+  else
+    dense_prepare_slabs_body(blk - dense_blocks - rg_blocks, g, p, n, n_l2, fin.l2, slabs, nullptr, 1, 0, 1.f,
+                             fin.partial + rg_blocks);
+}
+
 constexpr int kMatchThreads = 1024;
 __global__ __launch_bounds__(kMatchThreads) void step_match_kernel(int S, int L, const int32_t* __restrict__ uniq_rows,
                                                                   const int32_t* __restrict__ num_uniq,
@@ -103,6 +120,51 @@
   if (threadIdx.x == 0) {
     float tot = 0.f;
     for (int i = 0; i < 16; ++i) tot += wsum[i];
+    sq_out[0] = tot;
+    if (clip_out) {
+      float c = 1.f;
+      if (max_norm > 0.f) c = fminf(1.f, max_norm / (sqrtf(tot) + 1e-6f));
+      clip_out[0] = c;
+    }
+    if (step_tick) step_tick[0] += 1;
+    if (seed_tick) seed_tick[0] += 1;
+  }
+}
+
+constexpr int kFinalizeElems = 4 * 1024;
+__global__ __launch_bounds__(1024) void step_finalize_kernel(const float* __restrict__ slices, int parts,
+                                                             int elems, float l2, float* __restrict__ g,
+                                                             const float* __restrict__ p, int n_l2,
+                                                             const float* __restrict__ partial, int n,
+                                                             float max_norm, float* __restrict__ sq_out,
+                                                             float* __restrict__ clip_out,
+                                                             int32_t* __restrict__ step_tick,
+                                                             int64_t* __restrict__ seed_tick) {
+  __shared__ float wsum[16];
+  float acc = 0.f;
+  const int i = threadIdx.x * 4;
+  if (i < elems) {
+    float4 gi = ld4(g + i);
+    for (int q = 0; q < parts; ++q) {
+      const float4 t = ld4(slices + static_cast<int64_t>(q) * elems + i);
+      gi.x += t.x; gi.y += t.y; gi.z += t.z; gi.w += t.w;
+    }
+    if (i < n_l2) {
+      const float k = 2.f * l2;
+      const float4 pi = ld4(p + i);
+      gi.x = fmaf(k, pi.x, gi.x); gi.y = fmaf(k, pi.y, gi.y); gi.z = fmaf(k, pi.z, gi.z); gi.w = fmaf(k, pi.w, gi.w);
+    }
+    st4(g + i, gi);
+    acc = fmaf(gi.x, gi.x, acc); acc = fmaf(gi.y, gi.y, acc); acc = fmaf(gi.z, gi.z, acc); acc = fmaf(gi.w, gi.w, acc);
+  }
+  for (int j = threadIdx.x; j < n; j += 1024) acc += partial[j];
+#pragma unroll
+  for (int m = 32; m >= 1; m >>= 1) acc += __shfl_xor(acc, m, kWave);
+  if (lane_id() == 0) wsum[threadIdx.x >> 6] = acc;
+  __syncthreads();
+  if (threadIdx.x == 0) {
+    float tot = 0.f;
+    for (int j = 0; j < 16; ++j) tot += wsum[j];
     sq_out[0] = tot;
     if (clip_out) {
       float c = 1.f;
@@ -314,6 +376,141 @@
 }
 
 namespace {
+inline int64_t rowgrad_blocks(int num_sparse, int dim, int64_t batch) {
+  const int64_t lists = (batch + CH - 1) / CH * num_sparse;
+  return (lists * CH * (dim / 4) + kTailThreads - 1) / kTailThreads;
+}
+}
+
+extern "C" int64_t dfm_step_backward_prepare_num_partials(int num_sparse, int dim, int64_t batch, int64_t n,
+                                                          int64_t dense_grad_elems) {
+  if (num_sparse <= 0 || dim <= 0 || dim % 4 || batch <= 0 || dense_grad_elems < 0 || n < dense_grad_elems) return 0;
+  return rowgrad_blocks(num_sparse, dim, batch) + prep_blocks(n - dense_grad_elems) +
+         (batch + CH - 1) / CH * num_sparse * kMaxSplitRuns;
+}
+
+extern "C" int dfm_step_backward_prepare(const int32_t* d_dense_list, int num_dense, const void* const* dense_x,
+                                         const dfm_field_grad* dense_grads, const int32_t* field_of_sparse,
+                                         int num_sparse, int num_fields, int dim, int64_t batch,
+                                         const float* d_g_first, const float* d_g_field,
+                                         const int32_t* d_sorted_pos, int32_t* d_seg_start,
+                                         const int32_t* d_num_uniq, float* d_row_g2, float* d_row_g1,
+                                         float* d_dense_partials, int dense_parts, const float* d_dense_grad_base,
+                                         int64_t dense_grad_elems, const dfm_table* tables,
+                                         const int32_t* d_uniq_rows, int32_t* d_owner_flag, float grad_scale, float l2,
+                                         float* d_g, const float* d_p, int64_t n, int64_t n_l2,
+                                         const dfm_slab_ref* slabs, int num_slabs, float* d_partials,
+                                         dfm_stream_t stream) {
+  DFM_REQUIRE(d_g_first && d_g_field && field_of_sparse && d_sorted_pos && d_seg_start && d_num_uniq && d_row_g2 &&
+                  d_row_g1 && tables && d_uniq_rows && d_owner_flag && d_g && d_p && d_partials, "null argument");
+  DFM_REQUIRE(num_dense >= 0 && num_sparse > 0 && num_fields <= DFM_MAX_FIELDS && num_dense + num_sparse <= num_fields,
+              "bad field counts");
+  DFM_REQUIRE(dim > 0 && dim % 4 == 0 && dim <= 256 && batch > 0 && batch < (int64_t(1) << 31), "bad shape");
+  DFM_REQUIRE((reinterpret_cast<uintptr_t>(d_g_field) & 15) == 0, "d_g_field must be 16-byte aligned");
+  DFM_REQUIRE(n > 0 && n_l2 >= 0 && n_l2 <= n && n_l2 % 16 == 0, "bad dense sizes (n_l2 must be a multiple of 16)");
+  DFM_REQUIRE((reinterpret_cast<uintptr_t>(d_g) & 63) == 0 && (reinterpret_cast<uintptr_t>(d_p) & 15) == 0,
+              "dense buffers must be 64-byte aligned");
+  if (kTailThreads % (dim / 4) != 0)
+    return fail(DFM_ERR_UNSUPPORTED, "dim %d: a row's %d lanes do not tile the workgroup", dim, dim / 4);
+  if (num_dense > 0 && !d_dense_partials)
+    return fail(DFM_ERR_UNSUPPORTED, "DENSE-field gradients added in place would race with the dense blocks: "
+                                     "they must travel as batch slices (d_dense_partials)");
+  int64_t skip = 0;
+  if (num_dense > 0) {
+    if (d_dense_grad_base != d_g || dense_grad_elems <= 0 || dense_grad_elems > kFinalizeElems ||
+        dense_grad_elems % 16 != 0 || dense_grad_elems > n)
+      return fail(DFM_ERR_UNSUPPORTED, "the sliced range must be the first 16..%d floats of the dense buffer (a "
+                                       "multiple of 16): one pass of dfm_step_finalize", kFinalizeElems);
+    skip = dense_grad_elems;
+  }
+  PtrTable in;
+  GradTable gt;
+  memset(&in, 0, sizeof(in));
+  memset(&gt, 0, sizeof(gt));
+  int dense_blocks = 0;
+  DensePartials dp = {nullptr, nullptr, 0, 0, 0};
+  if (num_dense > 0) {
+    DFM_REQUIRE(d_dense_list && dense_x && dense_grads, "null argument");
+    DFM_REQUIRE(dense_parts >= 1 && dense_parts <= 64, "bad dense slices");
+    for (int f = 0; f < num_fields; ++f) {
+      in.p[f] = dense_x[f];
+      gt.g[f] = dense_grads[f];
+      const dfm_field_grad& g = gt.g[f];
+      if (!g.w2) continue;
+      DFM_REQUIRE(g.w2 >= d_g && g.w2 + dim <= d_g + skip && g.b2 >= d_g && g.b2 + dim <= d_g + skip &&
+                      g.w1 >= d_g && g.w1 < d_g + skip && g.b1 >= d_g && g.b1 < d_g + skip,
+                  "field %d: a DENSE-field gradient buffer lies outside the sliced range", f);
+    }
+    dense_blocks = num_dense * (dim / 4 + 1);
+    dp.out = d_dense_partials; dp.base = d_g; dp.elems = skip;
+    dp.rows = (batch + dense_parts - 1) / dense_parts;
+    dp.per_slice = dense_blocks;
+    dense_blocks *= dense_parts;
+  }
+  FieldMap fm;
+  memset(&fm, 0, sizeof(fm));
+  RowFinish fin;
+  memset(&fin, 0, sizeof(fin));
+  TableArgs ta;
+  if (int rc = fill_tables(tables, num_sparse, dim, &ta, 0)) return rc;
+  for (int s = 0; s < num_sparse; ++s) {
+    DFM_REQUIRE(field_of_sparse[s] >= 0 && field_of_sparse[s] < num_fields, "field_of_sparse[%d] out of range", s);
+    fm.f[s] = field_of_sparse[s];
+    fin.w2[s] = ta.t[s].w2; fin.w1[s] = ta.t[s].w1;
+    fin.stride2[s] = ta.t[s].stride2; fin.stride1[s] = ta.t[s].stride1;
+  }
+  fin.uniq_rows = d_uniq_rows; fin.owner_flag = d_owner_flag;
+  fin.grad_scale = grad_scale; fin.l2 = l2; fin.partial = d_partials;
+  fin.split_partial = d_partials + rowgrad_blocks(num_sparse, dim, batch) + prep_blocks(n - skip);
+  dfm_slab_ref kept[kMaxSlabs];
+  int n_kept = 0;
+  DFM_REQUIRE(num_slabs >= 0 && num_slabs <= kMaxSlabs && (num_slabs == 0 || slabs), "0..%d slab references", kMaxSlabs);
+  for (int i = 0; i < num_slabs; ++i) {
+    if (d_dense_partials && slabs[i].workspace == d_dense_partials) {
+      DFM_REQUIRE(slabs[i].g_w == d_g && slabs[i].splits == dense_parts &&
+                      static_cast<int64_t>(slabs[i].out_features) * slabs[i].in_features == skip,
+                  "the slab reference of the DENSE-field slices does not describe them");
+      continue;
+    }
+    DFM_REQUIRE(slabs[i].g_w >= d_g + skip, "a slab-backed weight overlaps the sliced range");
+    kept[n_kept++] = slabs[i];
+  }
+  SlabTable st = {};
+  if (int rc = fill_slab_table(kept, n_kept, d_g, n, &st)) return rc;
+  const int lists = static_cast<int>((batch + CH - 1) / CH) * num_sparse;
+  const int64_t rg = rowgrad_blocks(num_sparse, dim, batch), pb = prep_blocks(n - skip);
+  const int64_t l2_behind = n_l2 > skip ? n_l2 - skip : 0;
+  hipLaunchKernelGGL(step_backward_prepare_kernel, dim3(static_cast<unsigned>(dense_blocks + rg + pb)),
+                     dim3(kTailThreads), 0, as_stream(stream), dense_blocks, d_dense_list, in, gt, batch, num_fields, dim,
+                     d_g_first, d_g_field, fm, num_sparse, lists, d_sorted_pos, d_seg_start, d_num_uniq, d_row_g2,
+                     d_row_g1, dp, static_cast<int>(rg), fin, d_g + skip, d_p + skip, n - skip, l2_behind, st);
+  DFM_LAUNCH_CHECK();
+  return DFM_OK;
+}
+
+extern "C" int dfm_step_finalize(const float* d_dense_partials, int dense_parts, int64_t dense_grad_elems, float l2,
+                                 float* d_g, const float* d_p, int64_t n_l2, const float* d_partials,
+                                 int64_t num_partials, float max_norm, float* d_sq_norm, float* d_clip_coef,
+                                 int32_t* d_step_tick, int64_t* d_seed_tick, dfm_stream_t stream) {
+  DFM_REQUIRE(d_partials && d_sq_norm, "null argument");
+  DFM_REQUIRE(num_partials >= 0 && num_partials < (int64_t(1) << 31), "bad partial count");
+  if (!d_dense_partials) dense_grad_elems = 0;
+  if (dense_grad_elems > 0) {
+    DFM_REQUIRE(d_g && d_p && dense_parts >= 1 && dense_parts <= 64 && n_l2 >= 0, "bad dense slices");
+    if (dense_grad_elems > kFinalizeElems || dense_grad_elems % 16 != 0)
+      return fail(DFM_ERR_UNSUPPORTED, "the sliced range must be 16..%d floats, a multiple of 16", kFinalizeElems);
+    DFM_REQUIRE((reinterpret_cast<uintptr_t>(d_g) & 63) == 0 && (reinterpret_cast<uintptr_t>(d_p) & 15) == 0 &&
+                    (reinterpret_cast<uintptr_t>(d_dense_partials) & 15) == 0, "dense buffers must be aligned");
+  }
+  const int64_t l2_in = n_l2 < dense_grad_elems ? n_l2 : dense_grad_elems;
+  hipLaunchKernelGGL(step_finalize_kernel, dim3(1), dim3(1024), 0, as_stream(stream), d_dense_partials, dense_parts,
+                     static_cast<int>(dense_grad_elems), l2, d_g, d_p, static_cast<int>(l2_in), d_partials,
+                     static_cast<int>(num_partials), max_norm, d_sq_norm, d_clip_coef, d_step_tick, d_seed_tick);
+  DFM_LAUNCH_CHECK();
+  return DFM_OK;
+}
+
+namespace {
 int check_optim(const dfm_optim* o) {
   DFM_REQUIRE(o, "null dfm_optim");
   DFM_REQUIRE(o->kind == DFM_OPT_ADAM || o->kind == DFM_OPT_ADAMW || o->kind == DFM_OPT_SGD,
diff --git a/deepfm_amd/csrc/tail_bodies.h b/deepfm_amd/csrc/tail_bodies.h
--- a/deepfm_amd/csrc/tail_bodies.h
+++ b/deepfm_amd/csrc/tail_bodies.h
@@ -190,12 +190,49 @@
   }
 }
 
+struct RowFinish {
+  const float* w2[DFM_MAX_FIELDS];
+  const float* w1[DFM_MAX_FIELDS];
+  int32_t stride2[DFM_MAX_FIELDS], stride1[DFM_MAX_FIELDS];
+  const int32_t* uniq_rows;
+  int32_t* owner_flag;
+  float grad_scale, l2;
+  float* partial;
+  float* split_partial;
+};
+struct RowWeights {
+  float4 w;
+  float w1;
+};
+__device__ __forceinline__ RowWeights finish_load(const RowFinish& fin, int s, int64_t ent, int q) {
+  const int64_t row = fin.uniq_rows[ent];
+  RowWeights r;
+  r.w = ld4(fin.w2[s] + row * fin.stride2[s] + q * 4);
+  r.w1 = q == 0 ? fin.w1[s][row * fin.stride1[s]] : 0.f;
+  return r;
+}
+__device__ __forceinline__ float finish_row(const RowFinish& fin, const RowWeights& r, int64_t ent, int q, float4& g,
+                                            float& g1) {
+  const float k = 2.f * fin.l2, gs = fin.grad_scale;
+  g.x = fmaf(k, r.w.x, gs * g.x); g.y = fmaf(k, r.w.y, gs * g.y);
+  g.z = fmaf(k, r.w.z, gs * g.z); g.w = fmaf(k, r.w.w, gs * g.w);
+  float sq = g.x * g.x + g.y * g.y + g.z * g.z + g.w * g.w;
+  if (q == 0) {
+    g1 = fmaf(k, r.w1, gs * g1);
+    sq = fmaf(g1, g1, sq);
+    fin.owner_flag[ent] = 1;
+  }
+  return sq;
+}
+
+template <bool FINISH = false>
 __device__ __forceinline__ void rowgrad_body(int blk, FieldMap fmap, int S, int F, int D, int lists, const float* __restrict__ g_first,
     const float* __restrict__ g_field, const int32_t* __restrict__ sorted_pos,
     int32_t* seg_start, const int32_t* __restrict__ num_uniq,
-    float* row_g2, float* row_g1, SampleSegments segs = SampleSegments{0, 0}) {
+    float* row_g2, float* row_g1, SampleSegments segs = SampleSegments{0, 0}, const RowFinish* fin = nullptr) {
   __shared__ float red[kRowgradLds];
   __shared__ int s_last;
+  __shared__ float s_sq[kWave];
   __shared__ int s_long, s_ent[kTailThreads], s_p0[kTailThreads], s_p1[kTailThreads];
   const int lpr = D / 4, groups = kTailThreads / lpr;
   const bool coop = kTailThreads % lpr == 0;
@@ -227,17 +264,22 @@
     const int i = atomicAdd(&s_long, 1);
     s_ent[i] = u; s_p0[i] = p0; s_p1[i] = p1;
   }
+  const int sf = static_cast<int>(list % S);
+  float sq = 0.f;
   if (valid && !is_long && !is_split) {
-    const int f = fmap.f[static_cast<int>(list % S)];
+    const int f = fmap.f[sf];
     const int32_t* pos = sorted_pos + list * CH;
     float4 acc = make_float4(0.f, 0.f, 0.f, 0.f);
     float acc1 = 0.f;
+    RowWeights rw;
+    if (FINISH) rw = finish_load(*fin, sf, list * CH + u, q);
     rowgrad_run(g_field, g_first, pos, p0, p1, 1, F, f, D, q, segs, acc, acc1);
+    if (FINISH) sq += finish_row(*fin, rw, list * CH + u, q, acc, acc1);
     st4(row_g2 + (list * CH + u) * D + q * 4, acc);
     if (q == 0) row_g1[list * CH + u] = acc1;
   }
   __syncthreads();
-  if (!s_long && !n_split) return;
+  if (s_long || n_split) {
   const int n_long = s_long;
   for (int e = 0; e < n_long; ++e) {
     const int64_t ls = list;
@@ -260,15 +302,15 @@
         tot.x += v.x; tot.y += v.y; tot.z += v.z; tot.w += v.w;
         if (q == 0) tot1 += red[gi * (D + 4) + D];
       }
+      if (FINISH) sq += finish_row(*fin, finish_load(*fin, sf, ls * CH + ue, q), ls * CH + ue, q, tot, tot1);
       st4(row_g2 + (ls * CH + ue) * D + q * 4, tot);
       if (q == 0) row_g1[ls * CH + ue] = tot1;
     }
     __syncthreads();
   }
-  if (!n_split) return;
   const int nsl = nbl < kMaxSlices ? nbl : kMaxSlices, bl = blk % nbl;
-  if (bl >= nsl) return;
-  const int f = fmap.f[static_cast<int>(list % S)];
+  if (n_split && bl < nsl) {
+  const int f = fmap.f[sf];
   const int32_t* pos = sorted_pos + list * CH;
   for (int e = 0; e < n_split; ++e) {
     const int ue = seg[CH - 1 - e];
@@ -305,7 +347,7 @@
   if (threadIdx.x == 0)
     s_last = __hip_atomic_fetch_add(counter, 1, __ATOMIC_RELAXED, __HIP_MEMORY_SCOPE_AGENT) == nsl - 1 ? 1 : 0;
   __syncthreads();
-  if (!s_last) return;
+  if (s_last) {
   const int nred = groups < nsl ? groups : nsl;
   for (int e = 0; e < n_split; ++e) {
     const int ue = seg[CH - 1 - e];
@@ -330,12 +372,27 @@
         tot.x += v.x; tot.y += v.y; tot.z += v.z; tot.w += v.w;
         if (q == 0) tot1 += red[gi * (D + 4) + D];
       }
+      if (FINISH)
+        s_sq[q] = finish_row(*fin, finish_load(*fin, sf, list * CH + ue, q), list * CH + ue, q, tot, tot1);
       st4(row_g2 + (list * CH + ue) * D + q * 4, tot);
       if (q == 0) row_g1[list * CH + ue] = tot1;
     }
     __syncthreads();
+    if (FINISH && threadIdx.x == 0) {
+      float t = 0.f;
+      for (int i = 0; i < lpr; ++i) t += s_sq[i];
+      fin->split_partial[list * kMaxSplitRuns + e] = t;
+    }
   }
   if (threadIdx.x == 0) __hip_atomic_store(counter, 0, __ATOMIC_RELAXED, __HIP_MEMORY_SCOPE_AGENT);
+  }
+  }
+  }
+  if (FINISH) {
+    if (coop && blk % nbl == 0 && list < lists && threadIdx.x >= n_split && threadIdx.x < kMaxSplitRuns)
+      fin->split_partial[list * kMaxSplitRuns + threadIdx.x] = 0.f;
+    block_partial(sq, fin->partial, blk);
+  }
 }
 
 __device__ __forceinline__ int find_row(const int32_t* __restrict__ rows, int n, int32_t row) {
diff --git a/deepfm_amd/models/layers/embedding.py b/deepfm_amd/models/layers/embedding.py
--- a/deepfm_amd/models/layers/embedding.py
+++ b/deepfm_amd/models/layers/embedding.py
@@ -327,10 +327,12 @@
 
     def backward_rowsparse(self, inputs: List[torch.Tensor], g_fo: torch.Tensor, g_fe: torch.Tensor,
                            dense_grads: Dict[int, torch.Tensor], sparse: bool = True,
-                           dense_slices: Optional[Tuple[torch.Tensor, int, torch.Tensor]] = None) -> None:
+                           dense_slices: Optional[Tuple[torch.Tensor, int, torch.Tensor]] = None,
+                           finish=None) -> None:
         B, F, D = g_fe.shape
         if B == 0:
             return
+        from deepfm_amd.training import eligibility
         lib = _lib.load()
         plan = self._ensure_plan(g_fe.device)
         S = len(self._sparse_pos) if sparse else 0
@@ -341,17 +343,25 @@
                 pos = [i for i, sp in enumerate(self.schema.fields.values()) if sp.feature_type is FeatureType.DENSE]
                 self._dense_list = torch.tensor(pos, dtype=torch.int32, device=g_fe.device)
             nd = self._dense_list.numel()
-            _lib.check(lib.dfm_step_embedding_backward(
-                self._dense_list.data_ptr(), nd, self._ptr_array(inputs), self._grad_struct(dense_grads), fmap, S, F, D,
-                B, g_fo.data_ptr(), g_fe.data_ptr(), rs.sorted_pos.data_ptr() if S else None,
-                rs.seg_start.data_ptr() if S else None, rs.num_uniq.data_ptr() if S else None,
-                rs.row_g2.data_ptr() if S else None, rs.row_g1.data_ptr() if S else None,
-                dense_slices[0].data_ptr() if dense_slices else None, dense_slices[1] if dense_slices else 0,
-                dense_slices[2].data_ptr() if dense_slices else None,
-                dense_slices[0].numel() // dense_slices[1] if dense_slices else 0, _lib.stream_handle()))
+            args = (self._dense_list.data_ptr(), nd, self._ptr_array(inputs), self._grad_struct(dense_grads), fmap, S, F, D,
+                    B, g_fo.data_ptr(), g_fe.data_ptr(), rs.sorted_pos.data_ptr() if S else None,
+                    rs.seg_start.data_ptr() if S else None, rs.num_uniq.data_ptr() if S else None,
+                    rs.row_g2.data_ptr() if S else None, rs.row_g1.data_ptr() if S else None,
+                    dense_slices[0].data_ptr() if dense_slices else None, dense_slices[1] if dense_slices else 0,
+                    dense_slices[2].data_ptr() if dense_slices else None,
+                    dense_slices[0].numel() // dense_slices[1] if dense_slices else 0)
+            if finish is not None:
+                finish.tail_reason = eligibility.three_launch_tail_reason(finish, True, S, D, nd, dense_slices)
+            if finish is not None and finish.tail_reason is None:
+                _lib.check(lib.dfm_step_backward_prepare(*args, *finish.backward_prepare_args(rs, dense_slices),
+                                                         _lib.stream_handle()))
+            else:
+                _lib.check(lib.dfm_step_embedding_backward(*args, _lib.stream_handle()))
             if S:
                 rs.has_grad = True
             return
+        if finish is not None:
+            finish.tail_reason = eligibility.three_launch_tail_reason(finish, False, S, D, 0, dense_slices)
         if dense_grads:
             _lib.check(lib.dfm_embedding_backward_dense_fields(
                 plan, self._ptr_array(inputs), B, g_fo.data_ptr(), g_fe.data_ptr(), None,
diff --git a/deepfm_amd/training/eligibility.py b/deepfm_amd/training/eligibility.py
--- a/deepfm_amd/training/eligibility.py
+++ b/deepfm_amd/training/eligibility.py
@@ -167,6 +167,35 @@
     return None
 
 
+TAIL3_MAX_SLICED = 4096
+
+
+def three_launch_tail_reason(opt, grouped: bool, sparse: int, dim: int, dense_fields: int, dense_slices) -> Optional[str]:
+    import os
+    if os.environ.get("DFM_TAIL3") != "1":
+        return "not selected (DFM_TAIL3=1 selects the three-launch tail)"
+    if opt is None or not opt.row_tables or opt.split or type(opt)._norm_partials is not _plain_optimizer()._norm_partials:
+        return "the optimizer merges several sets of row lists or exchanges its norm partials (data parallel, sharded)"
+    if not grouped or sparse == 0:
+        return "the embedding backward is not the grouped launch with row gradients"
+    if 256 % (dim // 4):
+        return f"embedding_dim {dim}: a row's {dim // 4} lanes do not tile the 256-thread workgroup"
+    if dense_fields:
+        if dense_slices is None:
+            return "DENSE-field gradients are added in place (no batch slices)"
+        partials, parts, flat = dense_slices
+        elems = partials.numel() // parts
+        if flat.data_ptr() != opt.flat_grad.data_ptr() or elems % 16 or not 0 < elems <= TAIL3_MAX_SLICED:
+            return (f"the sliced DENSE-field range ({elems} floats) is not the first 16..{TAIL3_MAX_SLICED} floats of "
+                    "the flat gradient buffer")
+    return None
+
+
+def _plain_optimizer():
+    from deepfm_amd.training.rowsparse import RowSparseOptimizer
+    return RowSparseOptimizer
+
+
 def _predictor_reason(model, gather_reason) -> Optional[str]:
     if family_reason(model, "fused predictor") is not None:
         return f"no fused predictor for {type(model).__name__} ({_FAMILY} only)"
diff --git a/deepfm_amd/training/rowsparse.py b/deepfm_amd/training/rowsparse.py
--- a/deepfm_amd/training/rowsparse.py
+++ b/deepfm_amd/training/rowsparse.py
@@ -116,6 +116,12 @@
         self._cur = None
         self.seed_tick: Optional[torch.Tensor] = None
         self.slab_refs = None
+        self.tail_reason: Optional[str] = "no embedding backward of a training step has run"
+        self._finished = None
+
+    @property
+    def tail_launches(self) -> int:
+        return 3 if self.tail_reason is None else 4
 
     @property
     def lr(self) -> float:
@@ -143,6 +149,7 @@
     def zero_grad(self, force: bool = False) -> None:
         if force:
             self.flat_grad.zero_()
+        self._finished = None
         if self.row_emb.rowsparse is not None:
             self.row_emb.rowsparse.has_grad = False
 
@@ -184,13 +191,18 @@
         grad_scale = 1.0 / self.world
         uniq, num, g2, g1, lists = self._cur
         n_dense = self.flat_param.numel()
-        n_partials = lib.dfm_step_prepare_num_partials(self.num_sparse, self.dim, lists, n_dense)
-        if self._owner is None or self._owner.shape != uniq.shape:
-            self._owner = torch.empty_like(uniq)
-            self._partials = torch.zeros(n_partials + self._extra_partial_count(lists), dtype=torch.float32,
-                                         device=self.device)
-            mbytes = lib.dfm_step_match_bytes(self.num_sparse, lists)
-            self._match = torch.empty(mbytes, dtype=torch.uint8, device=self.device) if mbytes else None
+        n_partials = self._tail_buffers(uniq, lists)
+        fin, self._finished = self._finished, None
+        if fin is not None and fin[0].uniq_rows is uniq:
+            _, n_norm, slices = fin
+            _lib.check(lib.dfm_step_finalize(
+                slices[0].data_ptr() if slices else None, slices[1] if slices else 0,
+                slices[0].numel() // slices[1] if slices else 0, self.l2, self.flat_grad.data_ptr(),
+                self.flat_param.data_ptr(), self.n_l2, self._partials.data_ptr(), n_norm, self.max_grad_norm or 0.0,
+                self.sq_norm.data_ptr(), self.clip_coef.data_ptr(), self.step_count.data_ptr(),
+                _lib.ptr(self.seed_tick), stream))
+            self._apply_launch(self._table_struct(), stream)
+            return
         dense_gathered, gathered_stride = self._dense_source()
         tabs = self._table_struct()
         refs, n_refs = self.slab_refs if (self.slab_refs is not None and not self.split) else (None, 0)
@@ -205,6 +217,10 @@
                                               self.max_grad_norm or 0.0, self.sq_norm.data_ptr(),
                                               self.clip_coef.data_ptr(), self.step_count.data_ptr(),
                                               _lib.ptr(self.seed_tick), stream))
+        self._apply_launch(tabs, stream)
+
+    def _apply_launch(self, tabs, stream) -> None:
+        lib = _lib.load()
         if self.next_plan is not None:
             ids_ptr, target = self.next_plan
             self.next_plan = None
@@ -212,6 +228,30 @@
         else:
             _lib.check(lib.dfm_step_apply(*self._apply_args(tabs, self._cur), stream))
         self.row_emb.rowsparse.has_grad = False
+
+    def _tail_buffers(self, uniq: torch.Tensor, lists: int) -> int:
+        lib = _lib.load()
+        n_partials = lib.dfm_step_prepare_num_partials(self.num_sparse, self.dim, lists, self.flat_param.numel())
+        if self._owner is None or self._owner.shape != uniq.shape:
+            self._owner = torch.empty_like(uniq)
+            self._partials = torch.zeros(n_partials + 2 * lists * self.num_sparse + self._extra_partial_count(lists),
+                                         dtype=torch.float32, device=self.device)
+            mbytes = lib.dfm_step_match_bytes(self.num_sparse, lists)
+            self._match = torch.empty(mbytes, dtype=torch.uint8, device=self.device) if mbytes else None
+        return n_partials
+
+    def backward_prepare_args(self, rs, dense_slices):
+        lib = _lib.load()
+        self._tail_buffers(rs.uniq_rows, rs.chunks)
+        tabs = self._table_struct()
+        refs, n_refs = self.slab_refs if self.slab_refs is not None else (None, 0)
+        n = self.flat_param.numel()
+        elems = dense_slices[0].numel() // dense_slices[1] if dense_slices else 0
+        n_norm = lib.dfm_step_backward_prepare_num_partials(self.num_sparse, self.dim, rs.batch, n, elems)
+        self._finished = (rs, n_norm, dense_slices)
+        return (tabs, rs.uniq_rows.data_ptr(), self._owner.data_ptr(), 1.0 / self.world, self.l2,
+                self.flat_grad.data_ptr(), self.flat_param.data_ptr(), n, self.n_l2, refs, n_refs,
+                self._partials.data_ptr())
 
     def _apply_args(self, tabs, cur):
         uniq, num, g2, g1, lists = cur
diff --git a/deepfm_amd/training/step.py b/deepfm_amd/training/step.py
--- a/deepfm_amd/training/step.py
+++ b/deepfm_amd/training/step.py
@@ -178,7 +178,8 @@
         self.emb.build_rowplan(self.inputs, self.B)
 
     def _embedding_backward(self, g_fo: torch.Tensor, g_fe: torch.Tensor) -> None:
-        self.emb.backward_rowsparse(self.inputs, g_fo, g_fe, self.dense_grads, dense_slices=self._dense_slices())
+        self.emb.backward_rowsparse(self.inputs, g_fo, g_fe, self.dense_grads, dense_slices=self._dense_slices(),
+                                    finish=self.opt)
 
     def _dense_slices(self):
         return None
diff --git a/include/deepfm_hip.h b/include/deepfm_hip.h
--- a/include/deepfm_hip.h
+++ b/include/deepfm_hip.h
@@ -378,6 +378,24 @@
                      const float* d_p, int64_t n, int64_t n_l2, const dfm_slab_ref* slabs, int num_slabs,
                      const float* d_dense_gathered, int world, int64_t gathered_stride, float* d_partials,
                      int64_t dense_partial_offset, void* d_match, dfm_stream_t stream);
+int64_t dfm_step_backward_prepare_num_partials(int num_sparse, int dim, int64_t batch, int64_t n,
+                                               int64_t dense_grad_elems);
+int dfm_step_backward_prepare(const int32_t* d_dense_list, int num_dense, const void* const* dense_x,
+                              const dfm_field_grad* dense_grads, const int32_t* field_of_sparse,
+                              int num_sparse, int num_fields, int dim, int64_t batch,
+                              const float* d_g_first, const float* d_g_field,
+                              const int32_t* d_sorted_pos, int32_t* d_seg_start,
+                              const int32_t* d_num_uniq, float* d_row_g2, float* d_row_g1,
+                              float* d_dense_partials, int dense_parts, const float* d_dense_grad_base,
+                              int64_t dense_grad_elems, const dfm_table* tables,
+                              const int32_t* d_uniq_rows, int32_t* d_owner_flag, float grad_scale, float l2,
+                              float* d_g, const float* d_p, int64_t n, int64_t n_l2,
+                              const dfm_slab_ref* slabs, int num_slabs, float* d_partials,
+                              dfm_stream_t stream);
+int dfm_step_finalize(const float* d_dense_partials, int dense_parts, int64_t dense_grad_elems, float l2,
+                      float* d_g, const float* d_p, int64_t n_l2, const float* d_partials,
+                      int64_t num_partials, float max_norm, float* d_sq_norm, float* d_clip_coef,
+                      int32_t* d_step_tick, int64_t* d_seed_tick, dfm_stream_t stream);
 int64_t dfm_step_dense_num_partials(int64_t n);
 int dfm_step_dense_prepare(float l2, float* d_g, const float* d_p, int64_t n, int64_t n_l2, const dfm_slab_ref* slabs,
                            int num_slabs, float* d_partials, dfm_stream_t stream);
```
